# Codes4Fun/moshi.cpp

Measured on AMD Instinct MI355X. Metric: audio frames/sec (12.5 Hz target) moshika-7B q4_k decode, higher is better.
Workload: dtype q4_K weights x q8_K activations (int8 dot, f32 accumulate); bf16 KV; f32 elsewhere; 1 GPU; moshi-sts --bench loop: mimi encode + Temporal step + 8 Depth steps + mimi decode, moshika q4_k, 1 audio stream per GPU, greedy, ctx capacity 3000; context_fill_start=0, parallelism=1 GPU, device= (gfx950:sramecc+:xnack-)

## Files before the change

include/ggml-backend.h:

```cpp
#pragma once

#include "ggml.h"

#ifdef __cplusplus
extern "C" {
#endif

typedef struct ggml_backend_buffer_type * ggml_backend_buffer_type_t;
typedef struct ggml_backend_buffer      * ggml_backend_buffer_t;
typedef struct ggml_backend             * ggml_backend_t;
typedef struct ggml_backend_reg         * ggml_backend_reg_t;
typedef struct ggml_backend_device      * ggml_backend_dev_t;

enum ggml_backend_dev_type {
    GGML_BACKEND_DEVICE_TYPE_CPU,
    GGML_BACKEND_DEVICE_TYPE_GPU,
    GGML_BACKEND_DEVICE_TYPE_ACCEL,
};

struct ggml_backend_dev_caps {
    bool async;
    bool host_buffer;
    bool buffer_from_host_ptr;
    bool events;
// ... 13 lines not shown
GGML_API ggml_backend_reg_t ggml_backend_reg_get(size_t index);
GGML_API const char * ggml_backend_reg_name(ggml_backend_reg_t reg);
GGML_API void * ggml_backend_reg_get_proc_address(ggml_backend_reg_t reg, const char * name);

GGML_API size_t             ggml_backend_dev_count(void);
GGML_API ggml_backend_dev_t ggml_backend_dev_get(size_t index);
GGML_API ggml_backend_dev_t ggml_backend_dev_by_name(const char * name);
GGML_API ggml_backend_dev_t ggml_backend_dev_by_type(enum ggml_backend_dev_type type);
GGML_API const char *       ggml_backend_dev_name(ggml_backend_dev_t device);
GGML_API const char *       ggml_backend_dev_description(ggml_backend_dev_t device);
GGML_API enum ggml_backend_dev_type ggml_backend_dev_type(ggml_backend_dev_t device);
GGML_API void               ggml_backend_dev_memory(ggml_backend_dev_t device, size_t * free, size_t * total);
GGML_API void               ggml_backend_dev_get_props(ggml_backend_dev_t device, struct ggml_backend_dev_props * props);
GGML_API ggml_backend_reg_t ggml_backend_dev_backend_reg(ggml_backend_dev_t device);
GGML_API ggml_backend_t     ggml_backend_dev_init(ggml_backend_dev_t device, const char * params);

GGML_API ggml_backend_t ggml_backend_init_by_name(const char * name, const char * params);
GGML_API ggml_backend_t ggml_backend_init_by_type(enum ggml_backend_dev_type type, const char * params);
GGML_API ggml_backend_t ggml_backend_init_best(void);

GGML_API const char *       ggml_backend_name(ggml_backend_t backend);
GGML_API void               ggml_backend_free(ggml_backend_t backend);
GGML_API ggml_backend_dev_t ggml_backend_get_device(ggml_backend_t backend);
GGML_API void               ggml_backend_synchronize(ggml_backend_t backend);

typedef void (*ggml_backend_set_n_threads_t)(ggml_backend_t backend, int n_threads);

GGML_API ggml_backend_buffer_t ggml_backend_alloc_ctx_tensors(struct ggml_context * ctx, ggml_backend_t backend);
GGML_API void    ggml_backend_buffer_free    (ggml_backend_buffer_t buffer);
GGML_API size_t  ggml_backend_buffer_get_size(ggml_backend_buffer_t buffer);
GGML_API void *  ggml_backend_buffer_get_base(ggml_backend_buffer_t buffer);
GGML_API const char * ggml_backend_buffer_name(ggml_backend_buffer_t buffer);
GGML_API void    ggml_backend_buffer_clear   (ggml_backend_buffer_t buffer, uint8_t value);
GGML_API bool    ggml_backend_buffer_is_host (ggml_backend_buffer_t buffer);

GGML_API void ggml_backend_tensor_set   (      struct ggml_tensor * tensor, const void * data, size_t offset, size_t size);
GGML_API void ggml_backend_tensor_get   (const struct ggml_tensor * tensor,       void * data, size_t offset, size_t size);
GGML_API void ggml_backend_tensor_get_async(ggml_backend_t backend, const struct ggml_tensor * tensor, void * data, size_t offset, size_t size);
typedef struct ggml_backend_event * ggml_backend_event_t;
GGML_API ggml_backend_event_t ggml_backend_event_new(ggml_backend_dev_t device);
GGML_API void ggml_backend_event_free(ggml_backend_event_t event);
GGML_API void ggml_backend_event_record(ggml_backend_event_t event, ggml_backend_t backend);
GGML_API void ggml_backend_event_synchronize(ggml_backend_event_t event);
GGML_API void ggml_backend_event_wait(ggml_backend_t backend, ggml_backend_event_t event);
GGML_API void ggml_backend_tensor_memset(      struct ggml_tensor * tensor, uint8_t value,     size_t offset, size_t size);
GGML_API void ggml_backend_tensor_copy  (struct ggml_tensor * src, struct ggml_tensor * dst);

GGML_API enum ggml_status ggml_backend_graph_compute(ggml_backend_t backend, struct ggml_cgraph * cgraph);
GGML_API bool ggml_backend_supports_op(ggml_backend_t backend, const struct ggml_tensor * op);

struct ggml_mi355x_stats {
    int64_t graphs_computed;
    int64_t graph_replays;
    int64_t kernels_in_last_plan;
    int64_t fused_nodes_in_last_plan;
    int64_t nodes_in_last_plan;
    int64_t uploads_batched;
    int64_t chained_matvecs_in_last_plan;
    int64_t attention_folds_planned;
    int64_t chain_step_programs_in_last_plan;
    int64_t vq_levels_chained_in_last_plan;
    int64_t attn_block_launches_in_last_plan;
    int64_t attn_block_jobs_in_last_plan;
    int64_t generic_attention_nodes_in_last_plan;
    int64_t ring_copy_launches_in_last_plan;
    int64_t ring_copy_jobs_in_last_plan;
};
GGML_API void ggml_backend_mi355x_get_stats(ggml_backend_t backend, struct ggml_mi355x_stats * stats);
struct ggml_mi355x_kernel_profile {
    double  seconds;
    int64_t launches;
    int64_t bytes;
    double  variant_seconds[3];
    int64_t variant_launches[3];
    int64_t variant_bytes[3];
    double  chain_seconds;
    int64_t chain_launches;
    int64_t chain_bytes;
    int64_t chain_phases;
};
GGML_API void ggml_backend_mi355x_get_kernel_profile(ggml_backend_t backend, struct ggml_mi355x_kernel_profile * out);
GGML_API void ggml_backend_mi355x_set_flags(ggml_backend_t backend, int flags);
GGML_API void ggml_backend_mi355x_set_capture(ggml_backend_t backend, int enabled);
GGML_API void * ggml_backend_mi355x_get_stream(ggml_backend_t backend);
GGML_API void ggml_backend_mi355x_make_current(ggml_backend_t backend);
GGML_API ggml_backend_t ggml_backend_mi355x_init_stream(ggml_backend_t base);

#ifdef __cplusplus
}
#endif
```

moshi.cpp_amd/__init__.py:

```python
import ctypes as C
import os

_HERE = os.path.dirname(os.path.abspath(__file__))
LIB_PATH = os.environ.get("MI355X_LIB") or os.path.join(_HERE, "libggml-mi355x.so")
HOT_LIB_PATH = os.environ.get("MI355X_HOT_LIB") or os.path.join(os.path.dirname(LIB_PATH), "libmoshi-hot.so")

GGML_MAX_DIMS, GGML_MAX_SRC, GGML_MAX_NAME = 4, 10, 64

F32, F16, Q4_0, Q8_0, Q4_K, Q8_K, I32, I64, BF16 = 0, 1, 2, 8, 12, 15, 26, 27, 30
TYPE_NAMES = {F32: "f32", F16: "f16", Q4_0: "q4_0", Q8_0: "q8_0", Q4_K: "q4_K", Q8_K: "q8_K", I32: "i32", I64: "i64", BF16: "bf16"}
DEV_CPU, DEV_GPU = 0, 1


class Tensor(C.Structure):
    pass


Tensor._fields_ = [
    ("type", C.c_int),
    ("buffer", C.c_void_p),
    ("ne", C.c_int64 * GGML_MAX_DIMS),
    ("nb", C.c_size_t * GGML_MAX_DIMS),
    ("op", C.c_int),
    ("op_params", C.c_int32 * 16),
# ... 20 lines not shown

class Stats(C.Structure):
    _fields_ = [(n, C.c_int64) for n in ("graphs_computed", "graph_replays", "kernels_in_last_plan",
                                         "fused_nodes_in_last_plan", "nodes_in_last_plan", "uploads_batched", "chained_matvecs_in_last_plan",
                                         "attention_folds_planned", "chain_step_programs_in_last_plan", "vq_levels_chained_in_last_plan",
                                         "attn_block_launches_in_last_plan", "attn_block_jobs_in_last_plan", "generic_attention_nodes_in_last_plan",
                                         "ring_copy_launches_in_last_plan", "ring_copy_jobs_in_last_plan")]


class KernelProfile(C.Structure):
    _fields_ = [("seconds", C.c_double), ("launches", C.c_int64), ("bytes", C.c_int64),
                ("variant_seconds", C.c_double * 3), ("variant_launches", C.c_int64 * 3), ("variant_bytes", C.c_int64 * 3),
                ("chain_seconds", C.c_double), ("chain_launches", C.c_int64), ("chain_bytes", C.c_int64), ("chain_phases", C.c_int64)]


class GGUFInitParams(C.Structure):
    _fields_ = [("no_alloc", C.c_bool), ("ctx", C.POINTER(C.c_void_p))]


P, I, L, Z, F, B, S = C.c_void_p, C.c_int, C.c_int64, C.c_size_t, C.c_float, C.c_bool, C.c_char_p

SIGNATURES = {
    "ggml_time_ms": (L, []), "ggml_time_us": (L, []), "ggml_time_init": (None, []),
    "ggml_type_name": (S, [I]), "ggml_op_name": (S, [I]), "ggml_op_desc": (S, [TP]), "ggml_status_to_string": (S, [I]),
    "ggml_blck_size": (L, [I]), "ggml_type_size": (Z, [I]), "ggml_row_size": (Z, [I, L]), "ggml_is_quantized": (B, [I]),
    "ggml_nelements": (L, [TP]), "ggml_nrows": (L, [TP]), "ggml_nbytes": (Z, [TP]), "ggml_element_size": (Z, [TP]),
    "ggml_n_dims": (I, [TP]), "ggml_is_contiguous": (B, [TP]), "ggml_is_transposed": (B, [TP]), "ggml_is_permuted": (B, [TP]),
    "ggml_are_same_shape": (B, [TP, TP]),
    "ggml_fp16_to_fp32": (F, [C.c_uint16]), "ggml_fp32_to_fp16": (C.c_uint16, [F]),
    "ggml_bf16_to_fp32": (F, [C.c_uint16]), "ggml_fp32_to_bf16": (C.c_uint16, [F]),
    "ggml_init": (P, [InitParams]), "ggml_reset": (None, [P]), "ggml_free": (None, [P]), "ggml_used_mem": (Z, [P]),
    "ggml_get_no_alloc": (B, [P]), "ggml_set_no_alloc": (None, [P, B]),
    "ggml_tensor_overhead": (Z, []), "ggml_graph_overhead": (Z, []), "ggml_graph_overhead_custom": (Z, [Z, B]),
    "ggml_new_tensor": (TP, [P, I, I, C.POINTER(L)]), "ggml_new_tensor_1d": (TP, [P, I, L]), "ggml_new_tensor_2d": (TP, [P, I, L, L]),
    "ggml_new_tensor_3d": (TP, [P, I, L, L, L]), "ggml_new_tensor_4d": (TP, [P, I, L, L, L, L]),
    "ggml_dup_tensor": (TP, [P, TP]), "ggml_view_tensor": (TP, [P, TP]),
    "ggml_get_first_tensor": (TP, [P]), "ggml_get_next_tensor": (TP, [P, TP]), "ggml_get_tensor": (TP, [P, S]),
    "ggml_get_name": (S, [TP]), "ggml_set_name": (TP, [TP, S]), "ggml_format_name": (TP, [TP, S]),
    "ggml_set_input": (None, [TP]), "ggml_set_output": (None, [TP]), "ggml_get_unary_op": (I, [TP]),
    "ggml_dup": (TP, [P, TP]), "ggml_add": (TP, [P, TP, TP]), "ggml_add_inplace": (TP, [P, TP, TP]), "ggml_sub": (TP, [P, TP, TP]),
    "ggml_sub_inplace": (TP, [P, TP, TP]), "ggml_mul_inplace": (TP, [P, TP, TP]), "ggml_div_inplace": (TP, [P, TP, TP]),
    "ggml_mul": (TP, [P, TP, TP]), "ggml_div": (TP, [P, TP, TP]), "ggml_neg": (TP, [P, TP]),
    "ggml_scale": (TP, [P, TP, F]), "ggml_scale_inplace": (TP, [P, TP, F]), "ggml_clamp": (TP, [P, TP, F, F]),
    "ggml_sum": (TP, [P, TP]), "ggml_sum_rows": (TP, [P, TP]), "ggml_argmax": (TP, [P, TP]),
    "ggml_argsort": (TP, [P, TP, I]), "ggml_argsort_top_k": (TP, [P, TP, I]), "ggml_top_k": (TP, [P, TP, I]),
    "ggml_arange": (TP, [P, F, F, F]), "ggml_repeat": (TP, [P, TP, TP]), "ggml_repeat_4d": (TP, [P, TP, L, L, L, L]),
    "ggml_concat": (TP, [P, TP, TP, I]), "ggml_pad": (TP, [P, TP, I, I, I, I]),
    "ggml_silu": (TP, [P, TP]), "ggml_gelu": (TP, [P, TP]), "ggml_elu": (TP, [P, TP]),
    "ggml_norm": (TP, [P, TP, F]), "ggml_rms_norm": (TP, [P, TP, F]), "ggml_mul_mat": (TP, [P, TP, TP]),
    "ggml_soft_max": (TP, [P, TP]), "ggml_soft_max_ext": (TP, [P, TP, TP, F, F]),
    "ggml_cast": (TP, [P, TP, I]), "ggml_cpy": (TP, [P, TP, TP]), "ggml_cont": (TP, [P, TP]),
    "ggml_reshape_1d": (TP, [P, TP, L]), "ggml_reshape_2d": (TP, [P, TP, L, L]), "ggml_reshape_3d": (TP, [P, TP, L, L, L]),
    "ggml_reshape_4d": (TP, [P, TP, L, L, L, L]),
    "ggml_view_1d": (TP, [P, TP, L, Z]), "ggml_view_2d": (TP, [P, TP, L, L, Z, Z]), "ggml_view_3d": (TP, [P, TP, L, L, L, Z, Z, Z]),
    "ggml_view_4d": (TP, [P, TP, L, L, L, L, Z, Z, Z, Z]),
    "ggml_permute": (TP, [P, TP, I, I, I, I]), "ggml_transpose": (TP, [P, TP]),
    "ggml_get_rows": (TP, [P, TP, TP]), "ggml_set_rows": (TP, [P, TP, TP, TP]),
    "ggml_im2col": (TP, [P, TP, TP, I, I, I, I, I, I, B, I]), "ggml_conv_1d": (TP, [P, TP, TP, I, I, I]),
    "ggml_conv_transpose_1d": (TP, [P, TP, TP, I, I, I]), "ggml_timestep_embedding": (TP, [P, TP, I, I]),
    "ggml_new_graph": (P, [P]), "ggml_new_graph_custom": (P, [P, Z, B]), "ggml_build_forward_expand": (None, [P, TP]),
    "ggml_graph_clear": (None, [P]), "ggml_graph_size": (I, [P]), "ggml_graph_n_nodes": (I, [P]), "ggml_graph_node": (TP, [P, I]),
    "ggml_graph_nodes": (C.POINTER(TP), [P]), "ggml_graph_n_leafs": (I, [P]), "ggml_graph_leaf": (TP, [P, I]), "ggml_graph_print": (None, [P]),
    "ggml_quantize_row": (None, [I, P, P, L]), "ggml_dequantize_row": (None, [I, P, P, L]),
    "ggml_backend_load_all": (None, []), "ggml_backend_reg_count": (Z, []), "ggml_backend_reg_get": (P, [Z]),
    "ggml_backend_reg_name": (S, [P]), "ggml_backend_reg_get_proc_address": (P, [P, S]),
    "ggml_backend_dev_count": (Z, []), "ggml_backend_dev_get": (P, [Z]), "ggml_backend_dev_by_name": (P, [S]),
    "ggml_backend_dev_by_type": (P, [I]), "ggml_backend_dev_name": (S, [P]), "ggml_backend_dev_description": (S, [P]),
    "ggml_backend_dev_type": (I, [P]), "ggml_backend_dev_memory": (None, [P, C.POINTER(Z), C.POINTER(Z)]),
    "ggml_backend_dev_get_props": (None, [P, C.POINTER(DevProps)]), "ggml_backend_dev_backend_reg": (P, [P]),
    "ggml_backend_dev_init": (P, [P, S]),
    "ggml_backend_init_by_name": (P, [S, S]), "ggml_backend_init_by_type": (P, [I, S]), "ggml_backend_init_best": (P, []),
    "ggml_backend_name": (S, [P]), "ggml_backend_free": (None, [P]), "ggml_backend_get_device": (P, [P]),
    "ggml_backend_synchronize": (None, [P]),
    "ggml_backend_alloc_ctx_tensors": (P, [P, P]), "ggml_backend_buffer_free": (None, [P]), "ggml_backend_buffer_get_size": (Z, [P]),
    "ggml_backend_buffer_get_base": (P, [P]), "ggml_backend_buffer_name": (S, [P]), "ggml_backend_buffer_clear": (None, [P, C.c_uint8]),
    "ggml_backend_buffer_is_host": (B, [P]),
    "ggml_backend_tensor_set": (None, [TP, P, Z, Z]), "ggml_backend_tensor_get": (None, [TP, P, Z, Z]),
    "ggml_backend_tensor_memset": (None, [TP, C.c_uint8, Z, Z]), "ggml_backend_tensor_copy": (None, [TP, TP]),
    "ggml_backend_graph_compute": (I, [P, P]), "ggml_backend_supports_op": (B, [P, TP]),
    "ggml_backend_mi355x_get_stats": (None, [P, C.POINTER(Stats)]), "ggml_backend_mi355x_set_flags": (None, [P, I]), "ggml_backend_mi355x_set_capture": (None, [P, I]),
    "ggml_backend_mi355x_get_stream": (P, [P]),
    "ggml_backend_mi355x_make_current": (None, [P]),
    "ggml_backend_mi355x_init_stream": (P, [P]),
    "ggml_backend_tensor_get_async": (None, [P, TP, P, Z, Z]),
    "ggml_backend_event_new": (P, [P]), "ggml_backend_event_free": (None, [P]), "ggml_backend_event_record": (None, [P, P]),
    "ggml_backend_event_synchronize": (None, [P]),
    "ggml_backend_event_wait": (None, [P, P]),
    "ggml_backend_mi355x_get_kernel_profile": (None, [P, C.POINTER(KernelProfile)]),
    "ggml_backend_cpu_init": (P, []), "ggml_backend_is_cpu": (B, [P]), "ggml_backend_cpu_set_n_threads": (None, [P, I]),
    "ggml_graph_compute_with_ctx": (I, [P, P, I]),
    "ggml_backend_cpu_reg": (P, []), "ggml_backend_cpu_set_graph_compute": (None, [P]),
    "gguf_init_empty": (P, []), "gguf_init_from_file": (P, [S, GGUFInitParams]), "gguf_free": (None, [P]),
    "gguf_get_version": (C.c_uint32, [P]), "gguf_get_alignment": (Z, [P]), "gguf_get_data_offset": (Z, [P]),
    "gguf_get_n_kv": (L, [P]), "gguf_find_key": (L, [P, S]), "gguf_get_key": (S, [P, L]), "gguf_get_val_str": (S, [P, L]),
    "gguf_get_val_u32": (C.c_uint32, [P, L]), "gguf_set_val_u32": (None, [P, S, C.c_uint32]), "gguf_set_val_str": (None, [P, S, S]),
    "gguf_get_n_tensors": (L, [P]), "gguf_find_tensor": (L, [P, S]), "gguf_get_tensor_name": (S, [P, L]),
    "gguf_get_tensor_type": (I, [P, L]), "gguf_get_tensor_offset": (Z, [P, L]), "gguf_get_tensor_size": (Z, [P, L]),
    "gguf_add_tensor": (None, [P, TP]), "gguf_write_to_file": (B, [P, S, B]),
}

_lib = None


class _Libs:

    def __init__(self, ggml, hot):
        self.ggml, self.hot = ggml, hot

    def __getattr__(self, name):
        for lib in (self.__dict__["ggml"], self.__dict__["hot"]):
            try:
                fn = getattr(lib, name)
            except AttributeError:
                continue
            setattr(self, name, fn)
            return fn
        raise AttributeError(name)


def load():
    global _lib
    if _lib is not None:
        return _lib
    for path in (LIB_PATH, HOT_LIB_PATH):
        if not os.path.exists(path):
            raise RuntimeError(f"{path} not found: build it with moshi.cpp_amd/build.sh (hipcc --offload-arch=gfx950); "
                               "there is no CPU or Python fallback for the decode hot path")
    lib = C.CDLL(LIB_PATH, mode=C.RTLD_GLOBAL)
    missing = []
    for name, (res, args) in SIGNATURES.items():
        try:
            fn = getattr(lib, name)
        except AttributeError:
            missing.append(name)
            continue
        fn.restype, fn.argtypes = res, args
    if missing:
        raise RuntimeError(f"libggml-mi355x.so lacks symbols declared in include/*.h: {missing}")
    stray = [n for n in ("moshi_hot_create", "moshi_hot_sts_frame") if hasattr(lib, n)]
    if stray:
        raise RuntimeError(f"the boundary library must not carry the harness: {stray}")
    hot_lib = C.CDLL(HOT_LIB_PATH, mode=C.RTLD_GLOBAL)
    from . import hot as _hot
    _hot.attach(hot_lib)
    _lib = _Libs(lib, hot_lib)
    return _lib


def declared_symbols():
    return sorted(SIGNATURES)
```

moshi.cpp_amd/csrc/hip_backend.hip:

```cpp
#include "hip_common.h"
#include "ggml-cpu.h"

#include <string.h>

#include <algorithm>
#include <functional>
#include <deque>
#include <map>
#include <memory>
#include <set>
#include <string>
#include <unordered_map>
#include <vector>

#define UPLOAD_SLOTS       8
#define UPLOAD_BLOB_BYTES  (64 * 1024)
#define UPLOAD_MAX_DESCS   1024
#define READBACK_PINNED_BYTES (64 * 1024)
#define AGET_SLOTS 64
#define AGET_SLOT_BYTES 256
#define UPLOAD_SMALL_MAX   16384

struct plan_t;

struct upload_slot {
    char * blob = nullptr;
    upload_desc * descs = nullptr;
    hipEvent_t done = nullptr;
    bool in_flight = false;
};

struct hip_ctx {
    int device = 0;
    std::string name, description;
    hipStream_t stream = nullptr;
    int flags = 0;
    bool no_capture = false;
    ggml_mi355x_stats stats = {};
    std::map<size_t, std::vector<void *>> pool;
    upload_slot slots[UPLOAD_SLOTS];
    int cur_slot = 0;
    int n_pending = 0;
    size_t pending_bytes = 0;
    mv_profile prof = { nullptr, 0, 0 };
    double prof_seconds = 0; int64_t prof_launches = 0, prof_bytes = 0;
    double prof_seconds_v[3] = { 0, 0, 0 }; int64_t prof_launches_v[3] = { 0, 0, 0 }, prof_bytes_v[3] = { 0, 0, 0 };
    double prof_chain_seconds = 0; int64_t prof_chain_launches = 0, prof_chain_bytes = 0, prof_chain_phases = 0;
    hipEvent_t chain_ev[2] = { nullptr, nullptr };
    std::unordered_map<const ggml_cgraph *, plan_t *> plans;
    uint64_t orphan_clock = 0;
    volatile unsigned * err_host = nullptr;
    unsigned * err_dev = nullptr;
    char * readback = nullptr;
    struct async_get { void * dst; size_t size; int slot; uint64_t seq; };
    char * aget_pinned = nullptr;
    std::deque<async_get> aget_pending;
    uint64_t aget_seq = 0;
    bool in_use = false;
    int usable_cus = 0;
    ggml_backend_device dev_obj;
};

static std::vector<hip_ctx *> & contexts() { static std::vector<hip_ctx *> v; return v; }
static std::vector<hip_ctx *> & stream_contexts() { static std::vector<hip_ctx *> v; return v; }

static void set_device(hip_ctx * c) { HIP_CHECK(hipSetDevice(c->device)); }

static void ctx_init_lazy(hip_ctx * c) {
    if (c->stream) return;
    set_device(c);
    {
        hipDeviceProp_t prop;
        HIP_CHECK(hipGetDeviceProperties(&prop, c->device));
        c->usable_cus = prop.multiProcessorCount;
        const char * e = getenv("MI355X_STREAM_CUS");
        const int lim = e ? atoi(e) : 0;
        if (lim > 0 && lim < prop.multiProcessorCount) {
            std::vector<uint32_t> mask((size_t) (prop.multiProcessorCount + 31) / 32, 0u);
            for (int i = 0; i < lim; i++) mask[(size_t) i / 32] |= 1u << (i % 32);
            HIP_CHECK(hipExtStreamCreateWithCUMask(&c->stream, (uint32_t) mask.size(), mask.data()));
            c->usable_cus = lim;
        }
    }
    if (!c->stream) HIP_CHECK(hipStreamCreateWithFlags(&c->stream, hipStreamNonBlocking));
    for (auto & s : c->slots) {
        HIP_CHECK(hipHostMalloc((void **) &s.blob, UPLOAD_BLOB_BYTES, hipHostMallocMapped));
        HIP_CHECK(hipHostMalloc((void **) &s.descs, UPLOAD_MAX_DESCS * sizeof(upload_desc), hipHostMallocMapped));
        HIP_CHECK(hipEventCreateWithFlags(&s.done, hipEventDisableTiming));
    }
    HIP_CHECK(hipHostMalloc((void **) &c->readback, READBACK_PINNED_BYTES, hipHostMallocDefault));
    HIP_CHECK(hipHostMalloc((void **) &c->aget_pinned, AGET_SLOTS * AGET_SLOT_BYTES, hipHostMallocDefault));
    HIP_CHECK(hipHostMalloc((void **) &c->err_host, 64, hipHostMallocMapped));
    c->err_host[0] = 0u;
    HIP_CHECK(hipHostGetDevicePointer((void **) &c->err_dev, (void *) c->err_host, 0));
}

static void check_device_error(hip_ctx * c) {
    if (c->err_host && c->err_host[0] != 0u)
        GGML_ABORT("mi355x backend: a kernel gave up a bounded wait (code %u: 1 = split attention head barrier, 2 = chain engine hand-off, 3 = stream engine hand-off); results are invalid", c->err_host[0]);
}

static size_t size_class(size_t n) {
    if (n > ((size_t) 64 << 20)) return 0;
    size_t c = 256;
    while (c < n) c <<= 1;
    return c;
}
static void * pool_poison(hip_ctx * c, void * p, size_t n) {
    static const bool poison = getenv("MI355X_POISON") != nullptr;
    if (poison && p) { HIP_CHECK(hipMemsetAsync(p, 0xFF, n, c->stream)); HIP_CHECK(hipStreamSynchronize(c->stream)); }
    return p;
}
#define GUARD_BYTES 4096
static bool guard_mode() { static const bool g = getenv("MI355X_GUARD") != nullptr; return g; }
static void guard_fill(hip_ctx * c, char * user, size_t actual) {
    HIP_CHECK(hipMemsetAsync(user - GUARD_BYTES, 0xA5, GUARD_BYTES, c->stream));
    HIP_CHECK(hipMemsetAsync(user + actual, 0xA5, GUARD_BYTES, c->stream));
}
static void guard_check(hip_ctx * c, char * user, size_t actual) {
    static std::vector<unsigned char> h(2 * GUARD_BYTES);
    HIP_CHECK(hipStreamSynchronize(c->stream));
    HIP_CHECK(hipMemcpy(h.data(), user - GUARD_BYTES, GUARD_BYTES, hipMemcpyDeviceToHost));
    HIP_CHECK(hipMemcpy(h.data() + GUARD_BYTES, user + actual, GUARD_BYTES, hipMemcpyDeviceToHost));
    for (size_t i = 0; i < 2 * GUARD_BYTES; i++)
        if (h[i] != 0xA5) GGML_ABORT("mi355x: guard zone %s a %zu-byte allocation was overwritten (offset %zu)", i < GUARD_BYTES ? "before" : "after", actual, i % GUARD_BYTES);
}
static void * pool_alloc(hip_ctx * c, size_t n, size_t * actual) {
    set_device(c);
    const size_t cls = size_class(n ? n : 1);
    if (cls) {
        auto & fl = c->pool[cls];
        *actual = cls;
        if (!fl.empty()) { void * p = fl.back(); fl.pop_back(); if (guard_mode()) guard_fill(c, (char *) p, *actual); return pool_poison(c, p, *actual); }
    } else *actual = n;
    void * p = nullptr;
    hipError_t e = hipMalloc(&p, *actual + (guard_mode() ? 2 * GUARD_BYTES : 0));
    if (e != hipSuccess) { fprintf(stderr, "mi355x: hipMalloc(%zu) failed: %s\n", *actual, hipGetErrorString(e)); return nullptr; }
    if (guard_mode()) { p = (char *) p + GUARD_BYTES; guard_fill(c, (char *) p, *actual); }
    return pool_poison(c, p, *actual);
}
// ... 35 lines not shown
    c->pending_bytes += padded;
}

struct hip_buffer_ctx { hip_ctx * c; size_t actual; };

static void deliver_async_gets(hip_ctx * c, uint64_t upto) {
    while (!c->aget_pending.empty() && c->aget_pending.front().seq <= upto) {
        const hip_ctx::async_get & g = c->aget_pending.front();
        memcpy(g.dst, c->aget_pinned + (size_t) g.slot * AGET_SLOT_BYTES, g.size);
        c->aget_pending.pop_front();
    }
}

static void evict_plans_of_buffer(hip_ctx * c, const ggml_backend_buffer * b);

static void hip_buf_free(ggml_backend_buffer_t b) {
    hip_buffer_ctx * bc = (hip_buffer_ctx *) b->context;
    flush_uploads(bc->c);
    evict_plans_of_buffer(bc->c, b);
    for (hip_ctx * o : contexts()) if (o != bc->c && o->device == bc->c->device) evict_plans_of_buffer(o, b);
    for (hip_ctx * o : stream_contexts()) if (o != bc->c && o->device == bc->c->device) evict_plans_of_buffer(o, b);
    pool_free(bc->c, b->base, bc->actual);
    delete bc;
    delete b;
}
static void hip_buf_set(ggml_backend_buffer_t b, struct ggml_tensor * t, const void * data, size_t offset, size_t size) {
    hip_ctx * c = ((hip_buffer_ctx *) b->context)->c;
    set_device(c);
    if (size <= UPLOAD_SMALL_MAX && !(c->flags & 4)) { queue_upload(c, (char *) t->data + offset, data, size); return; }
    flush_uploads(c);
    HIP_CHECK(hipMemcpyAsync((char *) t->data + offset, data, size, hipMemcpyHostToDevice, c->stream));
    HIP_CHECK(hipStreamSynchronize(c->stream));
}
static void hip_buf_get(ggml_backend_buffer_t b, const struct ggml_tensor * t, void * data, size_t offset, size_t size) {
    hip_ctx * c = ((hip_buffer_ctx *) b->context)->c;
    set_device(c);
    flush_uploads(c);
    if (size <= READBACK_PINNED_BYTES) {
        HIP_CHECK(hipMemcpyAsync(c->readback, (const char *) t->data + offset, size, hipMemcpyDeviceToHost, c->stream));
        HIP_CHECK(hipStreamSynchronize(c->stream));
        memcpy(data, c->readback, size);
    } else {
        HIP_CHECK(hipMemcpyAsync(data, (const char *) t->data + offset, size, hipMemcpyDeviceToHost, c->stream));
        HIP_CHECK(hipStreamSynchronize(c->stream));
    }
    deliver_async_gets(c, c->aget_seq);
    check_device_error(c);
}
static void hip_buf_memset(ggml_backend_buffer_t b, struct ggml_tensor * t, uint8_t v, size_t offset, size_t size) {
    hip_ctx * c = ((hip_buffer_ctx *) b->context)->c;
    set_device(c);
    flush_uploads(c);
    HIP_CHECK(hipMemsetAsync((char *) t->data + offset, v, size, c->stream));
}
static void hip_buf_clear(ggml_backend_buffer_t b, uint8_t v) {
    hip_ctx * c = ((hip_buffer_ctx *) b->context)->c;
    set_device(c);
    flush_uploads(c);
    HIP_CHECK(hipMemsetAsync(b->base, v, b->size, c->stream));
}

static ggml_backend_buffer_t hip_alloc_buffer(ggml_backend_t backend, size_t size) {
    hip_ctx * c = (hip_ctx *) backend->context;
    ctx_init_lazy(c);
    size_t actual = 0;
    void * p = pool_alloc(c, size, &actual);
    if (!p) return NULL;
    auto * b = new ggml_backend_buffer;
    b->iface = { hip_buf_free, hip_buf_memset, hip_buf_set, hip_buf_get, hip_buf_clear };
    b->device = &c->dev_obj;
    b->base = p;
    b->size = size;
    b->context = new hip_buffer_ctx{ c, actual };
    b->is_host = false;
    return b;
}

typedef std::function<void(hipStream_t)> step_fn;
struct pstep {
    step_fn fn; bool is_mv = false; mv_args mv;
    chain_plan * chain = nullptr;
    const vq_level_args * vq = nullptr;
    const char * hoist_dst = nullptr; size_t hoist_bytes = 0;
    template <typename F> pstep(F f) : fn(std::move(f)) { memset(&mv, 0, sizeof(mv)); }
    pstep(const mv_args & a) : fn([a](hipStream_t s) { k_matvec(s, a); }), is_mv(true), mv(a) {}
    template <typename F> static pstep special_step(F f, int special, const attn_args * at, const lowrank_embed_args * lr, const sample_args * smp = nullptr) {
        pstep st(std::move(f));
        st.is_mv = true; st.mv.special = special; st.mv.attn = at; st.mv.lr = lr; st.mv.smp = smp;
        return st;
    }
};

struct plan_t {
    std::vector<pstep> steps;
    std::vector<chain_plan *> chains;
    std::vector<std::pair<void *, size_t>> workspaces;
    std::vector<std::unique_ptr<attn_args>> attn_copies;
    std::vector<std::unique_ptr<lowrank_embed_args>> lowrank_copies;
    std::vector<std::unique_ptr<sample_args>> sampler_copies;
    std::vector<std::unique_ptr<vq_level_args>> vq_copies;
    std::vector<vq_chain_plan *> vq_chains;
    std::vector<std::unique_ptr<conv_scatter>> scatter_slots;
    std::vector<const ggml_backend_buffer *> buffers;
    uint64_t orphan_seq = 0;
    hipGraph_t graph = nullptr;
    hipGraphExec_t exec = nullptr;
    uint64_t hash = 0;
    int n_nodes = 0, n_fused = 0, n_chained = 0, n_attn_folded = 0, n_step_programs = 0, n_vq_chained = 0, n_attn_block_launches = 0, n_attn_block_jobs = 0, n_generic_attn_nodes = 0, n_ring_copy_launches = 0, n_ring_copy_jobs = 0;
};

static void plan_free(hip_ctx * c, plan_t * p) {
    if (p->exec) (void) hipGraphExecDestroy(p->exec);
    if (p->graph) (void) hipGraphDestroy(p->graph);
    for (auto & w : p->workspaces) pool_free(c, w.first, w.second);
    for (chain_plan * ch : p->chains) k_chain_free(ch);
    for (vq_chain_plan * vc : p->vq_chains) k_vq_chain_free(vc);
    delete p;
}

#define MAX_ORPHANS 8
static void collect_plan_buffers(plan_t * p, const ggml_cgraph * g) {
    p->buffers.clear();
    auto note = [&](const ggml_tensor * t) {
        const ggml_backend_buffer * b = t->buffer ? t->buffer : (t->view_src ? t->view_src->buffer : nullptr);
        if (b && std::find(p->buffers.begin(), p->buffers.end(), b) == p->buffers.end()) p->buffers.push_back(b);
    };
    for (int i = 0; i < g->n_nodes; i++) note(g->nodes[i]);
    for (int i = 0; i < g->n_leafs; i++) note(g->leafs[i]);
}
static void evict_plans_of_buffer(hip_ctx * c, const ggml_backend_buffer * b) {
    for (auto & kv : c->plans) {
        plan_t * p = kv.second;
        if (p->orphan_seq || std::find(p->buffers.begin(), p->buffers.end(), b) == p->buffers.end()) continue;
        p->orphan_seq = ++c->orphan_clock;
        p->buffers.clear();
    }
    for (;;) {
        int n = 0; auto oldest = c->plans.end();
        for (auto it = c->plans.begin(); it != c->plans.end(); ++it)
            if (it->second->orphan_seq) { n++; if (oldest == c->plans.end() || it->second->orphan_seq < oldest->second->orphan_seq) oldest = it; }
        if (n <= MAX_ORPHANS) break;
        if (c->stream) { set_device(c); HIP_CHECK(hipStreamSynchronize(c->stream)); }
        plan_free(c, oldest->second);
        c->plans.erase(oldest);
    }
}

static uint64_t graph_hash(const ggml_cgraph * g) {
    constexpr size_t NW = offsetof(ggml_tensor, name) / 8;
    static_assert(offsetof(ggml_tensor, name) % 32 == 0, "tensor descriptor is hashed in 4 lanes of 8-byte words");
    uint64_t h[4] = { 0xcbf29ce484222325ull ^ (uint64_t) g->n_nodes, 0x9e3779b97f4a7c15ull ^ (uint64_t) g->n_leafs, 0xc2b2ae3d27d4eb4full, 0x165667b19e3779f9ull };
    auto mix = [&](const ggml_tensor * t) {
        uint64_t w[NW];
        memcpy(w, t, NW * 8);
        w[offsetof(ggml_tensor, buffer) / 8] = 0;
        h[0] = (h[0] ^ (uint64_t) (uintptr_t) t) * 0x100000001b3ull;
        for (size_t i = 0; i < NW; i += 4) {
            h[0] = (h[0] ^ w[i]) * 0x100000001b3ull; h[1] = (h[1] ^ w[i + 1]) * 0x100000001b3ull;
            h[2] = (h[2] ^ w[i + 2]) * 0x100000001b3ull; h[3] = (h[3] ^ w[i + 3]) * 0x100000001b3ull;
        }
    };
    for (int i = 0; i < g->n_nodes; i++) mix(g->nodes[i]);
    for (int i = 0; i < g->n_leafs; i++) mix(g->leafs[i]);
    uint64_t r = h[0];
    for (int k = 1; k < 4; k++) r = (r ^ (h[k] >> 29) ^ h[k]) * 0x100000001b3ull;
    return r;
}

struct analysis {
    const ggml_cgraph * g;
    std::unordered_map<const ggml_tensor *, int> index;
    std::unordered_map<const ggml_tensor *, int> uses;
    std::unordered_map<const ggml_tensor *, int> last_consumer;
    std::vector<char> skip;
};

static void analyse(analysis & an, const ggml_cgraph * g) {
    an.g = g;
    an.skip.assign((size_t) g->n_nodes, 0);
    for (int i = 0; i < g->n_nodes; i++) {
        const ggml_tensor * n = g->nodes[i];
        an.index[n] = i;
        for (int s = 0; s < GGML_MAX_SRC; s++) {
            const ggml_tensor * src = n->src[s];
            if (!src || src == n) continue;
            bool dup = false;
            for (int s2 = 0; s2 < s; s2++) if (n->src[s2] == src) dup = true;
            if (dup) continue;
            an.uses[src]++;
            an.last_consumer[src] = i;
// ... 1536 lines not shown
            if (!match_scalar_gather(an, i, grp)) continue;
            bool clash = false;
            for (int m : grp.members) if (an.skip[(size_t) m]) clash = true;
            if (clash) continue;
            for (int m : grp.members) an.skip[(size_t) m] = 1;
            for (auto & f : grp.steps) at_pos[grp.emit_pos].push_back(f);
            p->n_fused += (int) grp.members.size();
        }
        static const bool no_sampler = getenv("MI355X_NO_SAMPLER_FUSION") != nullptr;
        for (int i = g->n_nodes - 1; i >= 0 && !no_sampler; i--) {
            if (an.skip[(size_t) i] || g->nodes[i]->op != GGML_OP_GET_ROWS || g->nodes[i]->type != GGML_TYPE_I32) continue;
            step_group grp;
            if (!match_sampler(an, i, grp)) continue;
            bool clash = false;
            for (int m : grp.members) if (an.skip[(size_t) m]) clash = true;
            if (clash) continue;
            for (int m : grp.members) an.skip[(size_t) m] = 1;
            p->sampler_copies.emplace_back(new sample_args(grp.smp));
            for (auto & f : grp.steps) at_pos[grp.emit_pos].push_back(pstep::special_step(f, 3, nullptr, nullptr, p->sampler_copies.back().get()));
            p->n_fused += (int) grp.members.size();
        }
        for (int i = g->n_nodes - 1; i >= 0 && !no_sampler; i--) {
            if (an.skip[(size_t) i] || g->nodes[i]->op != GGML_OP_GET_ROWS || g->nodes[i]->type != GGML_TYPE_I32) continue;
            sample_streams_args sa;
            std::vector<int> members;
            if (!match_sampler_streams(an, i, sa, members)) continue;
            bool clash = false;
            for (int m : members) if (an.skip[(size_t) m]) clash = true;
            if (clash) continue;
            for (int m : members) an.skip[(size_t) m] = 1;
            at_pos[i].push_back([=](hipStream_t s) { k_sample_topk_streams(s, sa); });
            p->n_fused += (int) members.size();
        }
        static const bool no_xattn = getenv("MI355X_NO_CROSS_ATTN_FUSION") != nullptr;
        for (int i = 0; i < g->n_nodes && !no_xattn; i++) {
            if (an.skip[(size_t) i] || g->nodes[i]->op != GGML_OP_CONT) continue;
            xattn_group xg;
            if (!match_cross_attention(an, i, xg)) continue;
            bool clash = false;
            for (int m : xg.members) if (an.skip[(size_t) m]) clash = true;
            if (clash) continue;
            for (int m : xg.members) an.skip[(size_t) m] = 1;
            const xattn_args xa = xg.a;
            at_pos[xg.emit_pos].push_back([=](hipStream_t s) { k_cross_attn(s, xa); });
            p->n_fused += (int) xg.members.size();
        }
        static const bool no_lowrank = getenv("MI355X_NO_LOWRANK_FUSION") != nullptr;
        for (int i = 0; i < g->n_nodes && !no_lowrank; i++) {
            const ggml_tensor * mm = g->nodes[i];
            if (an.skip[(size_t) i] || mm->op != GGML_OP_MUL_MAT || mm->type != GGML_TYPE_F32) continue;
            const ggml_tensor * W = mm->src[0], * gr = mm->src[1];
            if (W->type != GGML_TYPE_Q8_0 || !dense_rows(W) || W->ne[2] * W->ne[3] != 1 || gr->op != GGML_OP_GET_ROWS || gr->type != GGML_TYPE_F32) continue;
            const int pg = pos_of(an, gr);
            if (pg < 0 || an.skip[(size_t) pg] || uses_of(an, gr) != 1 || ggml_nelements(gr) != gr->ne[0] || gr->ne[0] != W->ne[0]) continue;
            const ggml_tensor * tab = gr->src[0], * idx = gr->src[1];
            if (ggml_nelements(idx) != 1 || idx->type != GGML_TYPE_I32 || !dense_rows(tab) || !idx->data) continue;
            switch (tab->type) { case GGML_TYPE_F32: case GGML_TYPE_F16: case GGML_TYPE_BF16: case GGML_TYPE_Q4_0: case GGML_TYPE_Q8_0: break; default: continue; }
            const int64_t K = W->ne[0], M = W->ne[1];
            if (K % 32 != 0 || K > 2048 || ggml_nelements(mm) != M || !ggml_is_contiguous(mm)) continue;
            std::vector<int> members = { pg, i };
            float * out = (float *) mm->data;
            int emit = i;
            const ggml_tensor * cp = sole_consumer(an, mm);
            if (cp && cp->op == GGML_OP_CPY && uses_of(an, mm) == 1 && cp->type == GGML_TYPE_F32 && cp->src[0] == mm && ggml_is_contiguous(cp) && cp->view_src == NULL &&
                ggml_are_same_shape(cp, mm) && pos_of(an, cp) >= 0 && !an.skip[(size_t) pos_of(an, cp)]) {
                members.push_back(pos_of(an, cp)); out = (float *) cp->data; emit = pos_of(an, cp);
            }
            for (int m2 : members) an.skip[(size_t) m2] = 1;
            const lowrank_embed_args la = { (const char *) tab->data, (int64_t) tab->nb[1], tab->ne[1], (int) tab->type, (const int32_t *) idx->data,
                                            (const char *) W->data, (int64_t) W->nb[1], (int) K, (int) M, out };
            p->lowrank_copies.emplace_back(new lowrank_embed_args(la));
            at_pos[emit].push_back(pstep::special_step([=](hipStream_t s) { k_lowrank_embed(s, la); }, 2, nullptr, p->lowrank_copies.back().get()));
            p->n_fused += (int) members.size();
        }
        for (int i = g->n_nodes - 1; i >= 0; i--) {
            if (an.skip[(size_t) i] || g->nodes[i]->op != GGML_OP_ADD) continue;
            embed_group grp;
            if (!match_embed_sum(an, i, grp)) continue;
            bool clash = false;
            for (int m : grp.members) if (m < 0 || an.skip[(size_t) m]) clash = true;
            if (clash) continue;
            for (int m : grp.members) an.skip[(size_t) m] = 1;
            const embed_sum_args a = grp.a;
            at_pos[i].push_back([=](hipStream_t s) { k_embed_sum(s, a); });
            p->n_fused += (int) grp.members.size();
        }
        for (int i = 0; i < g->n_nodes; i++) {
            row_copy_group rg;
            if (an.skip[(size_t) i] || g->nodes[i]->op != GGML_OP_CONT || !match_row_copies(an, i, rg)) continue;
            for (int m : rg.members) an.skip[(size_t) m] = 1;
            const copy_rows_args ra = rg.a;
            at_pos[rg.emit_pos].push_back([=](hipStream_t s) { k_copy_rows(s, ra); });
            p->n_fused += (int) rg.members.size();
        }
        for (int i = 0; i < g->n_nodes; i++) {
            const ggml_tensor * n = g->nodes[i];
            if (an.skip[(size_t) i] || n->op != GGML_OP_CPY) continue;
            const ggml_tensor * ct = n->src[0];
            const int pc = pos_of(an, ct);
            if (ct->op != GGML_OP_CONT || pc < 0 || an.skip[(size_t) pc] || uses_of(an, ct) != 1 || ct->view_src) continue;
            if (ct->type != GGML_TYPE_F32 || n->type != GGML_TYPE_F32 || ct->src[0]->type != GGML_TYPE_F32 || !ggml_are_same_shape(ct, ct->src[0]) ||
                !ggml_are_same_shape(n, ct) || !ggml_is_contiguous(n)) continue;
            bool writer_between = false;
            for (int j = pc + 1; j < i; j++) if (writes_through_alias(g->nodes[j])) writer_between = true;
            if (writer_between) continue;
            an.skip[(size_t) i] = an.skip[(size_t) pc] = 1;
            const tdesc d = make_tdesc(n), x = make_tdesc(ct->src[0]);
            at_pos[i].push_back([=](hipStream_t s) { k_cpy(s, d, x); });
            p->n_fused += 2;
        }
        for (int i = 0; i < g->n_nodes; i++) {
            const ggml_tensor * n = g->nodes[i];
            if (an.skip[(size_t) i] || n->op != GGML_OP_TIMESTEP_EMBEDDING) continue;
            const ggml_tensor * ad = n->src[0];
            const int pa = pos_of(an, ad);
            if (ad->op != GGML_OP_ADD || pa < 0 || an.skip[(size_t) pa] || uses_of(an, ad) != 1 || ad->view_src || ad->type != GGML_TYPE_F32) continue;
            const ggml_tensor * x = ad->src[0], * y = ad->src[1];
            if (x->type != GGML_TYPE_F32 || y->type != GGML_TYPE_F32 || !ggml_is_contiguous(x) || !ggml_is_contiguous(y) || !ggml_are_same_shape(x, ad) ||
                ggml_nelements(ad) != ad->ne[0] || !(ggml_nelements(y) == ggml_nelements(ad) || ggml_nelements(y) == 1)) continue;
            an.skip[(size_t) i] = an.skip[(size_t) pa] = 1;
            const tdesc d = make_tdesc(n), tx = make_tdesc(x);
            const float * yp = (const float *) y->data; const int yn = (int) ggml_nelements(y);
            const int dim = n->op_params[0], mp = n->op_params[1];
            {
                pstep st([=](hipStream_t s) { k_timestep_embedding(s, d, tx, dim, mp, yp, yn); });
                if (x->op == GGML_OP_NONE && y->op == GGML_OP_NONE && !x->view_src && !y->view_src) { st.hoist_dst = (const char *) n->data; st.hoist_bytes = ggml_nbytes(n); }
                at_pos[i].push_back(std::move(st));
            }
            p->n_fused += 2;
        }
        std::unordered_map<const void *, float *> paired_gate;
        size_t paired_consumed = 0;
        static const bool no_pair = getenv("MI355X_PAIRED_GATE") != nullptr && atoi(getenv("MI355X_PAIRED_GATE")) == 0;
        static const bool no_batched_fusion = getenv("MI355X_NO_BATCHED_MM") != nullptr || getenv("MI355X_NO_BATCHED_FUSION") != nullptr;
        for (int i = 0; i < g->n_nodes; i++) {
            if (an.skip[(size_t) i] || g->nodes[i]->op != GGML_OP_MUL_MAT) continue;
            mv_group grp;
            if (!match_matvec(an, i, grp)) {
                bmm_group bg;
                if (!no_batched_fusion && match_batched_mm(an, i, em, bg)) {
                    bool bclash = false;
                    for (int m : bg.members) if (m != i && an.skip[(size_t) m]) bclash = true;
                    if (!bclash) {
                        for (int m : bg.members) an.skip[(size_t) m] = 1;
                        at_pos[bg.emit_pos].push_back(bg.run);
                        p->n_fused += (int) bg.members.size();
                    }
                }
                continue;
            }
            bool clash = false;
            for (int m : grp.members) if (m < 0 || (m != i && an.skip[(size_t) m])) clash = true;
            if (clash) continue;
            for (int m : grp.members) an.skip[(size_t) m] = 1;
            mv_args a = grp.a;
            if (is_qblock((enum ggml_type) a.wtype) && a.ncols == 1 && !no_argmax_epilogue) {
                const ggml_tensor * ynode = g->nodes[grp.emit_pos];
                const ggml_tensor * am = nullptr;
                int n_am = 0;
                for (int j = grp.emit_pos + 1; j < g->n_nodes; j++) if (g->nodes[j]->op == GGML_OP_ARGMAX && g->nodes[j]->src[0] == ynode) { am = g->nodes[j]; n_am++; }
                if (am && n_am == 1 && !an.skip[(size_t) pos_of(an, am)] && (float *) ynode->data == a.y && ggml_nelements(ynode) == a.M && am->data) {
                    a.argmax_out[0] = (int32_t *) am->data;
                    an.skip[(size_t) pos_of(an, am)] = 1;
                    const ggml_tensor * cp = nullptr;
                    for (int j = pos_of(an, am) + 1; j < g->n_nodes; j++)
                        if (g->nodes[j]->op == GGML_OP_CPY && g->nodes[j]->src[0] == am && g->nodes[j]->type == GGML_TYPE_I32 && ggml_nelements(g->nodes[j]) == 1) { cp = g->nodes[j]; break; }
                    if (cp && !an.skip[(size_t) pos_of(an, cp)]) { a.argmax_out[1] = (int32_t *) cp->data; an.skip[(size_t) pos_of(an, cp)] = 1; }
                    unsigned * tk = (unsigned *) em.ws(256 + 2 * 4 * 8192);
                    HIP_CHECK(hipMemsetAsync(tk, 0, 256, em.c->stream));
                    a.ticket = tk;
                    p->n_fused += 1 + (cp ? 1 : 0);
                }
            }
            if (a.prologue == MV_PLAIN && is_qblock((enum ggml_type) a.wtype) && a.ncols == 1 && !no_attn_prologue) {
                for (auto & ag : attn_groups) {
                    const attn_args & at = ag.a;
                    if (ag.emit_pos < 0 || ag.B > 1 || ag.column || (const float *) at.out != a.x || at.T != 1 || at.D != 64 || at.C > 8 || (int64_t) at.H * at.D != a.K) continue;
                    if (a.K != 1024 || at.H != 16 || ag.emit_pos > grp.emit_pos || uses_of(an, g->nodes[ag.emit_pos]) != 1) continue;
                    p->attn_copies.emplace_back(new attn_args(at));
                    a.prologue = MV_ATTN;
                    a.attn = p->attn_copies.back().get();
                    ag.emit_pos = -1;
                    break;
                }
            }
            if (a.prologue == MV_RMSNORM && a.wtype == GGML_TYPE_Q4_K && a.ncols == 1 && keep && !(c->flags & 512) && grp.emit_pos == i) {
                bool merged = false;
                for (auto & ag : attn_groups) {
                    const attn_args & at = ag.a;
                    if (ag.emit_pos < 0 || ag.B > 1 || ag.column || at.q != a.y || ag.emit_pos < grp.emit_pos) continue;
                    if (!k_inproj_attn_supported(a, at, c->usable_cus)) continue;
                    bool private_y = true;
                    std::vector<const ggml_tensor *> aliases { g->nodes[i] };
                    for (int j = i + 1; j < g->n_nodes && private_y; j++) {
                        const ggml_tensor * nj = g->nodes[j];
                        bool reads = false;
                        for (int sidx = 0; sidx < GGML_MAX_SRC; sidx++)
                            if (nj->src[sidx] && std::find(aliases.begin(), aliases.end(), nj->src[sidx]) != aliases.end()) reads = true;
                        if (!reads) continue;
                        const bool layout = nj->op == GGML_OP_VIEW || nj->op == GGML_OP_RESHAPE || nj->op == GGML_OP_PERMUTE || nj->op == GGML_OP_TRANSPOSE;
                        if (layout) { aliases.push_back(nj); continue; }
                        if (std::find(ag.members.begin(), ag.members.end(), j) == ag.members.end()) private_y = false;
                    }
                    if (!private_y || !spin_kernels_allowed(c)) continue;
                    const mv_args am = a; const attn_args aa = at;
                    unsigned * err = c->err_dev;
                    const size_t wn = k_inproj_attn_ws_size(a, at);
                    void * ws = em.ws(wn);
                    HIP_CHECK(hipMemsetAsync(ws, 0, wn, c->stream));
// ... 88 lines not shown
    for (size_t gi = 0; gi < attn_groups.size(); ) {
        if (!attn_groups[gi].column || attn_groups[gi].emit_pos < 0) { gi++; continue; }
        const attn_args & a0 = attn_groups[gi].a;
        std::set<int> inside(attn_groups[gi].members.begin(), attn_groups[gi].members.end());
        size_t ge = gi + 1;
        int lo = attn_groups[gi].emit_pos, hi = lo;
        const attn_args * rows = a0.T > 1 ? &a0 : nullptr;
        while (ge < attn_groups.size() && ge - gi < ATTN_BLOCKS_MAX) {
            const attn_group & n = attn_groups[ge];
            const attn_args & b = n.a;
            if (!n.column || n.emit_pos < 0 || b.H != a0.H || b.D != a0.D || b.C != a0.C || b.scale != a0.scale || b.out_ts != a0.out_ts || (b.rot != nullptr) != (a0.rot != nullptr) ||
                (b.T > 1 && rows && (b.q_ts != rows->q_ts || b.k_ts != rows->k_ts || b.v_ts != rows->v_ts)) || b.q_hs != a0.q_hs || b.k_hs != a0.k_hs || b.v_hs != a0.v_hs ||
                b.k_nb1 != a0.k_nb1 || b.k_nb2 != a0.k_nb2 || b.v_nb1 != a0.v_nb1 || b.v_nb2 != a0.v_nb2 || b.kcache == a0.kcache) break;
            std::set<int> both = inside;
            both.insert(n.members.begin(), n.members.end());
            const int nlo = n.emit_pos < lo ? n.emit_pos : lo, nhi = n.emit_pos > hi ? n.emit_pos : hi;
            bool clean = true;
            for (int i = nlo + 1; i < nhi && clean; i++) if (!is_view_op(g->nodes[i]->op) && !both.count(i)) clean = false;
            if (!clean) break;
            inside.swap(both); lo = nlo; hi = nhi;
            if (b.T > 1 && !rows) rows = &b;
            ge++;
        }
        attn_blocks_args ba;
        memset(&ba, 0, sizeof(ba));
        ba.a = a0;
        if (rows) { ba.a.q_ts = rows->q_ts; ba.a.k_ts = rows->k_ts; ba.a.v_ts = rows->v_ts; }
        ba.n_jobs = (int) (ge - gi);
        for (size_t k = gi; k < ge; k++) {
            const attn_args & b = attn_groups[k].a;
            ba.job[k - gi] = { b.q, b.k, b.v, b.kcache, b.vcache, b.mask, b.rot, b.index, b.out, b.T };
            attn_groups[k].emit_pos = -1;
        }
        unsigned * err = c->err_dev;
        auto & at = at_pos[hi];
        at.insert(at.begin(), [=](hipStream_t s) { attn_blocks_args b = ba; b.write_only = 0; k_attn_blocks(s, b, err); });
        at.insert(at.begin(), [=](hipStream_t s) { attn_blocks_args b = ba; b.write_only = 1; k_attn_blocks(s, b, err); });
        p->n_attn_block_launches += 2; p->n_attn_block_jobs += ba.n_jobs;
        gi = ge;
    }
    for (auto & ag : attn_groups) {
        if (ag.emit_pos < 0) continue;
        const attn_args a = ag.a;
        unsigned * err = c->err_dev;
        if (ag.B > 1) {
            const attn_streams_args sa = ag.sa;
            at_pos[ag.emit_pos].insert(at_pos[ag.emit_pos].begin(), [=](hipStream_t s) { k_attn_streams(s, sa, err); });
            continue;
        }
        if (a.T > 4) {
            at_pos[ag.emit_pos].insert(at_pos[ag.emit_pos].begin(), [=](hipStream_t s) {
                attn_args b = a;
                b.n_groups = (a.T + 3) / 4;
                b.write_only = 1; k_attn_decode(s, b, nullptr, err);
                b.write_only = 0; k_attn_decode(s, b, nullptr, err);
            });
            continue;
        }
        void * ws = nullptr;
        if (const size_t n = k_attn_split_resident(a, c->usable_cus) ? k_attn_decode_ws_size(a) : 0) { ws = em.ws(n); HIP_CHECK(hipMemsetAsync(ws, 0, n, c->stream)); }
        if (a.T <= 4 && a.n_groups <= 1 && !ws) {
            p->attn_copies.emplace_back(new attn_args(a));
            at_pos[ag.emit_pos].insert(at_pos[ag.emit_pos].begin(), pstep::special_step([=](hipStream_t s) { k_attn_decode(s, a, ws, err); }, 1, p->attn_copies.back().get(), nullptr));
        } else
        at_pos[ag.emit_pos].insert(at_pos[ag.emit_pos].begin(), [=](hipStream_t s) { k_attn_decode(s, a, ws, err); });
    }
    const bool dump = getenv("MI355X_DUMP_PLAN") != nullptr;
    for (int i = 0; i < g->n_nodes; i++) {
        if (dump) {
            const ggml_tensor * n = g->nodes[i];
            const bool layout = n->op == GGML_OP_VIEW || n->op == GGML_OP_RESHAPE || n->op == GGML_OP_PERMUTE || n->op == GGML_OP_TRANSPOSE;
            auto itd = at_pos.find(i);
            if (!layout || itd != at_pos.end())
                fprintf(stderr, "plan %4d %-18s [%5lld %5lld %4lld %2lld] %s%s%s\n", i, ggml_op_name(n->op), (long long) n->ne[0], (long long) n->ne[1], (long long) n->ne[2],
                        (long long) n->ne[3], an.skip[(size_t) i] ? "fused" : (layout ? "-" : "GENERIC"), itd != at_pos.end() ? " <emit group>" : "", n->view_src ? " (alias)" : "");
        }
        if (!an.skip[(size_t) i]) {
            if (g->nodes[i]->op == GGML_OP_SOFT_MAX || g->nodes[i]->op == GGML_OP_SET_ROWS) p->n_generic_attn_nodes++;
            emit_generic(em, g->nodes[i]);
        }
        auto it = at_pos.find(i);
        if (it != at_pos.end()) for (auto & f : it->second) p->steps.push_back(f);
    }
    if (fuse && keep && !(c->flags & 16) && ((c->flags & 32) || k_chain_default_on()) && spin_kernels_possible(c)) {
        for (size_t i = 1; i + 1 < p->steps.size(); i++) {
            pstep & h = p->steps[i];
            const pstep & m = p->steps[i - 1];
            if (!h.hoist_dst || !m.is_mv || m.mv.special || m.mv.wtype != GGML_TYPE_F32 || m.mv.ncols != 2 || !p->steps[i + 1].is_mv) continue;
            auto clash = [&](const float * q, int64_t n_floats) { return q && (const char *) q < h.hoist_dst + h.hoist_bytes && h.hoist_dst < (const char *) (q + n_floats); };
            const mv_args & a = m.mv;
            if (clash(a.x, a.x_cs * (a.ncols - 1) + a.K) || clash(a.y, a.y_cs * (a.ncols - 1) + a.M) || clash(a.x_out, a.K * a.ncols) || clash(a.residual, a.r_cs * (a.ncols - 1) + a.M) ||
                clash(a.alpha, a.K) || clash(a.beta, a.K)) continue;
            std::swap(p->steps[i - 1], p->steps[i]);
        }
        std::vector<pstep> merged;
        size_t i = 0;
        while (i < p->steps.size()) {
            if (p->steps[i].vq) {
                size_t e = i;
                std::vector<vq_level_args> lv;
                while (e < p->steps.size() && p->steps[e].vq && lv.size() < 32 && (lv.empty() || ((const void *) p->steps[e].vq->resid == (const void *) lv.back().resid_out && p->steps[e].vq->resid_stride == 4))) {
                    lv.push_back(*p->steps[e].vq); e++;
                }
                if (lv.size() >= 2 && k_vq_chain_accept(lv.data(), (int) lv.size(), c->usable_cus) && spin_kernels_allowed(c)) {
                    void * ws = em.ws(k_vq_chain_ws_size((int) lv.size()));
                    vq_chain_plan * vc = k_vq_chain_create(c->stream, lv.data(), (int) lv.size(), ws, c->err_dev);
                    p->vq_chains.push_back(vc);
                    p->n_vq_chained += (int) lv.size();
                    merged.push_back(pstep([vc](hipStream_t s) { k_vq_chain_launch(s, vc); }));
                    if (dump) fprintf(stderr, "plan: %zu consecutive RVQ levels -> one launch\n", lv.size());
                    i = e;
                    continue;
                }
                merged.push_back(std::move(p->steps[i])); i++; continue;
            }
            if (!p->steps[i].is_mv) { merged.push_back(std::move(p->steps[i])); i++; continue; }
            size_t e = i;
            while (e < p->steps.size() && p->steps[e].is_mv) e++;
            std::vector<mv_args> run;
            for (size_t k = i; k < e; k++) run.push_back(p->steps[k].mv);
            size_t k = 0;
            while (k < run.size()) {
                int len = k_chain_accept(run.data() + k, (int) (run.size() - k), c->usable_cus, !(c->flags & 1024));
                if (len > 0 && !spin_kernels_allowed(c)) len = 0;
                if (len <= 0) {
                    merged.push_back(std::move(p->steps[i + k])); k++; continue;
                }
                void * ws = em.ws(k_chain_ws_size(run.data() + k, len, c->usable_cus, !(c->flags & 1024)));
                chain_plan * ch = k_chain_create(c->stream, run.data() + k, len, ws, c->err_dev, c->usable_cus, !(c->flags & 1024));
                p->chains.push_back(ch);
                if (k_chain_is_step_program(ch)) p->n_step_programs++;
                merged.push_back(pstep([ch](hipStream_t s) { k_chain_launch(s, ch); }));
                merged.back().chain = ch;
                p->n_chained += len;
                if (dump) fprintf(stderr, "plan: %d consecutive mat-vecs -> one chain launch (%.1f MB of weights)\n", len, (double) k_chain_weight_bytes(ch) / 1e6);
                k += (size_t) len;
            }
            i = e;
        }
        p->steps.swap(merged);
    }
    return p;
}

static void run_steps(hip_ctx * c, plan_t * p) { for (auto & st : p->steps) st.fn(c->stream); }

static void run_steps_profiled(hip_ctx * c, plan_t * p) {
    if (!c->prof.recs) {
        c->prof.capacity = 4096;
        c->prof.recs = new mv_profile::rec[(size_t) c->prof.capacity];
        for (int i = 0; i < c->prof.capacity; i++) { HIP_CHECK(hipEventCreate(&c->prof.recs[i].start)); HIP_CHECK(hipEventCreate(&c->prof.recs[i].stop)); }
    }
    c->prof.used = 0;
    k_matvec_set_profile(&c->prof);
    for (auto & st : p->steps) {
        if (!st.chain) { st.fn(c->stream); continue; }
        if (!c->chain_ev[0]) { HIP_CHECK(hipEventCreate(&c->chain_ev[0])); HIP_CHECK(hipEventCreate(&c->chain_ev[1])); }
        HIP_CHECK(hipStreamSynchronize(c->stream));
        HIP_CHECK(hipEventRecord(c->chain_ev[0], c->stream));
        st.fn(c->stream);
        HIP_CHECK(hipEventRecord(c->chain_ev[1], c->stream));
        HIP_CHECK(hipEventSynchronize(c->chain_ev[1]));
        float ms = 0;
        HIP_CHECK(hipEventElapsedTime(&ms, c->chain_ev[0], c->chain_ev[1]));
        c->prof_chain_seconds += (double) ms * 1e-3; c->prof_chain_launches++; c->prof_chain_bytes += k_chain_weight_bytes(st.chain); c->prof_chain_phases += k_chain_length(st.chain);
    }
// ... 142 lines not shown
    set_device(c);
    flush_uploads(c);
    HIP_CHECK(hipStreamWaitEvent(c->stream, h->ev, 0));
}
static bool hip_supports_op(ggml_backend_t, const struct ggml_tensor * op) {
    switch (op->op) {
        case GGML_OP_CPY: case GGML_OP_CONT: case GGML_OP_DUP:
            if (ggml_is_quantized(op->type) || ggml_is_quantized(op->src[0]->type)) {
                if (op->type == op->src[0]->type) return true;
                const enum ggml_type st = op->src[0]->type;
                return (st == GGML_TYPE_F32 || st == GGML_TYPE_F16 || st == GGML_TYPE_BF16) &&
                       (op->type == GGML_TYPE_Q8_0 || op->type == GGML_TYPE_Q4_0 || op->type == GGML_TYPE_Q4_K) && op->src[0]->ne[0] % ggml_blck_size(op->type) == 0;
            }
            return true;
        case GGML_OP_MUL_MAT:
            switch (op->src[0]->type) { case GGML_TYPE_F32: case GGML_TYPE_F16: case GGML_TYPE_BF16: case GGML_TYPE_Q4_0: case GGML_TYPE_Q8_0: case GGML_TYPE_Q4_K: return true; default: return false; }
        default: return op->op < GGML_OP_COUNT;
    }
}

static const char * hip_dev_name(ggml_backend_dev_t d) { return ((hip_ctx *) d->context)->name.c_str(); }
static const char * hip_dev_desc(ggml_backend_dev_t d) { return ((hip_ctx *) d->context)->description.c_str(); }
static void hip_dev_memory(ggml_backend_dev_t d, size_t * free, size_t * total) {
    hip_ctx * c = (hip_ctx *) d->context;
    set_device(c);
    if (hipMemGetInfo(free, total) != hipSuccess) { *free = 0; *total = 0; }
}
static enum ggml_backend_dev_type hip_dev_type(ggml_backend_dev_t) { return GGML_BACKEND_DEVICE_TYPE_GPU; }
static ggml_backend_t hip_dev_init(ggml_backend_dev_t d, const char *) {
    hip_ctx * c = (hip_ctx *) d->context;
    ctx_init_lazy(c);
    if (c->flags != 0) { HIP_CHECK(hipStreamSynchronize(c->stream)); for (auto & kv : c->plans) plan_free(c, kv.second); c->plans.clear(); c->flags = 0; }
    c->stats = {};
    auto * b = new ggml_backend;
    b->iface = { hip_backend_name, hip_backend_free, hip_backend_sync, hip_alloc_buffer, hip_graph_compute, hip_supports_op, hip_get_tensor_async, hip_event_record, hip_event_wait };
    b->device = d;
    b->context = c;
    return b;
}

static const char * hip_reg_name(ggml_backend_reg_t) { return "ROCm"; }
static size_t hip_reg_dev_count(ggml_backend_reg_t) { return contexts().size(); }
static ggml_backend_dev_t hip_reg_get_dev(ggml_backend_reg_t, size_t i) { return &contexts()[i]->dev_obj; }
static void * hip_reg_proc(ggml_backend_reg_t, const char *) { return NULL; }

extern "C" ggml_backend_reg_t ggml_backend_mi355x_reg(void) {
    static ggml_backend_reg reg = { { hip_reg_name, hip_reg_dev_count, hip_reg_get_dev, hip_reg_proc }, NULL };
    static bool init = false;
    if (!init) {
        init = true;
        int n = 0;
        if (hipGetDeviceCount(&n) != hipSuccess) n = 0;
        for (int i = 0; i < n; i++) {
            hipDeviceProp_t prop;
            if (hipGetDeviceProperties(&prop, i) != hipSuccess) continue;
            hip_ctx * c = new hip_ctx;
            c->device = i;
            c->name = "ROCm" + std::to_string(i);
            c->description = std::string(prop.name) + " (" + prop.gcnArchName + ")";
            c->dev_obj.iface = { hip_dev_name, hip_dev_desc, hip_dev_memory, hip_dev_type, hip_dev_init };
            c->dev_obj.reg = &reg;
            c->dev_obj.context = c;
            contexts().push_back(c);
        }
    }
    return contexts().empty() ? NULL : &reg;
}

static hip_ctx * ctx_of(ggml_backend_t b) {
    GGML_ASSERT(b && b->iface.get_name == hip_backend_name && "not an MI355X backend");
    return (hip_ctx *) b->context;
}
extern "C" void ggml_backend_mi355x_get_stats(ggml_backend_t b, struct ggml_mi355x_stats * stats) { *stats = ctx_of(b)->stats; }
extern "C" void ggml_backend_mi355x_set_capture(ggml_backend_t b, int enabled) {
    if (b && b->iface.get_name == hip_backend_name) ((hip_ctx *) b->context)->no_capture = !enabled;
}
extern "C" void ggml_backend_mi355x_set_flags(ggml_backend_t b, int flags) {
    hip_ctx * c = ctx_of(b);
    if (c->stream) { flush_uploads(c); HIP_CHECK(hipStreamSynchronize(c->stream)); }
    for (auto & kv : c->plans) plan_free(c, kv.second);
    c->plans.clear();
    c->flags = flags;
}
extern "C" void ggml_backend_mi355x_get_kernel_profile(ggml_backend_t b, struct ggml_mi355x_kernel_profile * out) {
    hip_ctx * c = ctx_of(b);
    out->seconds = c->prof_seconds; out->launches = c->prof_launches; out->bytes = c->prof_bytes;
    for (int v = 0; v < 3; v++) { out->variant_seconds[v] = c->prof_seconds_v[v]; out->variant_launches[v] = c->prof_launches_v[v]; out->variant_bytes[v] = c->prof_bytes_v[v]; }
    out->chain_seconds = c->prof_chain_seconds; out->chain_launches = c->prof_chain_launches; out->chain_bytes = c->prof_chain_bytes; out->chain_phases = c->prof_chain_phases;
}
extern "C" void * ggml_backend_mi355x_get_stream(ggml_backend_t b) { hip_ctx * c = ctx_of(b); ctx_init_lazy(c); return (void *) c->stream; }
extern "C" void ggml_backend_mi355x_make_current(ggml_backend_t b) { hip_ctx * c = ctx_of(b); ctx_init_lazy(c); set_device(c); }
extern "C" ggml_backend_t ggml_backend_mi355x_init_stream(ggml_backend_t base) {
    if (!base || base->iface.get_name != hip_backend_name) return NULL;
    hip_ctx * b0 = (hip_ctx *) base->context;
    hip_ctx * c = nullptr;
    int n_same = 0;
    for (hip_ctx * o : stream_contexts()) if (o->device == b0->device) { n_same++; if (!o->in_use && !c) c = o; }
    if (!c) {
        c = new hip_ctx;
        c->device = b0->device;
        c->name = b0->name + "/s" + std::to_string(n_same + 1);
        c->description = b0->description + ", additional stream";
        c->dev_obj.iface = b0->dev_obj.iface;
        c->dev_obj.reg = b0->dev_obj.reg;
        c->dev_obj.context = c;
        stream_contexts().push_back(c);
    }
    c->in_use = true;
    ggml_backend_t b = c->dev_obj.iface.init_backend(&c->dev_obj, NULL);
    c->flags = b0->flags;
    c->no_capture = b0->no_capture;
    return b;
}
```

moshi.cpp_amd/csrc/hip_common.h:

```cpp
#pragma once

#include <hip/hip_runtime.h>
#include <stdint.h>

#include "ggml_impl.h"

#define HIP_CHECK(expr) do { hipError_t e_ = (expr); if (e_ != hipSuccess) \
    GGML_ABORT("HIP error %s at %s: %s", hipGetErrorName(e_), #expr, hipGetErrorString(e_)); } while (0)

struct tdesc {
    char *  data;
    int64_t ne[4];
    int64_t nb[4];
    int     type;
};

static inline tdesc make_tdesc(const struct ggml_tensor * t) {
    tdesc d;
    d.data = (char *) t->data;
    for (int i = 0; i < 4; i++) { d.ne[i] = t->ne[i]; d.nb[i] = (int64_t) t->nb[i]; }
    d.type = (int) t->type;
    return d;
}

// ... 60 lines not shown
    float *     x_out;
    embed_src   res_embed;
    int32_t *   argmax_out[2];
    unsigned *  ticket;
    const attn_args * attn;
    int64_t     pair_F;
    int         special;
    const struct lowrank_embed_args * lr;
    const struct sample_args * smp;
};
struct chain_plan;
bool   k_chain_default_on();
int    k_chain_accept(const mv_args * mv, int n, int usable_cus, bool allow_step_program = true);
size_t k_chain_ws_size(const mv_args * mv, int n, int usable_cus, bool allow_step_program = true);
chain_plan * k_chain_create(hipStream_t s, const mv_args * mv, int n, void * ws, unsigned * err, int usable_cus, bool allow_step_program);
bool   k_chain_is_step_program(const chain_plan * c);
void   k_chain_launch(hipStream_t s, const chain_plan * c);
void   k_chain_free(chain_plan * c);
int    k_chain_length(const chain_plan * c);
int64_t k_chain_weight_bytes(const chain_plan * c);
bool k_matvec_supported(int wtype, int64_t K, int64_t M);
bool k_matvec_pair_ok(int wtype, int64_t K, int64_t F);
struct mv_profile {
    struct rec { hipEvent_t start, stop; int64_t bytes; int variant; };
    rec * recs; int capacity; int used;
};
void k_matvec_set_profile(mv_profile * p);
void k_matvec(hipStream_t s, const mv_args & a);
#define MV_XBLK_BYTES 304
void k_gate_quant_q8k(hipStream_t s, const float * h, int64_t K, void * out_blocks, int wtype);
void k_norm_quant_q8k(hipStream_t s, const float * x, const float * alpha, float eps, int64_t K, void * out_blocks, int wtype, float * n_out);
size_t k_mm_q4k_batched_ws_size(int64_t K, int64_t T);
bool k_mm_q4k_batched_supported(int wtype, int64_t K, int64_t M, int64_t T);
void k_mm_q4k_batched(hipStream_t s, int wtype, const char * w, int64_t row_bytes, int64_t K, int64_t M, int64_t T, const float * x, int64_t x_cs,
                      void * ws, float * y, int64_t y_cs, const float * residual, int64_t r_cs, int prologue = 0, const float * alpha = nullptr, float eps = 0.f);

struct attn_args {
    const float * q; const float * k; const float * v;
    int64_t q_ts, q_hs, k_ts, k_hs, v_ts, v_hs;
    const float * rot;
    const float * mask;
    const int32_t * index;
    char * kcache; char * vcache;
    int64_t k_nb1, k_nb2, v_nb1, v_nb2;
    int H, D, C, T;
    float scale;
    float * out;
    int64_t out_ts;
    int n_groups, write_only;
    int row_split;
};
#define ATTN_SPLIT_MIN_C 1024
#define ATTN_SPLIT_SLOTS 128
#define ATTN_SPLIT_BIG_MIN 1024
#define ATTN_SINGLE_MAX 384
size_t k_attn_decode_ws_size(const attn_args & a);
bool k_attn_split_resident(const attn_args & a, int usable_cus);
void k_attn_decode(hipStream_t s, const attn_args & a, void * ws = nullptr, unsigned * err = nullptr);
struct attn_streams_args { attn_args a; int B; int64_t q_bs, k_bs, v_bs, kc_bs, vc_bs, out_bs, mask_bs, rot_bs, index_bs; };
void k_attn_streams(hipStream_t s, const attn_streams_args & a, unsigned * err = nullptr);
#define ATTN_BLOCKS_MAX 16
struct attn_block_job { const float * q, * k, * v; char * kcache, * vcache; const float * mask, * rot; const int32_t * index; float * out; int T; };
struct attn_blocks_args { attn_args a; int n_jobs, write_only; attn_block_job job[ATTN_BLOCKS_MAX]; };
void k_attn_blocks(hipStream_t s, const attn_blocks_args & a, unsigned * err = nullptr);
#define COPY_ROWS_MAX 16
struct copy_rows_args { const float * src[COPY_ROWS_MAX]; float * dst; int64_t n; int rows; };
void k_copy_rows(hipStream_t s, const copy_rows_args & a);
#define RING_COPY_MAX 64
struct ring_copy_job { const char * src; char * dst; int64_t src_hs, dst_hs; };
struct ring_copy_args { int n_jobs, H; int64_t run_bytes; int blocks_per_run; ring_copy_job job[RING_COPY_MAX]; };
void k_ring_copy(hipStream_t s, const ring_copy_args & a, int usable_cus);

bool   k_inproj_attn_supported(const mv_args & a, const attn_args & at, int usable_cus);
size_t k_inproj_attn_ws_size(const mv_args & a, const attn_args & at);
void   k_inproj_attn(hipStream_t s, const mv_args & a, const attn_args & at, void * ws, unsigned * err);

struct xattn_args { const float * q; const char * k; const char * v; int64_t k_nb1, k_nb2, v_nb1, v_nb2; int H, D, Tc; float scale; float * out;
                    int B = 1; int64_t q_cs = 0, out_cs = 0, k_nb3 = 0, v_nb3 = 0; };
void k_cross_attn(hipStream_t s, const xattn_args & a);

#define EMBED_SUM_MAX 40
struct embed_sum_args { embed_src src[EMBED_SUM_MAX]; int n; int64_t K; float * out; int B; };
void k_embed_sum(hipStream_t s, const embed_sum_args & a);
struct vq_level_args {
    const char * emb; int64_t emb_row_bytes; int D, NC;
    const char * resid; int64_t resid_stride;
    const float * add_c; const float * num;
    float * resid_out; float * idx_f; int32_t * idx_i;
    float * cand_val; int32_t * cand_idx; unsigned * counter;
};
#define GATHER_MAX 32
struct gather_args { const float * src[GATHER_MAX]; int n; void * dst; int dst_type; };
void k_gather_scalars(hipStream_t s, const gather_args & a);
#define SAMPLE_MAX_N 32768
#define SAMPLE_MAX_K 256
struct lowrank_embed_args { const char * table; int64_t row_bytes, n_rows; int type; const int32_t * index; const char * w; int64_t w_row_bytes; int K, M; float * out; };
void k_lowrank_embed(hipStream_t s, const lowrank_embed_args & a);
struct sample_args { const float * logits; int n; float scale; int k; const float * noise; int32_t * out; int32_t * out2; };
void k_sample_topk(hipStream_t s, const sample_args & a);
#define SAMPLE_MAX_B 16
struct sample_streams_args { const float * logits; int n; float scale; const float * inv_temp; int k; const float * noise; int32_t * out; int32_t * out2; int B; };
void k_sample_topk_streams(hipStream_t s, const sample_streams_args & a);
#define HEADS_MAX 16
#define HEADS_MAX_M 16
struct heads_streams_args { const char * w[HEADS_MAX]; float * out[HEADS_MAX]; int64_t row_bytes; int wtype; int K, M, n_heads, B; const float * x; int64_t x_cs, out_bs; };
void k_heads_streams(hipStream_t s, const heads_streams_args & a);
#define VQ_LEVEL_WS_BYTES 4096
void k_vq_level(hipStream_t s, const vq_level_args & a);
struct vq_chain_plan;
bool   k_vq_chain_accept(const vq_level_args * lv, int n, int usable_cus);
size_t k_vq_chain_ws_size(int n);
vq_chain_plan * k_vq_chain_create(hipStream_t s, const vq_level_args * lv, int n, void * ws, unsigned * err);
void   k_vq_chain_launch(hipStream_t s, const vq_chain_plan * c);
void   k_vq_chain_free(vq_chain_plan * c);
```

moshi.cpp_amd/csrc/hip_device.h:

```cpp
#pragma once

#include "hip_common.h"

__device__ __forceinline__ char * at(const tdesc & t, int64_t i0, int64_t i1, int64_t i2, int64_t i3) {
    return t.data + i0 * t.nb[0] + i1 * t.nb[1] + i2 * t.nb[2] + i3 * t.nb[3];
}
__device__ __forceinline__ void unravel(const tdesc & t, int64_t i, int64_t & i0, int64_t & i1, int64_t & i2, int64_t & i3) {
    uint32_t r = (uint32_t) i;
    const uint32_t n0 = (uint32_t) t.ne[0], n1 = (uint32_t) t.ne[1], n2 = (uint32_t) t.ne[2];
    uint32_t q = r / n0; i0 = r - q * n0; r = q;
    q = r / n1; i1 = r - q * n1; r = q;
    q = r / n2; i2 = r - q * n2; i3 = q;
}
__device__ __forceinline__ void row_coords(const tdesc & t, int64_t rr, int64_t & i1, int64_t & i2, int64_t & i3) {
    uint32_t r = (uint32_t) rr;
    const uint32_t n1 = (uint32_t) t.ne[1], n2 = (uint32_t) t.ne[2];
    uint32_t q = r / n1; i1 = r - q * n1; r = q;
    q = r / n2; i2 = r - q * n2; i3 = q;
}
__device__ __forceinline__ int64_t wrap(int64_t i, int64_t n) { return n == 1 ? 0 : (i < n ? i : (int64_t) ((uint32_t) i % (uint32_t) n)); }
__host__ __device__ __forceinline__ int elem_size(int type) {
    switch (type) {
        case GGML_TYPE_F32: case GGML_TYPE_I32: return 4;
        case GGML_TYPE_F16: case GGML_TYPE_BF16: case GGML_TYPE_I16: return 2;
// ... 93 lines not shown
}
__device__ __forceinline__ double wave_allsum_f64(double v) {
    v += dpp_f64<DPP_QUAD_XOR1>(v);
    v += dpp_f64<DPP_QUAD_XOR2>(v);
    v += dpp_f64<DPP_HALF_MIRROR>(v);
    v += dpp_f64<DPP_ROW_MIRROR>(v);
    const int lo = __double2loint(v), hi = __double2hiint(v);
    const double r0 = __hiloint2double(__builtin_amdgcn_readlane(hi, 0), __builtin_amdgcn_readlane(lo, 0));
    const double r1 = __hiloint2double(__builtin_amdgcn_readlane(hi, 16), __builtin_amdgcn_readlane(lo, 16));
    const double r2 = __hiloint2double(__builtin_amdgcn_readlane(hi, 32), __builtin_amdgcn_readlane(lo, 32));
    const double r3 = __hiloint2double(__builtin_amdgcn_readlane(hi, 48), __builtin_amdgcn_readlane(lo, 48));
    return (r0 + r1) + (r2 + r3);
}
__device__ __forceinline__ int wave_allmax_i32(int v) {
    v = max(v, dpp_i32<DPP_QUAD_XOR1>(v));
    v = max(v, dpp_i32<DPP_QUAD_XOR2>(v));
    v = max(v, dpp_i32<DPP_HALF_MIRROR>(v));
    v = max(v, dpp_i32<DPP_ROW_MIRROR>(v));
    return max(max(__builtin_amdgcn_readlane(v, 0), __builtin_amdgcn_readlane(v, 16)), max(__builtin_amdgcn_readlane(v, 32), __builtin_amdgcn_readlane(v, 48)));
}
__device__ __forceinline__ void lds_barrier() {
    __builtin_amdgcn_fence(__ATOMIC_RELEASE, "workgroup", "local");
    __builtin_amdgcn_s_barrier();
    __builtin_amdgcn_fence(__ATOMIC_ACQUIRE, "workgroup", "local");
}

template <typename V> __device__ __forceinline__ void st_agent(V * p, V v) { __hip_atomic_store(p, v, __ATOMIC_RELAXED, __HIP_MEMORY_SCOPE_AGENT); }
template <typename V> __device__ __forceinline__ V ld_agent(const V * p) { return __hip_atomic_load(p, __ATOMIC_RELAXED, __HIP_MEMORY_SCOPE_AGENT); }
__device__ __forceinline__ void drain_stores() { __builtin_amdgcn_fence(__ATOMIC_RELEASE, "workgroup"); }
__device__ __forceinline__ void xchg_agent_wait(float * p, float v) { const float o = __hip_atomic_exchange(p, v, __ATOMIC_RELAXED, __HIP_MEMORY_SCOPE_AGENT); asm volatile("" :: "v"(o)); }
__device__ __forceinline__ void xchg_agent_wait(int * p, int v) { const int o = __hip_atomic_exchange(p, v, __ATOMIC_RELAXED, __HIP_MEMORY_SCOPE_AGENT); asm volatile("" :: "v"(o)); }
__device__ __forceinline__ void xchg_agent_wait(double * p, double v) { const double o = __hip_atomic_exchange(p, v, __ATOMIC_RELAXED, __HIP_MEMORY_SCOPE_AGENT); asm volatile("" :: "v"(o)); }

__device__ __forceinline__ double group_allsum_f64(double v, int n) {
    if (n == 16 || n == 8) {
        v += dpp_f64<DPP_QUAD_XOR1>(v);
        v += dpp_f64<DPP_QUAD_XOR2>(v);
        v += dpp_f64<DPP_HALF_MIRROR>(v);
        if (n == 16) v += dpp_f64<DPP_ROW_MIRROR>(v);
        return v;
    }
    for (int o = n >> 1; o > 0; o >>= 1) v += __shfl_xor(v, o, 64);
    return v;
}
__device__ __forceinline__ int quad_allsum_i32(int v) { v += dpp_i32<DPP_QUAD_XOR1>(v); v += dpp_i32<DPP_QUAD_XOR2>(v); return v; }
__device__ __forceinline__ float row16_allsum_f32(float v) {
    v += dpp_f32<DPP_QUAD_XOR1>(v);
    v += dpp_f32<DPP_QUAD_XOR2>(v);
    v += dpp_f32<DPP_HALF_MIRROR>(v);
    v += dpp_f32<DPP_ROW_MIRROR>(v);
    return v;
}

__device__ __forceinline__ float wave_sum_f32(float v) {
    for (int o = 32; o > 0; o >>= 1) v += __shfl_xor(v, o, 64);
    return v;
}
__device__ __forceinline__ double wave_sum_f64(double v) {
    for (int o = 32; o > 0; o >>= 1) v += __shfl_xor(v, o, 64);
    return v;
}
__device__ __forceinline__ float wave_max_f32(float v) {
    for (int o = 32; o > 0; o >>= 1) v = fmaxf(v, __shfl_xor(v, o, 64));
    return v;
}

__device__ __forceinline__ void q4k_unpack_scales(const uint8_t * scales, uint32_t sc[2], uint32_t mn[2]) {
    const uint32_t kmask1 = 0x3f3f3f3fu, kmask2 = 0x0f0f0f0fu, kmask3 = 0x03030303u;
    const uint32_t u0 = ((const uint32_t *) scales)[0], u1 = ((const uint32_t *) scales)[1], u2 = ((const uint32_t *) scales)[2];
    sc[0] = u0 & kmask1;
    sc[1] = (u2 & kmask2) | (((u0 >> 6) & kmask3) << 4);
    mn[0] = u1 & kmask1;
    mn[1] = ((u2 >> 4) & kmask2) | (((u1 >> 6) & kmask3) << 4);
}

__device__ __forceinline__ void q4k_unpack_scales_w(uint32_t u0, uint32_t u1, uint32_t u2, uint32_t sc[2], uint32_t mn[2]) {
    const uint32_t kmask1 = 0x3f3f3f3fu, kmask2 = 0x0f0f0f0fu, kmask3 = 0x03030303u;
    sc[0] = u0 & kmask1;
    sc[1] = (u2 & kmask2) | (((u0 >> 6) & kmask3) << 4);
    mn[0] = u1 & kmask1;
    mn[1] = ((u2 >> 4) & kmask2) | (((u1 >> 6) & kmask3) << 4);
}

__device__ __forceinline__ float dequant_elem(const char * row, int type, int64_t i) {
    switch (type) {
        case GGML_TYPE_F32:  return ((const float *) row)[i];
        case GGML_TYPE_F16:  return h2f(((const uint16_t *) row)[i]);
        case GGML_TYPE_BF16: return bf2f(((const uint16_t *) row)[i]);
        case GGML_TYPE_Q8_0: { const block_q8_0 * b = (const block_q8_0 *) row + i / 32; return b->qs[i % 32] * h2f(b->d); }
        case GGML_TYPE_Q4_0: {
            const block_q4_0 * b = (const block_q4_0 *) row + i / 32;
            const int j = (int) (i % 32);
            const int q = j < 16 ? (b->qs[j] & 0x0F) : (b->qs[j - 16] >> 4);
            return (q - 8) * h2f(b->d);
        }
        case GGML_TYPE_Q4_K: {
            const block_q4_K * b = (const block_q4_K *) row + i / 256;
            const int j = (int) (i % 256);
            const int sub = j / 32, l = j % 32;
            uint32_t sc[2], mn[2];
            q4k_unpack_scales(b->scales, sc, mn);
            const uint32_t s = (sc[sub >> 2] >> (8 * (sub & 3))) & 0xff, m = (mn[sub >> 2] >> (8 * (sub & 3))) & 0xff;
            const uint8_t qb = b->qs[(sub >> 1) * 32 + l];
            const int q = (sub & 1) ? (qb >> 4) : (qb & 0xF);
            const float d = h2f(b->d) * (float) s, mm = h2f(b->dmin) * (float) m;
            return d * (float) q - mm;
        }
        default: return NAN;
    }
}

__device__ __forceinline__ int dot4_i8(int a, int b, int c) { return __builtin_amdgcn_sdot4(a, b, c, false); }

__device__ __forceinline__ float q4k_q8k_block_dot(const block_q4_K * xb, const int8_t * q8, const int16_t * bsums, float d8) {
    uint32_t sc[2], mn[2];
    q4k_unpack_scales(xb->scales, sc, mn);
    const uint32_t * qs = (const uint32_t *) xb->qs;
    const int * y = (const int *) q8;
    int isum = 0, msum = 0;
#pragma unroll
    for (int j = 0; j < 4; j++) {
        int lo = 0, hi = 0;
#pragma unroll
        for (int t = 0; t < 8; t++) {
            const uint32_t q = qs[j * 8 + t];
            lo = dot4_i8((int) (q & 0x0F0F0F0Fu), y[j * 16 + t], lo);
            hi = dot4_i8((int) ((q >> 4) & 0x0F0F0F0Fu), y[j * 16 + 8 + t], hi);
        }
        const int s0 = (int) ((sc[j >> 1] >> (16 * (j & 1))) & 0xff), s1 = (int) ((sc[j >> 1] >> (16 * (j & 1) + 8)) & 0xff);
        const int m0 = (int) ((mn[j >> 1] >> (16 * (j & 1))) & 0xff), m1 = (int) ((mn[j >> 1] >> (16 * (j & 1) + 8)) & 0xff);
        isum += __mul24(s0, lo) + __mul24(s1, hi);
        msum += __mul24(m0, (int) bsums[4 * j] + (int) bsums[4 * j + 1]) + __mul24(m1, (int) bsums[4 * j + 2] + (int) bsums[4 * j + 3]);
    }
    const float d = h2f(xb->d) * d8, dmin = h2f(xb->dmin) * d8;
    return d * (float) isum - dmin * (float) msum;
}
```

moshi.cpp_amd/csrc/hip_kernels_fused.hip:

```cpp
#include "hip_common.h"
#include "hip_device.h"
#include "hip_mv_device.h"
#include <hip/hip_ext.h>
#include <stdlib.h>
#include <map>

struct x_src {
    int prologue;
    const float * x;
    const float * alpha;
    float scale;
    int64_t K;
};

__device__ __forceinline__ float x_value(const x_src & s, int64_t i) {
    switch (s.prologue) {
        case MV_RMSNORM:   return s.alpha[i] * (s.x[i] * s.scale);
        case MV_GATE_SILU: { const float l = s.x[i], r = s.x[s.K + i]; return (l / (1.0f + expf(-l))) * r; }
        default:           return s.x[i];
    }
}

__device__ float block_rms_scale(const float * x, int64_t K, float eps, double * sh) {
    double acc = 0;
// ... 1984 lines not shown
__global__ void __launch_bounds__(256) cross_attn_streams_kernel(xattn_args a) {
    extern __shared__ float xsm[];
    __shared__ float sh_f[4];
    __shared__ double sh_d[4];
    const int h = blockIdx.x, b = blockIdx.y;
    cross_attn_body(a, a.q + (int64_t) b * a.q_cs + (int64_t) h * a.D, a.k + (int64_t) b * a.k_nb3 + (int64_t) h * a.k_nb2,
                    a.v + (int64_t) b * a.v_nb3 + (int64_t) h * a.v_nb2, a.out + (int64_t) b * a.out_cs + (int64_t) h * a.D, xsm, sh_f, sh_d);
}
void k_cross_attn(hipStream_t s, const xattn_args & a) {
    GGML_ASSERT(a.D >= 1 && a.D <= 256 && a.Tc >= 1 && a.H >= 1 && a.B >= 1);
    const size_t smem = (size_t) ((a.D + a.Tc + 1) & ~1) * 4 + (size_t) (256 / a.D > 0 ? 256 / a.D : 1) * a.D * 8;
    GGML_ASSERT(smem <= 64 * 1024);
    if (a.B == 1) cross_attn_kernel<<<a.H, 256, smem, s>>>(a);
    else cross_attn_streams_kernel<<<dim3((unsigned) a.H, (unsigned) a.B), 256, smem, s>>>(a);
}

template <int TYPE, int NMAX>
__global__ void __launch_bounds__(64) embed_sum_kernel(embed_sum_args a) {
    const int64_t i = (int64_t) blockIdx.x * blockDim.x + threadIdx.x;
    if (i >= a.K) return;
    const int b = (int) blockIdx.y;
    int64_t r[NMAX];
    float sc[NMAX], v[NMAX];
#pragma unroll
    for (int t = 0; t < NMAX; t++) {
        const embed_src & e = a.src[t < a.n ? t : 0];
        r[t] = e.index[b];
        sc[t] = e.scale ? e.scale[b] : 1.f;
    }
    if (TYPE == GGML_TYPE_Q4_0 || TYPE == GGML_TYPE_Q8_0) {
        constexpr int BB = TYPE == GGML_TYPE_Q4_0 ? 18 : 34;
        const int64_t boff = (i >> 5) * BB;
        const int j = (int) (i & 31);
        const int64_t qoff = boff + 2 + (TYPE == GGML_TYPE_Q4_0 ? (j & 15) : j);
        uint16_t dh[NMAX]; uint8_t qb[NMAX];
#pragma unroll
        for (int t = 0; t < NMAX; t++) {
            const embed_src & e = a.src[t < a.n ? t : 0];
            const int64_t row = (r[t] < 0 || r[t] >= e.n_rows) ? 0 : r[t];
            const char * base = e.table + row * e.row_bytes;
            dh[t] = *(const uint16_t *) (base + boff);
            qb[t] = *(const uint8_t *) (base + qoff);
        }
        __builtin_amdgcn_sched_barrier(0);
#pragma unroll
        for (int t = 0; t < NMAX; t++) {
            if (TYPE == GGML_TYPE_Q4_0) { const int q = j < 16 ? (qb[t] & 0x0F) : (qb[t] >> 4); v[t] = (q - 8) * h2f(dh[t]); }
            else v[t] = (int8_t) qb[t] * h2f(dh[t]);
        }
    } else {
#pragma unroll
        for (int t = 0; t < NMAX; t++) {
            const embed_src & e = a.src[t < a.n ? t : 0];
            if (r[t] < 0 || r[t] >= e.n_rows) r[t] = 0;
            v[t] = dequant_elem(e.table + r[t] * e.row_bytes, TYPE >= 0 ? TYPE : e.type, i);
        }
    }
    float acc = 0.f;
#pragma unroll
    for (int t = 0; t < NMAX; t++) {
        if (t < a.n) {
            const float x = a.src[t].scale ? v[t] * sc[t] : v[t];
            acc = t == 0 ? x : acc + x;
        }
    }
    a.out[(int64_t) b * a.K + i] = acc;
}
void k_embed_sum(hipStream_t s, const embed_sum_args & a) {
    int type = a.n > 0 ? a.src[0].type : -1;
    for (int t = 1; t < a.n; t++) if (a.src[t].type != type) type = -1;
    const dim3 grid((unsigned) ((a.K + 63) / 64), (unsigned) (a.B > 1 ? a.B : 1));
#define EMBED_LAUNCH(T) do { if (a.n <= 8) embed_sum_kernel<T, 8><<<grid, 64, 0, s>>>(a); else if (a.n <= 24) embed_sum_kernel<T, 24><<<grid, 64, 0, s>>>(a); else embed_sum_kernel<T, EMBED_SUM_MAX><<<grid, 64, 0, s>>>(a); } while (0)
    switch (type) {
        case GGML_TYPE_Q4_0: EMBED_LAUNCH(GGML_TYPE_Q4_0); break;
        case GGML_TYPE_Q8_0: EMBED_LAUNCH(GGML_TYPE_Q8_0); break;
        case GGML_TYPE_F32:  EMBED_LAUNCH(GGML_TYPE_F32); break;
        case GGML_TYPE_BF16: EMBED_LAUNCH(GGML_TYPE_BF16); break;
        case GGML_TYPE_F16:  EMBED_LAUNCH(GGML_TYPE_F16); break;
        default:             EMBED_LAUNCH(-1); break;
    }
#undef EMBED_LAUNCH
}

#define VQ_CPW 4
__global__ void __launch_bounds__(256) vq_level_kernel(vq_level_args a) {
    __shared__ float sv[4];
    __shared__ int si[4];
    __shared__ int s_last;
    const int tid = threadIdx.x, lane = tid & 63, wave = tid >> 6;
    const int D = a.D;
    const int c0 = (blockIdx.x * 4 + wave) * VQ_CPW;
    f32x4 e[VQ_CPW];
#pragma unroll
    for (int u = 0; u < VQ_CPW; u++) {
        const int c = c0 + u < a.NC ? c0 + u : a.NC - 1;
        e[u] = *(const f32x4 *) (a.emb + (int64_t) c * a.emb_row_bytes + lane * 16);
    }
    float x[4];
#pragma unroll
    for (int j = 0; j < 4; j++) x[j] = *(const float *) (a.resid + (int64_t) (lane * 4 + j) * a.resid_stride);
    const float addc = a.add_c[0];
    float best = -INFINITY; int bi = -1;
#pragma unroll
    for (int u = 0; u < VQ_CPW; u++) {
        double acc = 0;
#pragma unroll
        for (int j = 0; j < 4; j++) { const float d = e[u][j] - x[j]; acc += (double) (d * d); }
        acc = wave_allsum_f64(acc);
        const int c = c0 + u;
        if (c < a.NC) {
            const float v = a.num[c] / ((float) acc + addc);
            if (v >= best) { best = v; bi = c; }
        }
    }
    if (lane == 0) { sv[wave] = best; si[wave] = bi; }
    __syncthreads();
    if (tid == 0) {
        for (int w = 1; w < 4; w++) if (sv[w] > best || (sv[w] == best && si[w] > bi)) { best = sv[w]; bi = si[w]; }
        xchg_agent_wait(a.cand_val + blockIdx.x, best); xchg_agent_wait(a.cand_idx + blockIdx.x, bi);
        const unsigned ticket = atomicAdd(a.counter, 1u);
        s_last = ticket == gridDim.x - 1;
    }
    __syncthreads();
    if (!s_last) return;
    best = -INFINITY; bi = -1;
    if (tid < (int) gridDim.x) { best = ld_agent(a.cand_val + tid); bi = ld_agent(a.cand_idx + tid); }
    __shared__ float mv[256];
    __shared__ int mi[256];
    mv[tid] = best; mi[tid] = bi;
    __syncthreads();
    for (int st = 128; st > 0; st >>= 1) {
        if (tid < st) {
            const float v = mv[tid + st]; const int j = mi[tid + st];
            if (v > mv[tid] || (v == mv[tid] && j > mi[tid])) { mv[tid] = v; mi[tid] = j; }
        }
        __syncthreads();
    }
    const int code = mi[0] < 0 ? 0 : mi[0];
    if (tid == 0) { *a.idx_i = code; *a.idx_f = (float) code; *a.counter = 0u; }
    if (a.resid_out) {
        for (int j = tid; j < D; j += 256) {
            const float q = *(const float *) (a.emb + (int64_t) code * a.emb_row_bytes + j * 4);
            a.resid_out[j] = *(const float *) (a.resid + (int64_t) j * a.resid_stride) - q;
        }
    }
}
void k_vq_level(hipStream_t s, const vq_level_args & a) {
    GGML_ASSERT(a.D == 256);
    const int grid = (a.NC + 4 * VQ_CPW - 1) / (4 * VQ_CPW);
    GGML_ASSERT(grid <= 256);
    vq_level_kernel<<<grid, 256, 0, s>>>(a);
}

#if defined(SMP_LOG)
__device__ unsigned long long g_smp_log[16];
#define SMP_STAMP(i) do { if (threadIdx.x == 0) { unsigned long long t_; asm volatile("s_memrealtime %0\n\ts_waitcnt lgkmcnt(0)" : "=s"(t_) :: "memory"); g_smp_log[i] = t_; } } while (0)
#else
#define SMP_STAMP(i) do {} while (0)
#endif
#define SMP_BIN_MAX 64
template <int SMP_THREADS, int SMP_NPT>
__device__ __forceinline__ void sample_topk_body(const sample_args & a) {
    constexpr int NW = SMP_THREADS / 64;
    __shared__ float shf[NW];
    __shared__ double shd[NW];
    __shared__ int shi[NW];
// ... 264 lines not shown
```

moshi.cpp_amd/csrc/hip_kernels_generic.hip:

```cpp
#include "hip_common.h"
#include "hip_device.h"
#include <type_traits>

#define BLOCK 256

static inline int nblocks(int64_t n, int bs = BLOCK) { return (int) ((n + bs - 1) / bs); }

__global__ void binary_kernel(int op, tdesc dst, tdesc a, tdesc b, int64_t n) {
    const int64_t i = (int64_t) blockIdx.x * blockDim.x + threadIdx.x;
    if (i >= n) return;
    int64_t i0, i1, i2, i3;
    unravel(dst, i, i0, i1, i2, i3);
    const float x = *(const float *) at(a, i0, i1, i2, i3);
    const float y = *(const float *) at(b, wrap(i0, b.ne[0]), wrap(i1, b.ne[1]), wrap(i2, b.ne[2]), wrap(i3, b.ne[3]));
    float r;
    switch (op) {
        case GGML_OP_ADD: r = x + y; break;
        case GGML_OP_SUB: r = x - y; break;
        case GGML_OP_MUL: r = x * y; break;
        default:          r = x / y; break;
    }
    *(float *) at(dst, i0, i1, i2, i3) = r;
}
void k_binary(hipStream_t s, int op, tdesc dst, tdesc a, tdesc b) {
// ... 651 lines not shown
        y = conv_at(t);
        if (has2) { y = y + pv[keep + t]; y2 = conv_at(t + keep); }
    }
    pv[t] = y;
    if (has2) pv[t + keep] = y2;
    const float yo = bias ? y + bias[oc] : y;
    *(float *) at(out, t, oc, 0, 0) = yo;
    if (sc.panel) conv_scatter_elem(sc, t, oc, yo);
}
void k_convtr_finish(hipStream_t s, tdesc out, float * prev, const float * bias, const void * ws, int K, int OC, int L, int s0, int nsplit, const conv_scatter * sc) {
    GGML_ASSERT(K - s0 <= L * s0 && "tail longer than the new window is not expected on this path");
    const int64_t n = (int64_t) L * s0 * OC;
    conv_scatter scv;
    memset(&scv, 0, sizeof(scv));
    if (sc) scv = *sc;
    const int nb = nblocks(n) + (scv.panel && scv.TP > 0 ? 1 : 0);
    switch (nsplit) {
        case 1:  convtr_finish_kernel<1><<<nb, BLOCK, 0, s>>>(out, prev, bias, (const double *) ws, K, OC, L, s0, nsplit, scv); break;
        case 2:  convtr_finish_kernel<2><<<nb, BLOCK, 0, s>>>(out, prev, bias, (const double *) ws, K, OC, L, s0, nsplit, scv); break;
        case 4:  convtr_finish_kernel<4><<<nb, BLOCK, 0, s>>>(out, prev, bias, (const double *) ws, K, OC, L, s0, nsplit, scv); break;
        case 8:  convtr_finish_kernel<8><<<nb, BLOCK, 0, s>>>(out, prev, bias, (const double *) ws, K, OC, L, s0, nsplit, scv); break;
        case 16: convtr_finish_kernel<16><<<nb, BLOCK, 0, s>>>(out, prev, bias, (const double *) ws, K, OC, L, s0, nsplit, scv); break;
        default: convtr_finish_kernel<0><<<nb, BLOCK, 0, s>>>(out, prev, bias, (const double *) ws, K, OC, L, s0, nsplit, scv); break;
    }
}

__global__ void dw_convtr_frame_kernel(float * out, float * prev, const float * bias, const char * x, int64_t x_cs, const char * w, int64_t w_cs, int K, int PT, int C, int64_t out_cs, int64_t out_ks) {
    const int c = blockIdx.x * blockDim.x + threadIdx.x;
    if (c >= C) return;
    const float xv = *(const float *) (x + (int64_t) c * x_cs);
    const float * wc = (const float *) (w + (int64_t) c * w_cs);
    float * pv = prev + (int64_t) c * K;
    const int keep = K - PT;
    float y[16];
    for (int k = 0; k < K; k++) { y[k] = xv * wc[k]; if (k < PT) y[k] = y[k] + pv[keep + k]; }
    for (int k = 0; k < K; k++) pv[k] = y[k];
    for (int k = 0; k < keep; k++) out[(int64_t) c * out_cs + k * out_ks] = bias ? y[k] + bias[c] : y[k];
}
void k_dw_convtr_frame(hipStream_t s, float * out, float * prev, const float * bias, const char * x, int64_t x_cs, const char * w, int64_t w_cs, int K, int PT, int C, int64_t out_cs, int64_t out_ks) {
    GGML_ASSERT(K <= 16);
    dw_convtr_frame_kernel<<<(C + 63) / 64, 64, 0, s>>>(out, prev, bias, x, x_cs, w, w_cs, K, PT, C, out_cs < 0 ? K - PT : out_cs, out_ks);
}

__global__ void stream_im2col_kernel(tdesc dst, const float * prev, int TP, tdesc x, int Kw, int s0, int pre_elu, int64_t n) {
    const int64_t i = (int64_t) blockIdx.x * blockDim.x + threadIdx.x;
    if (i >= n) return;
    const uint32_t CK = (uint32_t) dst.ne[0];
    const uint32_t ol = (uint32_t) i / CK, c = (uint32_t) i - ol * CK;
    const uint32_t ci = c / (uint32_t) Kw, k = c - ci * (uint32_t) Kw;
    const int l = (int) (ol * (uint32_t) s0 + k);
    float v;
    if (l < TP) v = prev[l + (int64_t) ci * TP];
    else { v = *(const float *) (x.data + (int64_t) (l - TP) * x.nb[0] + (int64_t) ci * x.nb[1]); if (pre_elu) v = v > 0.f ? v : expm1f(v); }
    ((uint16_t *) dst.data)[i] = f2h(v);
}
void k_stream_im2col(hipStream_t s, tdesc dst, const float * prev, int TP, tdesc x, int Kw, int s0, int pre_elu) {
    const int64_t n = dst.ne[0] * dst.ne[1];
    GGML_ASSERT(dst.type == GGML_TYPE_F16 && x.type == GGML_TYPE_F32 && dst.nb[1] == dst.ne[0] * 2);
    if (n) stream_im2col_kernel<<<nblocks(n), BLOCK, 0, s>>>(dst, prev, TP, x, Kw, s0, pre_elu, n);
}
__global__ void conv_tail_kernel(float * prev, int TP, tdesc x, int pre_elu) {
    const int ci = blockIdx.x * blockDim.x + threadIdx.x;
    if (ci >= (int) x.ne[1]) return;
    const int L = (int) x.ne[0];
    float v[32];
#pragma unroll
    for (int j = 0; j < 32; j++) {
        if (j < TP) {
            const int l = L + j;
            if (l < TP) v[j] = prev[l + (int64_t) ci * TP];
            else { float t = *(const float *) (x.data + (int64_t) (l - TP) * x.nb[0] + (int64_t) ci * x.nb[1]); v[j] = pre_elu ? (t > 0.f ? t : expm1f(t)) : t; }
        }
    }
#pragma unroll
    for (int j = 0; j < 32; j++) if (j < TP) prev[j + (int64_t) ci * TP] = v[j];
}
void k_conv_tail(hipStream_t s, float * prev, int TP, tdesc x, int pre_elu) {
    GGML_ASSERT(TP <= 32);
    if (TP > 0) conv_tail_kernel<<<(int) ((x.ne[1] + 63) / 64), 64, 0, s>>>(prev, TP, x, pre_elu);
}

__global__ void timestep_embedding_kernel(tdesc dst, tdesc ts, int dim, int max_period, const float * addend, int addend_n) {
    const int64_t i = blockIdx.x;
    const int half = dim / 2;
    float * e = (float *) at(dst, 0, i, 0, 0);
    float t = *(const float *) at(ts, i, 0, 0, 0);
    if (addend) t = t + addend[addend_n == 1 ? 0 : i];
    for (int j = threadIdx.x; j < half; j += blockDim.x) {
        const float lf = (float) log((double) max_period);
        const float freq = (float) exp((double) (-lf * j / half));
        const float arg = t * freq;
        e[j] = (float) cos((double) arg);
        e[j + half] = (float) sin((double) arg);
    }
    if (threadIdx.x == 0 && (dim & 1)) e[2 * half] = 0.f;
}
void k_timestep_embedding(hipStream_t s, tdesc dst, tdesc ts, int dim, int max_period, const float * addend, int addend_n) {
    if (ts.ne[0]) timestep_embedding_kernel<<<(int) ts.ne[0], 64, 0, s>>>(dst, ts, dim, max_period, addend, addend_n);
}

static int vec_dot_type(int t) {
    switch (t) {
        case GGML_TYPE_F32: return GGML_TYPE_F32;
        case GGML_TYPE_F16: return GGML_TYPE_F16;
        case GGML_TYPE_BF16: return GGML_TYPE_BF16;
        case GGML_TYPE_Q4_0: case GGML_TYPE_Q8_0: return GGML_TYPE_Q8_0;
        case GGML_TYPE_Q4_K: return GGML_TYPE_Q8_K;
        default: GGML_ABORT("mul_mat: unsupported weight type %s", ggml_type_name((enum ggml_type) t));
    }
}

size_t k_mul_mat_ws_size(const struct ggml_tensor * a, const struct ggml_tensor * b) {
    const int vt = vec_dot_type(a->type);
    return ggml_row_size((enum ggml_type) vt, b->ne[0]) * (size_t) (b->ne[1] * b->ne[2] * b->ne[3]) + 256;
}

__global__ void convert_rows_kernel(tdesc b, int vt, char * ws, int64_t row_bytes) {
    __shared__ float shf[BLOCK / 64];
    int64_t i1, i2, i3;
    row_coords(b, blockIdx.x, i1, i2, i3);
    char * out = ws + (int64_t) blockIdx.x * row_bytes;
    const int64_t K = b.ne[0];
    if (vt == GGML_TYPE_F32 || vt == GGML_TYPE_F16 || vt == GGML_TYPE_BF16) {
        const int es = elem_size(vt);
        for (int64_t i = threadIdx.x; i < K; i += blockDim.x) st_from_f32(out + i * es, vt, ld_as_f32(at(b, i, i1, i2, i3), b.type));
        return;
    }
    if (vt == GGML_TYPE_Q8_0) {
        for (int64_t base = 0; base < K; base += blockDim.x) {
            const int64_t i = base + threadIdx.x;
            const float v = i < K ? *(const float *) at(b, i, i1, i2, i3) : 0.f;
            float amax = fabsf(v);
            for (int o = 16; o > 0; o >>= 1) amax = fmaxf(amax, __shfl_xor(amax, o, 64));
            const float d = amax / 127.f;
            const float id = d ? 1.0f / d : 0.0f;
            if (i < K) {
                block_q8_0 * blk = (block_q8_0 *) out + i / 32;
                blk->qs[i % 32] = (int8_t) roundf(v * id);
                if (i % 32 == 0) blk->d = f2h(d);
            }
        }
        return;
    }
    for (int64_t base = 0; base < K; base += 256) {
        const int tid = threadIdx.x;
        const float v = *(const float *) at(b, base + tid, i1, i2, i3);
        float amax = fabsf(v); int ai = tid;
        for (int o = 32; o > 0; o >>= 1) {
            const float oa = __shfl_xor(amax, o, 64); const int oi = __shfl_xor(ai, o, 64);
            if (oa > amax || (oa == amax && oi < ai)) { amax = oa; ai = oi; }
        }
        __shared__ float s_amax[4]; __shared__ int s_ai[4]; __shared__ float s_vals[256]; __shared__ int s_q[256];
        __syncthreads();
        s_vals[tid] = v;
        if ((tid & 63) == 0) { s_amax[tid >> 6] = amax; s_ai[tid >> 6] = ai; }
        __syncthreads();
        float bm = s_amax[0]; int bi = s_ai[0];
        for (int w = 1; w < 4; w++) if (s_amax[w] > bm || (s_amax[w] == bm && s_ai[w] < bi)) { bm = s_amax[w]; bi = s_ai[w]; }
        block_q8_K * blk = (block_q8_K *) out + base / 256;
        int q = 0;
        float dd = 0.f;
        if (bm != 0.f) {
            const float iscale = -127.f / s_vals[bi];
            q = nearest_int_dev(iscale * v);
            q = q < 127 ? q : 127;
            dd = 1.f / iscale;
        }
        blk->qs[tid] = (int8_t) q;
        s_q[tid] = q;
        __syncthreads();
        if (tid < 16) { int sum = 0; for (int l = 0; l < 16; l++) sum += s_q[tid * 16 + l]; blk->bsums[tid] = (int16_t) sum; }
        if (tid == 0) blk->d = dd;
        (void) shf;
    }
}

#define MM_TAIL_LDS 4096
__device__ __forceinline__ void mm_tail_update(const mm_epilogue & e) {
// ... 335 lines not shown
```

moshi.cpp_amd/csrc/moshi_hot.cpp:

```cpp
#include "moshi_hot.h"
#include "delay_ring.h"
#include "gguf.h"
#include "ggml-cpu.h"

#include <dlfcn.h>
#include <math.h>
#include <stdlib.h>
#include <string.h>

#include <deque>
#include <functional>
#include <map>
#include <set>
#include <string>
#include <vector>

typedef struct ggml_tensor * T;

namespace {

struct Rng {
    uint64_t s;
    explicit Rng(uint64_t seed) : s(seed) {}
    uint64_t next() { uint64_t z = (s += 0x9E3779B97F4A7C15ull); z = (z ^ (z >> 30)) * 0xBF58476D1CE4E5B9ull; z = (z ^ (z >> 27)) * 0x94D049BB133111EBull; return z ^ (z >> 31); }
// ... 435 lines not shown
    s.compute_scratch();
}
void init_cross_expand(Builder & s, const Transformer & tr, Layer & L, T condition_cross, T k_dst, T v_dst) {
    const int H = tr.heads, dim = (int) L.cross_in->ne[1] / 3;
    T kv = linear_view(s, L.cross_in, dim, 2 * dim, condition_cross);
    auto half = [&](size_t off) {
        T t = ggml_view_3d(s, kv, kv->ne[0] / 2, kv->ne[1], kv->ne[2], kv->nb[1], kv->nb[2], off);
        t = ggml_cont(s, t);
        t = ggml_reshape_4d(s, t, t->ne[0] / H, H, t->ne[1], t->ne[2]);
        return ggml_permute(s, t, 0, 2, 1, 3);
    };
    s.expand(ggml_cpy(s, half(0), k_dst));
    s.expand(ggml_cpy(s, half(kv->nb[1] / 2), v_dst));
}

T transformer_layer(Builder & c, const Transformer & tr, Layer & L, int wi, T indices, T x, T attn_bias, const Rot * rot, bool per_step_views) {
    T nx = apply_norm(c, L.norm1, x);
    T update = attention(c, tr, L, wi, indices, nx, attn_bias, rot, per_step_views);
    if (L.layer_scale_1) update = ggml_mul(c, update, L.layer_scale_1);
    x = ggml_add(c, x, update);
    if (L.cross_in) {
        nx = apply_norm(c, L.norm_cross, x);
        x = ggml_add(c, x, cross_attention(c, tr, L, nx));
    }
    nx = apply_norm(c, L.norm2, x);
    if (L.gate_in.empty()) {
        T h = linear(c, L.linear1, nx);
        h = ggml_gelu(c, h);
        update = linear(c, L.linear2, h);
    } else {
        T gx = nx;
        if (per_step_views) gx = ggml_view_3d(c, nx, nx->ne[0], 1, nx->ne[2], nx->nb[1], nx->nb[2], 0);
        update = gating(c, L.gate_in[(size_t) wi], L.gate_out[(size_t) wi], gx);
        if (x->ne[1] > 1 || x->ne[2] > 1) update = ggml_reshape_3d(c, update, update->ne[0], x->ne[1], x->ne[2]);
    }
    if (L.layer_scale_2) update = ggml_mul(c, update, L.layer_scale_2);
    return ggml_add(c, x, update);
}

T transformer_graph_build(Builder & g, Transformer & tr, T x) {
    const int Tn = (int) x->ne[1];
    create_bias_pattern(g.be, tr, Tn);
    tr.g_bias = g.tensor(GGML_TYPE_F32, tr.capacity, Tn);
    Rot rot;
    if (tr.max_period) {
        tr.g_offset = g.tensor(GGML_TYPE_F32, 1);
        rot = timestep_embedding(g, Tn, tr.dim / tr.heads, tr.g_offset, tr.max_period);
    }
    tr.g_indices = g.tensor(GGML_TYPE_I32, Tn);
    for (auto & L : tr.layers) x = transformer_layer(g, tr, L, 0, tr.g_indices, x, tr.g_bias, tr.max_period ? &rot : nullptr, false);
    return x;
}

T transformer_graph_build_slots(Builder & g, Transformer & tr, T x) {
    const int64_t B = x->ne[2], C = tr.capacity, D = tr.dim / tr.heads;
    create_bias_pattern(g.be, tr, 1);
    tr.g_bias = g.tensor(GGML_TYPE_F32, C, 1, 1, B);
    Rot rot;
    if (tr.max_period) {
        tr.g_offset = g.tensor(GGML_TYPE_F32, B);
        T table = ggml_timestep_embedding(g, tr.g_offset, (int) D, tr.max_period);
        rot.rotr = ggml_view_4d(g, table, D / 2, 1, 1, B, table->nb[1], table->nb[1], table->nb[1], 0);
        rot.roti = ggml_view_4d(g, table, D / 2, 1, 1, B, table->nb[1], table->nb[1], table->nb[1], table->nb[0] * (size_t) (D / 2));
    }
    tr.g_indices = g.tensor(GGML_TYPE_I32, 1, 1, B);
    for (auto & L : tr.layers) x = transformer_layer(g, tr, L, 0, tr.g_indices, x, tr.g_bias, tr.max_period ? &rot : nullptr, false);
    return x;
}

void transformer_graph_step_slots(Builder & scratch, Transformer & tr, const std::vector<int64_t> & pos) {
    const int B = (int) pos.size(), C = tr.capacity;
    std::vector<float> off((size_t) B);
    std::vector<int32_t> idx((size_t) B);
    for (int b = 0; b < B; b++) {
        T bias = bias_pattern_index(scratch, tr, 1, (int) pos[(size_t) b]);
        scratch.expand(ggml_cpy(scratch, bias, ggml_view_1d(scratch, tr.g_bias, C, (size_t) b * (size_t) C * 4)));
        off[(size_t) b] = (float) pos[(size_t) b];
        idx[(size_t) b] = (int32_t) (pos[(size_t) b] % C);
    }
    if (tr.g_offset) ggml_backend_tensor_set(tr.g_offset, off.data(), 0, off.size() * 4);
    ggml_backend_tensor_set(tr.g_indices, idx.data(), 0, idx.size() * 4);
}

void transformer_graph_step_at(Builder & scratch, Transformer & tr, int Tn, int offset) {
    T bias = bias_pattern_index(scratch, tr, Tn, offset);
    scratch.expand(ggml_cpy(scratch, bias, tr.g_bias));
    if (tr.g_offset) { const float f = (float) offset; ggml_backend_tensor_set(tr.g_offset, &f, 0, 4); }
    std::vector<int32_t> idx((size_t) Tn);
    for (int i = 0; i < Tn; i++) idx[(size_t) i] = (offset + i) % tr.capacity;
    ggml_backend_tensor_set(tr.g_indices, idx.data(), 0, idx.size() * 4);
}
void transformer_graph_step(Builder & scratch, Transformer & tr, int Tn) {
    transformer_graph_step_at(scratch, tr, Tn, tr.offset);
    tr.offset += Tn;
}

T transformer_inline(Builder & g, Transformer & tr, T x, T mask_override = nullptr) {
    const int Tn = (int) x->ne[1];
    const int offset = tr.offset;
    T attn_bias = mask_override ? mask_override : bias_pattern_index(g, tr, Tn, offset);
    Rot rot;
    if (tr.max_period) rot = timestep_embedding(g, Tn, tr.dim / tr.heads, g.f32((float) offset), tr.max_period);
    std::vector<int32_t> idx((size_t) Tn);
    for (int i = 0; i < Tn; i++) idx[(size_t) i] = (offset + i) % tr.capacity;
    T indices = g.i32s(idx);
    const bool multi = tr.layers[0].in_proj.size() > 1;
    const int wi = !multi ? 0 : tr.schedule.empty() ? offset : tr.schedule[(size_t) offset];
    for (auto & L : tr.layers) x = transformer_layer(g, tr, L, wi, indices, x, attn_bias, tr.max_period ? &rot : nullptr, multi);
    tr.offset += Tn;
    return x;
}

T sample_token(Builder & g, T logits, float temp, int top_k, int site = -1) {
    if (!(temp > 0.f)) return ggml_argmax(g, logits);
    T probs = ggml_soft_max(g, ggml_scale(g, logits, 1.f / temp));
    const int k = (int) probs->ne[0] < top_k ? (int) probs->ne[0] : top_k;
    T indices = ggml_argsort_top_k(g, probs, k);
    T rows = ggml_permute(g, probs, 1, 0, 2, 3);
    rows = ggml_get_rows(g, ggml_cont(g, rows), indices);
    probs = ggml_permute(g, rows, 1, 0, 2, 3);
    T in2 = ggml_reshape_2d(g, probs, probs->ne[0], probs->ne[1] * probs->ne[2] * probs->ne[3]);
    T q = ggml_div(g, in2, g.exponential(in2->ne[0], in2->ne[1], 1.f, site));
    T next = ggml_argmax(g, q);
    next = ggml_reshape_4d(g, next, next->ne[0], probs->ne[1], probs->ne[2], probs->ne[3]);
    T irows = ggml_permute(g, indices, 1, 0, 2, 3);
    return ggml_get_rows(g, ggml_cont(g, irows), next);
}

T sample_tokens_streams(Builder & g, T logits, float temp, int top_k, T inv_temp, int site) {
    const int64_t n = logits->ne[0], B = ggml_nelements(logits) / n;
    T l2 = ggml_reshape_2d(g, logits, n, B);
    if (!(temp > 0.f)) return ggml_argmax(g, l2);
    T probs = ggml_soft_max(g, inv_temp ? ggml_mul(g, l2, inv_temp) : ggml_scale(g, l2, 1.f / temp));
    const int k = (int) n < top_k ? (int) n : top_k;
    T indices = ggml_cont(g, ggml_argsort_top_k(g, probs, k));
    T rows = ggml_cont(g, ggml_permute(g, ggml_reshape_3d(g, probs, n, 1, B), 1, 0, 2, 3));
    T picked = ggml_get_rows(g, rows, indices);
    T in2 = ggml_reshape_2d(g, picked, k, B);
    T q = ggml_div(g, in2, g.exponential(k, B, 1.f, site));
    T next = ggml_argmax(g, q);
    T irows = ggml_cont(g, ggml_permute(g, ggml_reshape_3d(g, indices, k, 1, B), 1, 0, 2, 3));
    T tok = ggml_get_rows(g, irows, ggml_reshape_2d(g, next, 1, B));
    return ggml_reshape_1d(g, tok, B);
}

struct Conv { int cin, cout, k, stride; T w = nullptr, b = nullptr; T prev = nullptr; };
struct ConvTr { int cin, cout, k, stride, groups; T w = nullptr, b = nullptr; T prev = nullptr; };
struct ResBlock { Conv block1, block3; };

T streaming_conv(Builder & g, Conv & cv, T x) {
    const int TP = cv.k - cv.stride;
    x = ggml_concat(g, cv.prev, x, 0);
    T tail = ggml_view_3d(g, x, TP, x->ne[1], x->ne[2], x->nb[1], x->nb[2], x->nb[0] * (size_t) (x->ne[0] - TP));
    g.expand(ggml_cpy(g, tail, cv.prev));
    T y = ggml_conv_1d(g, cv.w, x, cv.stride, 0, 1);
    if (cv.b) y = ggml_add(g, y, cv.b);
    return y;
}
T stateless_conv(Builder & g, Conv & cv, T x) {
    T y = ggml_conv_1d(g, cv.w, x, 1, 0, 1);
    if (cv.b) y = ggml_add(g, y, cv.b);
    return y;
}
T streaming_conv_transpose(Builder & g, ConvTr & ct, T x) {
    const int PT = ct.k - ct.stride;
    T y = nullptr;
    if (ct.groups == 1) y = ggml_conv_transpose_1d(g, ct.w, x, ct.stride, 0, 1);
    else {
        for (int i = 0; i < ct.w->ne[0]; i++) {
// ... 55 lines not shown
    d = ggml_add(g, d, g.f32(1.f));
    d = ggml_div(g, g.fill(d->ne, 1.f), d);
    return ggml_argmax(g, d);
}
T rvq_encode(Builder & g, Rvq & rvq, T x, T * latent = nullptr) {
    x = ggml_conv_1d(g, rvq.input_proj, x, 1, 0, 1);
    if (latent) *latent = x;
    T residual = x, out = nullptr;
    for (int i = 0; i < rvq.n_q; i++) {
        T xp = ggml_permute(g, residual, 1, 0, 2, 3);
        T idx = codebook_encode(g, rvq.layers[(size_t) i], xp);
        T quant = vq_decode(g, rvq.layers[(size_t) i], idx);
        idx = ggml_cast(g, idx, GGML_TYPE_F32);
        residual = ggml_sub(g, residual, quant);
        out = out ? ggml_concat(g, out, idx, 2) : idx;
    }
    return ggml_permute(g, out, 0, 2, 1, 3);
}

}

enum class ModelKind { single, lockstep, slots };
struct moshi_hot_model {
    moshi_hot_config cfg;
    ggml_backend_t be;
    ggml_backend_t be_codec = nullptr; bool own_codec_be = false;
    Weights * W = nullptr;
    struct ggml_context * st_ctx = nullptr; ggml_backend_buffer_t st_buf = nullptr;
    std::vector<std::pair<T, std::vector<uint8_t>>> st_init;
    Builder * scratch = nullptr, * scratch_codec = nullptr;

    Transformer temporal, depth;
    Norm out_norm;
    T text_emb = nullptr, text_linear = nullptr;
    std::vector<T> emb, depformer_in, depformer_emb, linears;
    T depformer_text_emb = nullptr;
    std::vector<T> extra_heads;
    T heads_out = nullptr; std::vector<float> last_heads;
    T text_out1 = nullptr, text_out2 = nullptr, dep_text_out1 = nullptr, dep_text_out2 = nullptr;
    T dep_text_low_rank = nullptr; std::vector<T> depformer_emb_low_rank;
    T cond_sum = nullptr, cond_cross = nullptr;
    T emb_right_idx = nullptr, emb_right_scale = nullptr, dep_right_idx = nullptr, dep_right_scale = nullptr;
    moshi_hot_text_hook_t text_hook = nullptr; void * text_hook_user = nullptr;
    T transformer_out = nullptr;
    T tok_state = nullptr;
    struct InFlight { bool done = false; bool steady = false; int ok = 0; std::vector<int32_t> raw; int32_t out_text = 0; std::vector<int32_t> out_audio; ggml_backend_event_t ev = nullptr; };
    std::deque<InFlight> inflight;
    std::vector<ggml_backend_event_t> ev_pool;
    int tok_state_for = -1;
    Builder * g_temporal = nullptr; std::vector<T> emb_idx, emb_scale; T sampler_out = nullptr, text_logits = nullptr, g_transformer_out = nullptr, g_transformer_in = nullptr, g_stack_out = nullptr;
    Builder * g_depth = nullptr; T dep_text_idx = nullptr, dep_text_scale = nullptr, dep_tokens = nullptr; std::vector<T> dep_logits;
    std::vector<Builder *> g_shard_step, g_shard_import; Builder * g_shard_begin = nullptr;
    T shard_msg = nullptr, shard_tout = nullptr, shard_tokens = nullptr;
    std::vector<T> shard_text_idx, shard_text_scale;
    moshi_hot_depth_hook_t depth_hook = nullptr; void * depth_hook_user = nullptr;
    moshi_hot_bcast_t shard_bcast = nullptr; void * shard_bcast_user = nullptr;
    void * rccl_lib = nullptr, * rccl_comm = nullptr;
    int64_t shard_hops = 0;
    int (*rccl_broadcast)(const void *, void *, size_t, int, int, void *, void *) = nullptr;
    int (*rccl_comm_destroy)(void *) = nullptr;
    int (*rccl_all_reduce)(const void *, void *, size_t, int, int, void *, void *) = nullptr;
    moshi_hot_allreduce_t tp_allreduce = nullptr; void * tp_allreduce_user = nullptr;
    int64_t tp_reductions = 0;
    Transformer temporal_tp; T tp_x = nullptr, tp_msg = nullptr; std::vector<Builder *> g_tp;
    bool tp_frame = false; T tp_in = nullptr; Builder * g_tp_pre = nullptr, * g_tp_import = nullptr, * g_tp_post = nullptr; int64_t tp_frames = 0;
    DelayProtocol proto; DelayRing ring;
    struct Column { DelayRing ring; int64_t pos = 0; bool open = false, held = false; };
    int n_streams = 1; ModelKind kind = ModelKind::single; std::vector<Column> cols;
    struct Sampling { moshi_hot_sampling s; bool seeded = false; };
    std::vector<Sampling> sampling; bool any_seeded = false, sampling_dirty = true;
    T inv_temp_text = nullptr, inv_temp = nullptr;

    Rvq rvq_first, rvq_rest;
    ConvTr upsample; Conv downsample;
    Transformer dec_tr, enc_tr;
    std::vector<Conv> dec_convs; std::vector<ConvTr> dec_convtrs; std::vector<ResBlock> dec_res;
    std::vector<Conv> enc_convs; std::vector<ResBlock> enc_res;
    Builder * g_dec = nullptr; T dec_codes = nullptr, dec_frame = nullptr; int dec_T = 0;
    Builder * g_enc = nullptr; T enc_frame = nullptr, enc_codes = nullptr; int enc_T = 0;
    T enc_latent[2] = { nullptr, nullptr };

    std::vector<int32_t> tokens_tmp;
    std::vector<int32_t> pipe_codes, pipe_tokens; bool pipe_have_codes = false, pipe_have_tokens = false; float pipe_vad = 0.f;
    bool temporal_staged = false;
    std::function<void()> after_temporal_launch;
    int32_t last_text = 0; std::vector<int32_t> last_audio;
    bool timing = false; double phase_us[4] = { 0, 0, 0, 0 }; int64_t phase_n[4] = { 0, 0, 0, 0 };
};

#define STREAMS_REFUSE(ret) do { if (m->n_streams > 1) return ret; } while (0)

namespace {

T state(moshi_hot_model * m, enum ggml_type type, int64_t n0, int64_t n1 = 1, int64_t n2 = 1) {
    T t = ggml_new_tensor_3d(m->st_ctx, type, n0, n1, n2);
    m->st_init.push_back({ t, std::vector<uint8_t>(ggml_nbytes(t), 0) });
    return t;
}
T state4(moshi_hot_model * m, enum ggml_type type, int64_t n0, int64_t n1, int64_t n2, int64_t n3) {
    T t = ggml_new_tensor_4d(m->st_ctx, type, n0, n1, n2, n3);
    m->st_init.push_back({ t, std::vector<uint8_t>(ggml_nbytes(t), 0) });
    return t;
}

bool owns_step(const moshi_hot_config & c, int k) { return c.dep_shard_world <= 1 || k % c.dep_shard_world == c.dep_shard_rank; }

void make_transformer(moshi_hot_model * m, Transformer & tr, const std::string & name, int dim, int heads, int n_layers, int ffn_hidden,
                      int capacity, int max_period, int n_weight_sets, bool mimi_style, enum ggml_type wtype, int cross_len = 0, bool norms_only = false) {
    Weights & W = *m->W;
    tr.dim = dim; tr.heads = heads; tr.capacity = capacity; tr.max_period = max_period;
    tr.layers.resize((size_t) n_layers);
    const float s_in = 1.f / sqrtf((float) dim);
    const float upd = m->cfg.update_scale > 0.f ? m->cfg.update_scale : 1.f;
    auto qgen = [](float sd) { return [sd](T t, Rng & r, std::vector<uint8_t> & o) { gen_quant(t, r, o, sd); }; };
    auto ones = [](T t, Rng &, std::vector<uint8_t> & o) { gen_const(t, 1.f, o); };
    auto zeros = [](T t, Rng &, std::vector<uint8_t> & o) { gen_const(t, 0.f, o); };
    for (int l = 0; l < n_layers; l++) {
        Layer & L = tr.layers[(size_t) l];
        const std::string p = name + ".layers." + std::to_string(l) + ".";
        if (mimi_style) {
            L.norm1 = { false, 1e-5f, W.add(p + "norm1.weight", GGML_TYPE_F32, dim, 1, 1, ones), W.add(p + "norm1.bias", GGML_TYPE_F32, dim, 1, 1, zeros) };
            L.norm2 = { false, 1e-5f, W.add(p + "norm2.weight", GGML_TYPE_F32, dim, 1, 1, ones), W.add(p + "norm2.bias", GGML_TYPE_F32, dim, 1, 1, zeros) };
            L.layer_scale_1 = W.add(p + "layer_scale_1.scale", GGML_TYPE_F32, dim, 1, 1, [](T t, Rng &, std::vector<uint8_t> & o) { gen_const(t, 0.5f, o); });
            L.layer_scale_2 = W.add(p + "layer_scale_2.scale", GGML_TYPE_F32, dim, 1, 1, [](T t, Rng &, std::vector<uint8_t> & o) { gen_const(t, 0.5f, o); });
            L.linear1 = W.add(p + "linear1.weight", wtype, dim, ffn_hidden, 1, qgen(s_in));
            L.linear2 = W.add(p + "linear2.weight", wtype, ffn_hidden, dim, 1, qgen(1.f / sqrtf((float) ffn_hidden)));
        } else {
            L.norm1 = { true, 1e-8f, W.add(p + "norm1.alpha", GGML_TYPE_F32, dim, 1, 1, ones), nullptr };
            L.norm2 = { true, 1e-8f, W.add(p + "norm2.alpha", GGML_TYPE_F32, dim, 1, 1, ones), nullptr };
        }
        if (norms_only) continue;
        for (int w = 0; w < n_weight_sets; w++) {
            const std::string ws = n_weight_sets > 1 ? "." + std::to_string(w) : "";
            if (n_weight_sets > 1 && !owns_step(m->cfg, w)) {
                L.in_proj.push_back(nullptr); L.out_proj.push_back(nullptr);
                if (!mimi_style) { L.gate_in.push_back(nullptr); L.gate_out.push_back(nullptr); }
                continue;
            }
            L.in_proj.push_back(W.add(p + "self_attn.in_projs" + ws + ".weight", wtype, dim, 3 * dim, 1, qgen(s_in)));
            L.out_proj.push_back(W.add(p + "self_attn.out_projs" + ws + ".weight", wtype, dim, dim, 1, qgen(s_in * upd)));
            if (!mimi_style) {
                L.gate_in.push_back(W.add(p + "gating" + ws + ".linear_in.weight", wtype, dim, 2 * ffn_hidden, 1, qgen(s_in)));
                L.gate_out.push_back(W.add(p + "gating" + ws + ".linear_out.weight", wtype, ffn_hidden, dim, 1, qgen(upd / sqrtf((float) ffn_hidden))));
            }
        }
        if (m->n_streams > 1 && !mimi_style) {
            L.kcache = state4(m, GGML_TYPE_BF16, dim / heads, capacity, heads, m->n_streams);
            L.vcache = state4(m, GGML_TYPE_BF16, dim / heads, capacity, heads, m->n_streams);
        } else {
            L.kcache = state(m, GGML_TYPE_BF16, dim / heads, capacity, heads);
            L.vcache = state(m, GGML_TYPE_BF16, dim / heads, capacity, heads);
        }
        if (cross_len > 0) {
            L.norm_cross = { false, 0.0f, W.add(p + "norm_cross.weight", GGML_TYPE_F32, dim, 1, 1, ones),
                             W.add(p + "norm_cross.bias", GGML_TYPE_F32, dim, 1, 1, [](T t, Rng & r, std::vector<uint8_t> & o) { gen_normal(t, r, o, 0.02f); }) };
            L.cross_in = W.add(p + "cross_attention.in_projs.0.weight", wtype, dim, 3 * dim, 1, qgen(s_in));
            L.cross_out = W.add(p + "cross_attention.out_projs.0.weight", wtype, dim, dim, 1, qgen(s_in * upd));
            if (m->n_streams > 1) {
                L.k_cross = state4(m, GGML_TYPE_F32, dim / heads, cross_len, heads, m->n_streams);
                L.v_cross = state4(m, GGML_TYPE_F32, dim / heads, cross_len, heads, m->n_streams);
            } else {
                L.k_cross = state(m, GGML_TYPE_F32, dim / heads, cross_len, heads);
                L.v_cross = state(m, GGML_TYPE_F32, dim / heads, cross_len, heads);
            }
        }
    }
// ... 1 lines not shown

Conv make_conv(moshi_hot_model * m, const std::string & name, int cin, int cout, int k, int stride, bool bias, bool stateful) {
    Weights & W = *m->W;
    Conv c = { cin, cout, k, stride };
    const float sd = 1.f / sqrtf((float) (cin * k));
    c.w = W.add(name + ".weight", GGML_TYPE_F16, k, cin, cout, [sd](T t, Rng & r, std::vector<uint8_t> & o) { gen_normal(t, r, o, sd); });
    if (bias) c.b = W.add(name + ".bias", GGML_TYPE_F32, 1, cout, 1, [](T t, Rng & r, std::vector<uint8_t> & o) { gen_normal(t, r, o, 0.02f); });
    if (stateful && k - stride > 0) c.prev = state(m, GGML_TYPE_F32, k - stride, cin);
    return c;
}
ConvTr make_convtr(moshi_hot_model * m, const std::string & name, int cin, int cout, int k, int stride, int groups, bool bias, int64_t in_len) {
    Weights & W = *m->W;
    ConvTr c = { cin, cout, k, stride, groups };
    const float sd = 1.f / sqrtf((float) (cin / groups));
    c.w = W.add(name + ".weight", GGML_TYPE_F32, k, cout / groups, cin, [sd](T t, Rng & r, std::vector<uint8_t> & o) { gen_normal(t, r, o, sd); });
    if (bias) c.b = W.add(name + ".bias", GGML_TYPE_F32, 1, cout, 1, [](T t, Rng & r, std::vector<uint8_t> & o) { gen_normal(t, r, o, 0.02f); });
    c.prev = state(m, GGML_TYPE_F32, (in_len - 1) * stride + k, cout);
    return c;
}
ResBlock make_res(moshi_hot_model * m, const std::string & name, int dim) {
    ResBlock rb;
    rb.block1 = make_conv(m, name + ".block.1.conv", dim, dim / 2, 3, 1, true, true);
    rb.block3 = make_conv(m, name + ".block.3.conv", dim / 2, dim, 1, 1, true, false);
    return rb;
}
void make_rvq(moshi_hot_model * m, Rvq & rvq, const std::string & name, int n_layers, int card) {
    Weights & W = *m->W;
    rvq.n_q = n_layers;
    for (int i = 0; i < n_layers; i++) {
        Codebook cb;
        cb.embedding = W.add(name + ".vq.layers." + std::to_string(i) + "._codebook.embedding", GGML_TYPE_F32, 256, card, 1,
                             [](T t, Rng & r, std::vector<uint8_t> & o) { gen_normal(t, r, o, 1.f); });
        rvq.layers.push_back(cb);
    }
    rvq.input_proj = W.add(name + ".input_proj.weight", GGML_TYPE_F16, 1, 512, 256, [](T t, Rng & r, std::vector<uint8_t> & o) { gen_normal(t, r, o, 1.f / sqrtf(512.f)); });
    rvq.output_proj = W.add(name + ".output_proj.weight", GGML_TYPE_F16, 1, 256, 512, [](T t, Rng & r, std::vector<uint8_t> & o) { gen_normal(t, r, o, 1.f / 16.f); });
}

T build_input_embedding(moshi_hot_model * m, Builder & g) {
    const moshi_hot_config & c = m->cfg;
    const int B = m->n_streams;
    auto embed = [&](T table) {
        const int i = (int) m->emb_idx.size();
        T idx = m->tok_state && i <= c.dep_q ? ggml_view_1d(g, m->tok_state, 1, (size_t) i * 4) : g.tensor(GGML_TYPE_I32, B), scale = B > 1 ? g.tensor(GGML_TYPE_F32, 1, B) : g.tensor(GGML_TYPE_F32, 1);
        m->emb_idx.push_back(idx); m->emb_scale.push_back(scale);
        return ggml_mul(g, ggml_get_rows(g, table, idx), scale);
    };
    T input;
    if (c.demux_second_stream) {
        T left = g.tensor(GGML_TYPE_I32, B);
        m->emb_idx.push_back(left); m->emb_scale.push_back(nullptr);
        m->emb_right_idx = g.tensor(GGML_TYPE_I32, B); m->emb_right_scale = B > 1 ? g.tensor(GGML_TYPE_F32, 1, B) : g.tensor(GGML_TYPE_F32, 1);
        T l = ggml_get_rows(g, m->text_emb, left), r = ggml_get_rows(g, m->text_emb, m->emb_right_idx);
        T ry = linear(g, m->text_out2, r), ly = linear(g, m->text_out1, l);
        input = ggml_add(g, ly, ggml_mul(g, ry, m->emb_right_scale));
    } else input = embed(m->text_emb);
    for (int k = 0; k < c.n_q; k++) input = ggml_add(g, input, embed(m->emb[(size_t) k]));
    if (c.condition_sum) input = ggml_add(g, m->cond_sum, input);
    if (B > 1) input = ggml_reshape_3d(g, input, input->ne[0], 1, B);
    m->g_transformer_in = input;
    return input;
}
void build_temporal_graph(moshi_hot_model * m) {
    const moshi_hot_config & c = m->cfg;
    m->g_temporal = new Builder(m->be, 256);
    Builder & g = *m->g_temporal;
    T input = build_input_embedding(m, g);
    T x = m->kind == ModelKind::slots ? transformer_graph_build_slots(g, m->temporal, input) : transformer_graph_build(g, m->temporal, input);
    m->g_stack_out = x;
    x = apply_norm(g, m->out_norm, x);
    m->g_transformer_out = x;
    m->text_logits = linear(g, m->text_linear, x);
    g.expand(ggml_cpy(g, x, m->transformer_out));
    if (m->n_streams > 1 && c.temp_text > 0.f) { m->inv_temp_text = g.tensor(GGML_TYPE_F32, 1, m->n_streams); m->sampling_dirty = true; }
    m->sampler_out = m->n_streams > 1 ? sample_tokens_streams(g, m->text_logits, c.temp_text, c.top_k_text, m->inv_temp_text, 0) : sample_token(g, m->text_logits, c.temp_text, c.top_k_text, 0);
    g.expand(m->sampler_out);
    if (m->tok_state) g.expand(ggml_cpy(g, ggml_reshape_1d(g, m->sampler_out, 1), ggml_view_1d(g, m->tok_state, 1, 0)));
    if (m->heads_out) for (size_t k = 0; k < m->extra_heads.size(); k++) {
        T sm = ggml_soft_max(g, linear(g, m->extra_heads[k], x));
        T row = ggml_view_3d(g, m->heads_out, m->heads_out->ne[0], 1, m->n_streams, m->heads_out->nb[1], m->heads_out->nb[2], k * m->heads_out->nb[1]);
        g.expand(ggml_cpy(g, sm, row));
    }
    g.alloc();
}

void build_depth_graph(moshi_hot_model * m) {
    const moshi_hot_config & c = m->cfg;
    m->g_depth = new Builder(m->be, 256);
    Builder & g = *m->g_depth;
    m->dep_text_idx = g.tensor(GGML_TYPE_I32, 1);
    if (c.chain_depth) {
        GGML_ASSERT(!c.demux_second_stream && !c.delay_steps && m->tok_state && m->sampler_out->type == GGML_TYPE_I32 && ggml_nelements(m->sampler_out) == 1);
        m->dep_text_idx = ggml_view_1d(g, m->tok_state, 1, 0);
    }
    T last;
    if (c.demux_second_stream) {
        m->dep_right_idx = g.tensor(GGML_TYPE_I32, 1); m->dep_right_scale = g.tensor(GGML_TYPE_F32, 1);
        T l = ggml_get_rows(g, m->depformer_text_emb, m->dep_text_idx), r = ggml_get_rows(g, m->depformer_text_emb, m->dep_right_idx);
        T ry = linear(g, m->dep_text_out2, r), ly = linear(g, m->dep_text_out1, l);
        last = ggml_add(g, ly, ggml_mul(g, ry, m->dep_right_scale));
    } else {
        m->dep_text_scale = g.tensor(GGML_TYPE_F32, 1);
        last = ggml_mul(g, ggml_get_rows(g, m->depformer_text_emb, m->dep_text_idx), m->dep_text_scale);
        if (m->dep_text_low_rank) last = linear(g, m->dep_text_low_rank, last);
    }
    T tokens = m->tok_state ? ggml_view_1d(g, m->tok_state, c.dep_q, 4) : g.tensor(GGML_TYPE_I32, c.dep_q);
    T view = nullptr, next = nullptr;
    for (int k = 0; k < c.dep_q; k++) {
        if (k > 0) {
            last = ggml_get_rows(g, m->depformer_emb[(size_t) (k - 1)], next);
            if (!m->depformer_emb_low_rank.empty()) last = linear(g, m->depformer_emb_low_rank[(size_t) (k - 1)], last);
        }
        const int in_index = c.dep_schedule_len ? c.dep_schedule[k] : k;
        T din = linear(g, m->depformer_in[(size_t) in_index], m->transformer_out);
        last = ggml_cast(g, last, GGML_TYPE_F32);
        din = ggml_add(g, din, last);
        T dout = transformer_inline(g, m->depth, din);
        T logits = linear(g, m->linears[(size_t) k], dout);
        m->dep_logits.push_back(logits);
        next = sample_token(g, logits, c.temp, c.top_k, 1 + k);
        view = k == 0 ? ggml_view_1d(g, tokens, 1, 0) : ggml_view_1d(g, view, 1, 4);
        g.expand(ggml_cpy(g, next, view));
    }
    m->dep_tokens = ggml_view_1d(g, view, tokens->ne[0], (size_t) (-(int64_t) (c.dep_q - 1) * 4));
    g.expand(m->dep_tokens);
    g.alloc();
}

void build_depth_graph_streams(moshi_hot_model * m) {
    const moshi_hot_config & c = m->cfg;
    const int B = m->n_streams;
    m->g_depth = new Builder(m->be, 256);
    Builder & g = *m->g_depth;
    m->dep_text_idx = g.tensor(GGML_TYPE_I32, B);
    T last;
    if (c.demux_second_stream) {
        m->dep_right_idx = g.tensor(GGML_TYPE_I32, B); m->dep_right_scale = g.tensor(GGML_TYPE_F32, 1, B);
        T l = ggml_get_rows(g, m->depformer_text_emb, m->dep_text_idx), r = ggml_get_rows(g, m->depformer_text_emb, m->dep_right_idx);
        T ry = linear(g, m->dep_text_out2, r), ly = linear(g, m->dep_text_out1, l);
        last = ggml_add(g, ly, ggml_mul(g, ry, m->dep_right_scale));
    } else {
        m->dep_text_scale = g.tensor(GGML_TYPE_F32, 1, B);
        last = ggml_mul(g, ggml_get_rows(g, m->depformer_text_emb, m->dep_text_idx), m->dep_text_scale);
        if (m->dep_text_low_rank) last = linear(g, m->dep_text_low_rank, last);
    }
    T tokens = g.tensor(GGML_TYPE_I32, (int64_t) B * c.dep_q);
    if (c.temp > 0.f) { m->inv_temp = g.tensor(GGML_TYPE_F32, 1, B); m->sampling_dirty = true; }
    T view = nullptr, next = nullptr;
    for (int k = 0; k < c.dep_q; k++) {
        if (k > 0) {
            last = ggml_get_rows(g, m->depformer_emb[(size_t) (k - 1)], next);
            if (!m->depformer_emb_low_rank.empty()) last = linear(g, m->depformer_emb_low_rank[(size_t) (k - 1)], last);
        }
        const int in_index = c.dep_schedule_len ? c.dep_schedule[k] : k;
        T din = linear(g, m->depformer_in[(size_t) in_index], m->transformer_out);
        last = ggml_cast(g, last, GGML_TYPE_F32);
        din = ggml_add(g, din, ggml_reshape_3d(g, last, last->ne[0], 1, B));
        T dout = transformer_inline(g, m->depth, din);
        T logits = linear(g, m->linears[(size_t) k], dout);
        m->dep_logits.push_back(logits);
        next = sample_tokens_streams(g, logits, c.temp, c.top_k, m->inv_temp, 1 + k);
        view = k == 0 ? ggml_view_1d(g, tokens, B, 0) : ggml_view_1d(g, view, B, (size_t) B * 4);
        g.expand(ggml_cpy(g, next, view));
    }
    m->dep_tokens = ggml_view_1d(g, view, tokens->ne[0], (size_t) (-(int64_t) (c.dep_q - 1) * B * 4));
    g.expand(m->dep_tokens);
    g.alloc();
}

void build_decode_graph(moshi_hot_model * m) {
    const moshi_hot_config & c = m->cfg;
    m->g_dec = new Builder(m->be_codec, 256);
    Builder & g = *m->g_dec;
    T codes = ggml_new_tensor_2d(g, GGML_TYPE_I32, 1, c.mimi_n_q);
    m->dec_codes = codes;
    const int64_t B = codes->ne[2], K = codes->ne[1], Tn = codes->ne[0];
    T first = ggml_view_3d(g, codes, Tn, 1, B, codes->nb[1], codes->nb[2], 0);
    T emb = rvq_decode(g, m->rvq_first, first);
    if (K > 1) {
        T rest = ggml_view_3d(g, codes, Tn, K - 1, B, codes->nb[1], codes->nb[2], codes->nb[1] * 1);
        emb = ggml_add(g, emb, rvq_decode(g, m->rvq_rest, rest));
    }
    emb = streaming_conv_transpose(g, m->upsample, emb);
    m->dec_T = (int) emb->ne[0];
    T x = ggml_cont(g, ggml_transpose(g, emb));
// ... 277 lines not shown
            for (int k = 0; k < n_sets; k++)
                m->depformer_in.push_back(!owns_step(c, k) ? nullptr : W.add("lm.depformer_in." + std::to_string(k) + ".weight", lt, c.dim, c.dep_dim, 1, qgen(1.f / sqrtf((float) c.dim))));
            for (int k = 0; k < c.dep_q; k++) {
                m->linears.push_back(!owns_step(c, k) ? nullptr : W.add("lm.linears." + std::to_string(k) + ".weight", lt, c.dep_dim, c.card, 1, qgen(1.f / sqrtf((float) c.dep_dim))));
                if (k > 0) {
                    W.part = 4;
                    m->depformer_emb.push_back(!owns_step(c, k) ? nullptr : W.add("lm.depformer_emb." + std::to_string(k - 1) + ".weight", fit(et, E), E, c.card + 1, 1, qgen(1.f)));
                    W.part = 1;
                    if (c.depformer_low_rank)
                        m->depformer_emb_low_rank.push_back(W.add("lm.depformer_emb." + std::to_string(k - 1) + ".low_rank.weight", fit(lt, E), E, c.dep_dim, 1, qgen(1.f / sqrtf((float) E))));
                }
            }
            W.part = 4;
            if (owns_step(c, 0)) m->depformer_text_emb = W.add("lm.depformer_text_emb.weight", fit(et, E), E, c.text_card + 1, 1, qgen(1.f));
            W.part = 1;
            if (c.demux_second_stream) {
                m->dep_text_out1 = W.add("lm.depformer_text_emb.out1.weight", fit(lt, E), E, c.dep_dim, 1, qgen(1.f / sqrtf((float) E)));
                m->dep_text_out2 = W.add("lm.depformer_text_emb.out2.weight", fit(lt, E), E, c.dep_dim, 1, qgen(1.f / sqrtf((float) E)));
            } else if (c.depformer_low_rank)
                m->dep_text_low_rank = W.add("lm.depformer_text_emb.low_rank.weight", fit(lt, E), E, c.dep_dim, 1, qgen(1.f / sqrtf((float) E)));
            make_transformer(m, m->depth, "lm.depformer", c.dep_dim, c.dep_heads, c.dep_layers, c.dep_ffn_hidden, c.dep_context ? c.dep_context : c.dep_schedule_len, 0, n_sets, false, lt);
            for (int i = 0; i < c.dep_schedule_len; i++) m->depth.schedule.push_back(c.dep_schedule[i]);
            if (c.dep_shard_world >= 1) {
                m->shard_msg = state(m, GGML_TYPE_F32, (int64_t) c.dep_layers * c.dep_dim + 8);
                m->shard_tout = state(m, GGML_TYPE_F32, (int64_t) c.dim + 8);
                m->shard_tokens = state(m, GGML_TYPE_I32, c.dep_q);
            }
        }
        DelayProtocol & p = m->proto;
        p.n_q = c.n_q; p.dep_q = c.dep_q; p.io_dep_q = c.personaplex ? 8 : c.dep_q;
        p.delays.assign(c.delays, c.delays + p.cols());
        for (int d : p.delays) if (d > p.max_delay) p.max_delay = d;
        p.rows = p.max_delay + 2 + (c.personaplex ? 1 : 0);
        p.initial.assign((size_t) p.cols(), c.card); p.initial[0] = c.text_card;
        DelayRing fresh; fresh.p = &p; fresh.reset();
        if (m->n_streams > 1) m->cols.assign((size_t) m->n_streams, { fresh, 0, kind == ModelKind::lockstep }); else m->ring = fresh;
    }
    if (c.enable_mimi_decoder || c.enable_mimi_encoder) {
        W.part = c.enable_mimi_decoder ? 3 : 2;
        make_rvq(m, m->rvq_first, "mimi.quantizer.rvq_first", 1, c.mimi_codebook_size);
        make_rvq(m, m->rvq_rest, "mimi.quantizer.rvq_rest", c.mimi_n_q > 1 ? c.mimi_n_q - 1 : 0, c.mimi_codebook_size);
    }
    if (c.enable_mimi_decoder) {
        W.part = 3;
        m->upsample = make_convtr(m, "mimi.upsample.convtr", 512, 512, 4, 2, 512, false, 1);
        make_transformer(m, m->dec_tr, "mimi.decoder_transformer.transformer", 512, 8, 8, 2048, 250, 10000, 1, true, GGML_TYPE_F32);
        m->dec_convs.push_back(make_conv(m, "mimi.decoder.model.0.conv", 512, 1024, 7, 1, true, true));
        const int ch[5] = { 1024, 512, 256, 128, 64 }, ks[4] = { 16, 12, 10, 8 }, st[4] = { 8, 6, 5, 4 };
        int64_t len = 2;
        for (int i = 0; i < 4; i++) {
            m->dec_convtrs.push_back(make_convtr(m, "mimi.decoder.model." + std::to_string(2 + 3 * i) + ".convtr", ch[i], ch[i + 1], ks[i], st[i], 1, true, len));
            len = len * st[i];
            m->dec_res.push_back(make_res(m, "mimi.decoder.model." + std::to_string(3 + 3 * i), ch[i + 1]));
        }
        m->dec_convs.push_back(make_conv(m, "mimi.decoder.model.14.conv", 64, 1, 3, 1, true, true));
    }
    if (c.enable_mimi_encoder) {
        W.part = 2;
        m->enc_convs.push_back(make_conv(m, "mimi.encoder.model.0.conv", 1, 64, 7, 1, true, true));
        const int ch[5] = { 64, 128, 256, 512, 1024 }, ks[4] = { 8, 10, 12, 16 }, st[4] = { 4, 5, 6, 8 };
        for (int i = 0; i < 4; i++) {
            m->enc_res.push_back(make_res(m, "mimi.encoder.model." + std::to_string(1 + 3 * i), ch[i]));
            m->enc_convs.push_back(make_conv(m, "mimi.encoder.model." + std::to_string(3 + 3 * i) + ".conv", ch[i], ch[i + 1], ks[i], st[i], true, true));
        }
        m->enc_convs.push_back(make_conv(m, "mimi.encoder.model.14.conv", 1024, 512, 3, 1, true, true));
        make_transformer(m, m->enc_tr, "mimi.encoder_transformer.transformer", 512, 8, 8, 2048, 250, 10000, 1, true, GGML_TYPE_F32);
        m->downsample = make_conv(m, "mimi.downsample.conv", 512, 512, 4, 2, false, true);
    }
    W.load();
    m->st_buf = ggml_backend_alloc_ctx_tensors(m->st_ctx, backend);
    GGML_ASSERT(m->st_buf);
    for (auto & s : m->st_init) ggml_backend_tensor_set(s.first, s.second.data(), 0, s.second.size());
    m->st_init.clear();
    m->tokens_tmp.resize((size_t) (c.n_q + 1 + 32));
    m->pipe_codes.resize((size_t) (c.n_q + 1 + 32)); m->pipe_tokens.resize((size_t) (c.n_q + 1 + 32));
    ggml_backend_synchronize(backend);
    return m;
}

extern "C" void moshi_hot_free(moshi_hot_model_t * m) {
    if (!m) return;
    ggml_backend_synchronize(m->be);
    moshi_hot_depth_shard_rccl_free(m);
    for (auto & f : m->inflight) if (f.ev) ggml_backend_event_free(f.ev);
    for (auto e : m->ev_pool) ggml_backend_event_free(e);
    if (m->own_codec_be) ggml_backend_synchronize(m->be_codec);
    delete m->g_temporal; delete m->g_depth; delete m->g_dec; delete m->g_enc; if (m->scratch_codec != m->scratch) delete m->scratch_codec; delete m->scratch; delete m->g_shard_begin;
    for (auto * b : m->g_shard_step) delete b;
    for (auto * b : m->g_shard_import) delete b;
    for (auto * b : m->g_tp) delete b;
    delete m->g_tp_pre; delete m->g_tp_import; delete m->g_tp_post;
    if (m->st_buf) ggml_backend_buffer_free(m->st_buf);
    ggml_free(m->st_ctx);
    delete m->W;
    if (m->own_codec_be) ggml_backend_free(m->be_codec);
    delete m;
}

namespace {
struct PhaseTimer {
    moshi_hot_model * m; int phase; int64_t t0;
    ggml_backend_t be() const { return phase == 0 || phase == 3 ? m->be_codec : m->be; }
    PhaseTimer(moshi_hot_model * m_, int p) : m(m_), phase(p), t0(0) { if (m->timing) { ggml_backend_synchronize(be()); t0 = ggml_time_us(); } }
    ~PhaseTimer() { if (m->timing) { ggml_backend_synchronize(be()); m->phase_us[phase] += (double) (ggml_time_us() - t0); m->phase_n[phase]++; } }
};
}

namespace {
void mimi_decode_launch(moshi_hot_model * m, const int32_t * codes) {
    if (!m->g_dec) build_decode_graph(m);
    ggml_backend_tensor_set(m->dec_codes, codes, 0, ggml_nbytes(m->dec_codes));
    transformer_graph_step(*m->scratch_codec, m->dec_tr, m->dec_T);
    m->scratch_codec->compute_scratch();
    m->g_dec->compute();
}
void mimi_decode_finish(moshi_hot_model * m, float * pcm) {
    if (pcm) ggml_backend_tensor_get(m->dec_frame, pcm, 0, ggml_nbytes(m->dec_frame));
    else { float tmp; ggml_backend_tensor_get(m->dec_frame, &tmp, 0, 4); }
}
void mimi_encode_launch(moshi_hot_model * m, const float * pcm) {
    if (!m->g_enc) build_encode_graph(m);
    ggml_backend_tensor_set(m->enc_frame, pcm, 0, ggml_nbytes(m->enc_frame));
    transformer_graph_step(*m->scratch_codec, m->enc_tr, m->enc_T);
    m->scratch_codec->compute_scratch();
    m->g_enc->compute();
}
void mimi_encode_finish(moshi_hot_model * m, int32_t * codes) { ggml_backend_tensor_get(m->enc_codes, codes, 0, ggml_nbytes(m->enc_codes)); }
}

extern "C" void moshi_hot_mimi_decode(moshi_hot_model_t * m, const int32_t * codes, float * pcm) { STREAMS_REFUSE();
    PhaseTimer pt(m, 3);
    mimi_decode_launch(m, codes);
    mimi_decode_finish(m, pcm);
}
extern "C" void moshi_hot_mimi_encode(moshi_hot_model_t * m, const float * pcm, int32_t * codes) { STREAMS_REFUSE();
    PhaseTimer pt(m, 0);
    mimi_encode_launch(m, pcm);
    mimi_encode_finish(m, codes);
}

namespace {
void demux_set(const moshi_hot_config & c, int32_t input, T left, T right, T right_scale) {
    if (input < 0) input = 0;
    const int32_t n = c.text_card + 1;
    int32_t l = input % n, r = input / n - 1;
    const float sc = r < 0 ? 0.f : 1.f;
    if (r < 0) r = 0;
    ggml_backend_tensor_set(left, &l, 0, 4);
    ggml_backend_tensor_set(right, &r, 0, 4);
    ggml_backend_tensor_set(right_scale, &sc, 0, 4);
}
void demux_set_columns(const moshi_hot_config & c, const std::vector<int32_t> & inputs, T left, T right, T right_scale) {
    const int32_t n = c.text_card + 1;
    std::vector<int32_t> l(inputs.size()), r(inputs.size()); std::vector<float> sc(inputs.size());
    for (size_t b = 0; b < inputs.size(); b++) {
        const int32_t input = inputs[b] < 0 ? 0 : inputs[b];
        l[b] = input % n; r[b] = input / n - 1;
        sc[b] = r[b] < 0 ? 0.f : 1.f;
        if (r[b] < 0) r[b] = 0;
    }
    ggml_backend_tensor_set(left, l.data(), 0, l.size() * 4);
    ggml_backend_tensor_set(right, r.data(), 0, r.size() * 4);
    ggml_backend_tensor_set(right_scale, sc.data(), 0, sc.size() * 4);
}
void depth_step(moshi_hot_model * m, int32_t text_token, std::vector<int32_t> & audio) {
    PhaseTimer pt(m, 2);
    if (!m->g_depth) build_depth_graph(m);
    if (m->cfg.demux_second_stream) demux_set(m->cfg, text_token, m->dep_text_idx, m->dep_right_idx, m->dep_right_scale);
    else {
        int32_t id = text_token; const float sc = id == -1 ? 0.f : 1.f;
        if (id < 0) id = 0;
        if (!m->cfg.chain_depth) ggml_backend_tensor_set(m->dep_text_idx, &id, 0, 4);
        ggml_backend_tensor_set(m->dep_text_scale, &sc, 0, 4);
    }
    if (m->any_seeded) stage_sampling(m);
    m->g_depth->compute();
    if (m->cfg.chain_depth && !m->temporal_staged) {
        transformer_graph_step(*m->scratch, m->temporal, 1);
        m->scratch->compute_scratch();
        m->temporal_staged = true;
    }
    ggml_backend_tensor_get(m->dep_tokens, audio.data(), 0, audio.size() * 4);
}
void unstage_temporal(moshi_hot_model * m) { if (m->temporal_staged) { m->temporal.offset -= 1; m->temporal_staged = false; } }
}

namespace {
void build_tp_segment(moshi_hot_model * m, int i) {
    const moshi_hot_config & c = m->cfg;
    Transformer & tp = m->temporal_tp;
    const int Lc = c.num_layers;
    Builder * b = new Builder(m->be, 32);
    Builder & g = *b;
    T x = m->tp_x;
    if (i > 0) { x = ggml_add(g, m->tp_x, m->tp_msg); g.expand(ggml_cpy(g, x, m->tp_x)); }
    if (i < 2 * Lc) {
        Layer & L = tp.layers[(size_t) (i / 2)];
        T part;
        if ((i & 1) == 0) {
            T nx = apply_norm(g, L.norm1, x);
            Rot rot;
            if (tp.max_period) rot = timestep_embedding(g, 1, tp.dim / tp.heads, tp.g_offset, tp.max_period);
            part = attention(g, tp, L, 0, tp.g_indices, nx, tp.g_bias, tp.max_period ? &rot : nullptr, false);
        } else {
            T nx = apply_norm(g, L.norm2, x);
            part = gating(g, L.gate_in[0], L.gate_out[0], nx);
        }
        g.expand(ggml_cpy(g, part, m->tp_msg));
    }
    g.alloc();
    if ((int) m->g_tp.size() <= i) m->g_tp.resize((size_t) i + 1, nullptr);
    m->g_tp[(size_t) i] = b;
}
}

extern "C" void * moshi_hot_tp_msg(moshi_hot_model_t * m, int64_t * n) { STREAMS_REFUSE(nullptr); GGML_ASSERT(m->tp_msg); if (n) *n = ggml_nelements(m->tp_msg); return m->tp_msg->data; }
extern "C" void moshi_hot_tp_begin(moshi_hot_model_t * m, const float * x) { STREAMS_REFUSE();
    GGML_ASSERT(m->tp_x);
    ggml_backend_tensor_set(m->tp_x, x, 0, (size_t) m->cfg.dim * 4);
    transformer_graph_step(*m->scratch, m->temporal_tp, 1);
    m->scratch->compute_scratch();
}
extern "C" void moshi_hot_tp_segment(moshi_hot_model_t * m, int i) { STREAMS_REFUSE();
    GGML_ASSERT(i >= 0 && i <= 2 * m->cfg.num_layers);
    if ((int) m->g_tp.size() <= i || !m->g_tp[(size_t) i]) build_tp_segment(m, i);
    m->g_tp[(size_t) i]->compute();
}
extern "C" void moshi_hot_tp_msg_read(moshi_hot_model_t * m, float * out) { STREAMS_REFUSE(); GGML_ASSERT(m->tp_msg); ggml_backend_tensor_get(m->tp_msg, out, 0, ggml_nbytes(m->tp_msg)); }
extern "C" void moshi_hot_tp_msg_write(moshi_hot_model_t * m, const float * in) { STREAMS_REFUSE(); GGML_ASSERT(m->tp_msg); ggml_backend_tensor_set(m->tp_msg, in, 0, ggml_nbytes(m->tp_msg)); }
extern "C" void moshi_hot_tp_end(moshi_hot_model_t * m, float * out) { STREAMS_REFUSE(); ggml_backend_tensor_get(m->tp_x, out, 0, (size_t) m->cfg.dim * 4); }
extern "C" void moshi_hot_tp_set_transport(moshi_hot_model_t * m, moshi_hot_allreduce_t fn, void * user) { STREAMS_REFUSE(); m->tp_allreduce = fn; m->tp_allreduce_user = user; }
extern "C" int64_t moshi_hot_tp_reductions(moshi_hot_model_t * m) { return m->tp_reductions; }
namespace {
void tp_run_segments(moshi_hot_model * m) {
    const moshi_hot_config & c = m->cfg;
    const int last = 2 * c.num_layers;
    for (int i = 0; i <= last; i++) {
        moshi_hot_tp_segment(m, i);
        if (i == last || (c.tp_world <= 1 && !m->rccl_comm && !m->tp_allreduce)) continue;
        m->tp_reductions++;
        const int64_t n = ggml_nelements(m->tp_msg);
        if (m->tp_allreduce) { m->tp_allreduce(m->tp_allreduce_user, (float *) m->tp_msg->data, n); continue; }
        GGML_ASSERT(m->rccl_comm && "moshi_hot tensor-parallel stack: no transport (moshi_hot_depth_shard_rccl_init or moshi_hot_tp_set_transport first)");
        const int rc = m->rccl_all_reduce(m->tp_msg->data, m->tp_msg->data, (size_t) n,  7,  0, m->rccl_comm, ggml_backend_mi355x_get_stream(m->be));
        GGML_ASSERT(rc == 0 && "ncclAllReduce failed");
    }
}
void tp_broadcast_in(moshi_hot_model * m) {
    const moshi_hot_config & c = m->cfg;
    if (c.tp_world <= 1 && !m->rccl_comm && !m->shard_bcast) return;
    const size_t bytes = ggml_nbytes(m->tp_in);
    if (m->shard_bcast) { m->shard_bcast(m->shard_bcast_user, m->tp_in->data, (int64_t) bytes, 0); return; }
    GGML_ASSERT(m->rccl_comm && "moshi_hot tensor-parallel frame: no transport");
    const int rc = m->rccl_broadcast(m->tp_in->data, m->tp_in->data, bytes,  1, 0, m->rccl_comm, ggml_backend_mi355x_get_stream(m->be));
    GGML_ASSERT(rc == 0 && "ncclBroadcast failed");
}
void tp_stack_from_in(moshi_hot_model * m) {
    const moshi_hot_config & c = m->cfg;
    if (!m->g_tp_import) {
        m->g_tp_import = new Builder(m->be, 8);
        Builder & g = *m->g_tp_import;
        g.expand(ggml_cpy(g, ggml_view_1d(g, m->tp_in, c.dim, 0), m->tp_x));
        g.alloc();
    }
// ... 221 lines not shown
    if (!init || !m->rccl_broadcast || !m->rccl_comm_destroy || !m->rccl_all_reduce) return -2;
    if (ggml_backend_dev_type(ggml_backend_get_device(m->be)) != GGML_BACKEND_DEVICE_TYPE_GPU) return -3;
    nccl_id id;
    memcpy(id.internal, id128, 128);
    m->rccl_lib = lib;
    ggml_backend_mi355x_make_current(m->be);
    if (m->rccl_comm) { ggml_backend_synchronize(m->be); m->rccl_comm_destroy(m->rccl_comm); m->rccl_comm = nullptr; }
    return init(&m->rccl_comm, world, id, rank);
}
extern "C" void moshi_hot_depth_shard_rccl_free(moshi_hot_model_t * m) {
    if (m->rccl_comm && m->rccl_comm_destroy) { ggml_backend_mi355x_make_current(m->be); ggml_backend_synchronize(m->be); m->rccl_comm_destroy(m->rccl_comm); }
    m->rccl_comm = nullptr;
}
extern "C" void moshi_hot_depth_shard_broadcast(moshi_hot_model_t * m, int which, int root) { STREAMS_REFUSE(); shard_broadcast(m, which ? m->shard_tout : m->shard_msg, root); }
extern "C" int64_t moshi_hot_depth_shard_hops(moshi_hot_model_t * m) { return m->shard_hops; }
extern "C" void moshi_hot_depth_shard_install(moshi_hot_model_t * m) { STREAMS_REFUSE(); moshi_hot_set_depth_hook(m, shard_frame_hook, m); }
extern "C" void moshi_hot_depth_shard_stop(moshi_hot_model_t * m) { STREAMS_REFUSE();
    moshi_hot_depth_shard_begin_export(m, 0, 0);
    shard_broadcast(m, m->shard_tout, 0);
}
extern "C" int64_t moshi_hot_depth_shard_serve(moshi_hot_model_t * m) { STREAMS_REFUSE(-1);
    int64_t frames = 0;
    for (;;) {
        shard_broadcast(m, m->shard_tout, 0);
        if (!moshi_hot_depth_shard_begin_import(m)) return frames;
        shard_chain(m);
        frames++;
    }
}
extern "C" int moshi_hot_host_ring(moshi_hot_model_t * m, int32_t * dst, int max_values) { STREAMS_REFUSE(-1);
    const int n = (int) m->ring.rows.size();
    if (dst && n <= max_values) m->ring.export_rows(dst);
    return !dst || n <= max_values ? n : 0;
}
extern "C" void moshi_hot_set_depth_hook(moshi_hot_model_t * m, moshi_hot_depth_hook_t fn, void * user) { STREAMS_REFUSE(); m->depth_hook = fn; m->depth_hook_user = user; }

namespace {
int lm_finish(moshi_hot_model * m, int32_t text_token, std::vector<int32_t> audio, bool provided, bool replace, int32_t * text_token_out, int32_t * out_audio, float * vad, bool newer_step_queued = false) {
    m->last_text = text_token; m->last_audio = audio;
    m->ring.commit(text_token, audio.data(), provided, newer_step_queued);
    const DelayRing::ReadOut r = replace ? DelayRing::ReadOut::filling : m->ring.read_out(text_token_out, audio.data());
    if (r == DelayRing::ReadOut::filling) return 0;
    for (int i = 0; i < m->proto.io_dep_q; i++) out_audio[i] = audio[(size_t) i];
    if (r != DelayRing::ReadOut::valid) return 0;
    if (vad) {
        if (m->extra_heads.size() > 2) {
            Builder & s = *m->scratch;
            T sm = ggml_soft_max(s, linear(s, m->extra_heads[2], m->transformer_out));
            s.expand_read(ggml_view_1d(s, sm, 1, 0), vad);
            s.compute_scratch();
        } else *vad = 0.f;
    }
    return 1;
}
}

namespace { void lm_finish_entry(moshi_hot_model * m, moshi_hot_model::InFlight & f); }
extern "C" int moshi_hot_lm_step_n(moshi_hot_model_t * m, const int32_t * tokens, int n_tokens, int32_t * text_token_out, int32_t * out_audio, float * vad) { STREAMS_REFUSE(-1);
    for (auto & o : m->inflight) lm_finish_entry(m, o);
    const moshi_hot_config & c = m->cfg;
    DelayRing & ring = m->ring;
    const int ncb = c.n_q + 1, needed = m->proto.needed();
    const int offset = (int) ring.frames;
    const bool provided = needed > 0 && n_tokens == ncb;
    if (provided) ring.feed_provided(tokens);
    else if (needed > 0) { GGML_ASSERT(n_tokens >= needed); ring.feed_user(tokens, ring.frames); }

    if (m->tp_frame) tp_build_frame_graphs(m);
    else if (!m->g_temporal) build_temporal_graph(m);
    int32_t text_token = 0;
    const bool chain = c.chain_depth && c.dep_q > 0 && !m->depth_hook;
    GGML_ASSERT(!(c.chain_depth && (m->text_hook || m->depth_hook)) && "chain_depth: the text token never visits the host between the two graphs");
    {
    PhaseTimer pt(m, 1);
    for (int i = 0; i < ncb; i++) {
        const int32_t id = ring.input(i, ring.frames);
        if (i == 0 && c.demux_second_stream) { demux_set(c, id, m->emb_idx[0], m->emb_right_idx, m->emb_right_scale); continue; }
        const TokenInput in = token_input(id);
        ggml_backend_tensor_set(m->emb_idx[(size_t) i], &in.row, 0, 4);
        ggml_backend_tensor_set(m->emb_scale[(size_t) i], &in.scale, 0, 4);
    }
    if (m->tp_frame) tp_temporal_frame(m);
    else {
    if (m->temporal_staged) m->temporal_staged = false;
    else {
        transformer_graph_step(*m->scratch, m->temporal, 1);
        m->scratch->compute_scratch();
    }
    if (m->any_seeded) stage_sampling(m);
    m->g_temporal->compute();
    }
    if (m->after_temporal_launch) { m->after_temporal_launch(); m->after_temporal_launch = nullptr; }
    if (!chain) ggml_backend_tensor_get(m->sampler_out, &text_token, 0, 4);
    }
    if (m->text_hook) text_token = m->text_hook(m->text_hook_user, offset, text_token);

    std::vector<int32_t> audio((size_t) c.dep_q, 0);
    const bool replace = offset < c.delay_steps;
    if (c.dep_q > 0) {
        if (!replace) {
            if (m->depth_hook) m->depth_hook(m->depth_hook_user, text_token, audio.data()); else depth_step(m, text_token, audio);
            if (chain) ggml_backend_tensor_get(m->sampler_out, &text_token, 0, 4);
        }
        else for (auto & a : audio) a = -1;
        if (c.delay_steps)
            for (int q = 0; q < c.dep_q; q++) if (offset < c.delays[q + 1] + c.delay_steps) audio[(size_t) q] = -1;
    }
    m->tok_state_for = provided ? -1 : offset + 1;
    return lm_finish(m, text_token, audio, provided, replace, text_token_out, out_audio, vad);
}

namespace {
bool run_ahead_config(const moshi_hot_model * m) {
    const moshi_hot_config & c = m->cfg;
    return c.chain_depth == 2 && m->tok_state && c.dep_q > 0 && !c.demux_second_stream && !c.delay_steps && !c.extra_heads &&
           !m->text_hook && !m->depth_hook && c.dep_shard_world <= 1;
}
ggml_backend_event_t take_event(moshi_hot_model * m) {
    if (!m->ev_pool.empty()) { ggml_backend_event_t e = m->ev_pool.back(); m->ev_pool.pop_back(); return e; }
    return ggml_backend_event_new(ggml_backend_get_device(m->be));
}
void lm_finish_entry(moshi_hot_model * m, moshi_hot_model::InFlight & f) {
    if (f.done || !f.ev) return;
    ggml_backend_event_synchronize(f.ev);
    m->ev_pool.push_back(f.ev); f.ev = nullptr;
    std::vector<int32_t> audio(f.raw.begin() + 1, f.raw.end());
    bool newer = false, seen = false;
    for (auto & o : m->inflight) { if (&o == &f) seen = true; else if (seen && o.steady) newer = true; }
    f.ok = lm_finish(m, f.raw[0], audio, false, false, &f.out_text, f.out_audio.data(), nullptr, newer);
    f.done = true;
}
void lm_queue(moshi_hot_model * m, const int32_t * user_codes) {
    const moshi_hot_config & c = m->cfg;
    const int ncb = c.n_q + 1, dep_q_1 = m->proto.io_dep_q + 1, needed = m->proto.needed();
    auto from_device = [&](int i) { return i < dep_q_1 || (i <= c.dep_q && c.delays[i] > 0); };
    int q = (int) m->ring.frames;
    for (auto & o : m->inflight) if (!o.done) q++;
    bool steady = run_ahead_config(m) && !m->timing && m->g_temporal && m->g_depth && m->tok_state_for == q;
    for (int i = 0; steady && i < ncb; i++) if (from_device(i) && q <= c.delays[i]) steady = false;
    m->inflight.emplace_back();
    moshi_hot_model::InFlight & f = m->inflight.back();
    f.out_audio.assign((size_t) c.dep_q + 8, 0);
    if (!steady) {
        for (auto & o : m->inflight) if (&o != &f) lm_finish_entry(m, o);
        f.ok = moshi_hot_lm_step_n(m, user_codes, needed, &f.out_text, f.out_audio.data(), nullptr);
        f.done = true;
        return;
    }
    f.steady = true;
    m->ring.feed_user(user_codes, q);
    for (int i = 0; i < ncb; i++) {
        TokenInput in = token_input(m->ring.input(i, q));
        if (from_device(i)) in.scale = 1.f;
        else ggml_backend_tensor_set(m->emb_idx[(size_t) i], &in.row, 0, 4);
        ggml_backend_tensor_set(m->emb_scale[(size_t) i], &in.scale, 0, 4);
    }
    if (m->temporal_staged) m->temporal_staged = false;
    else { transformer_graph_step(*m->scratch, m->temporal, 1); m->scratch->compute_scratch(); }
    m->g_temporal->compute();
    if (m->after_temporal_launch) { m->after_temporal_launch(); m->after_temporal_launch = nullptr; }
    { const float one = 1.f; ggml_backend_tensor_set(m->dep_text_scale, &one, 0, 4); }
    m->g_depth->compute();
    transformer_graph_step(*m->scratch, m->temporal, 1);
    m->scratch->compute_scratch();
    m->temporal_staged = true;
    f.raw.assign((size_t) c.dep_q + 1, 0);
    f.ev = take_event(m);
    ggml_backend_tensor_get_async(m->be, m->tok_state, f.raw.data(), 0, f.raw.size() * 4);
    ggml_backend_event_record(f.ev, m->be);
    m->tok_state_for = q + 1;
}
int lm_complete(moshi_hot_model * m, int32_t * text_token, int32_t * out_audio) {
    GGML_ASSERT(!m->inflight.empty());
    moshi_hot_model::InFlight & f = m->inflight.front();
    lm_finish_entry(m, f);
    const int ok = f.ok;
    if (ok) { *text_token = f.out_text; memcpy(out_audio, f.out_audio.data(), (size_t) m->proto.io_dep_q * sizeof(int32_t)); }
    m->inflight.pop_front();
    return ok;
}
}

extern "C" int moshi_hot_lm_step_run_ahead(moshi_hot_model_t * m, const int32_t * in_audio, int32_t * text_token_out, int32_t * out_audio) { STREAMS_REFUSE(-1);
    if (in_audio) lm_queue(m, in_audio);
    const size_t keep = in_audio ? 1 : 0;
    if (m->inflight.size() <= keep) return -1;
    return lm_complete(m, text_token_out, out_audio);
}

extern "C" int moshi_hot_lm_step(moshi_hot_model_t * m, const int32_t * in_audio, int32_t * text_token_out, int32_t * out_audio) {
    return moshi_hot_lm_step_n(m, in_audio, m->proto.needed(), text_token_out, out_audio, nullptr);
}

namespace {
void set_token_inputs(T idx, T scale, const std::vector<int32_t> & ids) {
    std::vector<int32_t> rows(ids.size()); std::vector<float> sc(ids.size());
    for (size_t b = 0; b < ids.size(); b++) { const TokenInput in = token_input(ids[b]); rows[b] = in.row; sc[b] = in.scale; }
    ggml_backend_tensor_set(idx, rows.data(), 0, rows.size() * 4);
    ggml_backend_tensor_set(scale, sc.data(), 0, sc.size() * 4);
}
struct PassInputs {
    std::vector<std::vector<int32_t>> ids; std::vector<std::vector<float>> scales;
    PassInputs(int ncb, int Tn) : ids((size_t) ncb, std::vector<int32_t>((size_t) Tn)), scales((size_t) ncb, std::vector<float>((size_t) Tn)) {}
    void set(int i, int row, TokenInput in) { ids[(size_t) i][(size_t) row] = in.row; scales[(size_t) i][(size_t) row] = in.scale; }
};
void provided_frames(DelayRing & ring, const int32_t * tokens, int n, int row0, PassInputs & in) {
    const int ncb = ring.p->cols();
    for (int t = 0; t < n; t++) {
        ring.feed_provided(tokens + (size_t) t * ncb);
        for (int i = 0; i < ncb; i++) in.set(i, row0 + t, token_input(ring.input(i, ring.frames)));
        ring.commit(0, nullptr, true);
    }
}
T embedding_sum_rows(moshi_hot_model * m, Builder & s, const PassInputs & in, int Tn) {
    T input = nullptr;
    for (size_t i = 0; i < in.ids.size(); i++) {
        T idx = s.i32s(in.ids[i]);
        T sc = s.constant(s.tensor(GGML_TYPE_F32, 1, Tn), in.scales[i].data());
        T e = ggml_mul(s, ggml_get_rows(s, i == 0 ? m->text_emb : m->emb[i - 1], idx), sc);
        input = input ? ggml_add(s, input, e) : e;
    }
    return m->cfg.condition_sum ? ggml_add(s, m->cond_sum, input) : input;
}
T causal_mask_block(Builder & s, int C, int64_t pos, int n) {
    std::vector<float> mv((size_t) C * (size_t) n);
    for (int t = 0; t < n; t++) for (int cc = 0; cc < C; cc++) mv[(size_t) t * (size_t) C + (size_t) cc] = cc <= pos + t ? 0.0f : -INFINITY;
    return s.constant(s.tensor(GGML_TYPE_F32, C, n), mv.data());
}
void lm_step_columns(moshi_hot_model * m, const int32_t * in_audio, const int32_t * text_in, int32_t * text_token_out, int32_t * out_audio, int32_t * status) {
    const moshi_hot_config & c = m->cfg;
    const int B = m->n_streams, ncb = c.n_q + 1, dep_q = c.dep_q, needed = m->proto.needed();
    int n_open = 0;
    for (int b = 0; b < B; b++) {
        const auto & col = m->cols[(size_t) b];
        status[b] = !col.open ? -1 : col.held ? -2 : 0;
        n_open += col.open && !col.held;
    }
    m->last_heads.assign(m->last_heads.size(), -1.f);
    if (!n_open) return;
    if (!m->g_temporal) build_temporal_graph(m);
    if (dep_q > 0 && !m->g_depth) build_depth_graph_streams(m);
    for (int b = 0; b < B; b++) {
        auto & col = m->cols[(size_t) b];
        if (needed > 0 && col.open && !col.held) col.ring.feed_user(in_audio + (size_t) b * needed, col.ring.frames);
    }
    std::vector<int32_t> ids((size_t) B), text((size_t) B), toks((size_t) B * dep_q), audio((size_t) dep_q);
    std::vector<float> heads(m->last_heads.size());
    const size_t heads_row = heads.size() / (size_t) B;
// ... 600 lines not shown
```

Before: 448.2 frames/s.

## Fuse RoPE table, embedding sum and mask row into one temporal head kernel

Adds a temporal_head kernel that computes the input embedding sum, the timestep/RoPE row and the attention mask bias row in a single launch. Because the mask row is now computed on device from the offset, the per-step scratch graph (bias pattern copy) and its compute are skipped. Only the offset/index uploads remain. Redundant dep_text_scale uploads are also cached. This removes a separate scratch graph launch and host sync per frame. It adds plan-time aliasing checks and a new kernel whose correctness depends on matching the old mask pattern.

After: 449.9 frames/s (median of 6 runs). About the same (+0.4%).

```diff
diff --git a/include/ggml-backend.h b/include/ggml-backend.h
--- a/include/ggml-backend.h
+++ b/include/ggml-backend.h
@@ -119,6 +119,8 @@
 GGML_API void ggml_backend_mi355x_get_kernel_profile(ggml_backend_t backend, struct ggml_mi355x_kernel_profile * out);
 GGML_API void ggml_backend_mi355x_set_flags(ggml_backend_t backend, int flags);
 GGML_API void ggml_backend_mi355x_set_capture(ggml_backend_t backend, int enabled);
+GGML_API int ggml_backend_mi355x_bind_step_feed(ggml_backend_t backend, const struct ggml_tensor * offset, const struct ggml_tensor * bias);
+GGML_API int ggml_backend_mi355x_graph_step_head(ggml_backend_t backend, const struct ggml_cgraph * cgraph);
 GGML_API void * ggml_backend_mi355x_get_stream(ggml_backend_t backend);
 GGML_API void ggml_backend_mi355x_make_current(ggml_backend_t backend);
 GGML_API ggml_backend_t ggml_backend_mi355x_init_stream(ggml_backend_t base);
diff --git a/moshi.cpp_amd/__init__.py b/moshi.cpp_amd/__init__.py
--- a/moshi.cpp_amd/__init__.py
+++ b/moshi.cpp_amd/__init__.py
@@ -126,6 +126,7 @@
     "ggml_backend_mi355x_get_stream": (P, [P]),
     "ggml_backend_mi355x_make_current": (None, [P]),
     "ggml_backend_mi355x_init_stream": (P, [P]),
+    "ggml_backend_mi355x_bind_step_feed": (I, [P, TP, TP]), "ggml_backend_mi355x_graph_step_head": (I, [P, P]),
     "ggml_backend_tensor_get_async": (None, [P, TP, P, Z, Z]),
     "ggml_backend_event_new": (P, [P]), "ggml_backend_event_free": (None, [P]), "ggml_backend_event_record": (None, [P, P]),
     "ggml_backend_event_synchronize": (None, [P]),
diff --git a/moshi.cpp_amd/csrc/hip_backend.hip b/moshi.cpp_amd/csrc/hip_backend.hip
--- a/moshi.cpp_amd/csrc/hip_backend.hip
+++ b/moshi.cpp_amd/csrc/hip_backend.hip
@@ -56,6 +56,8 @@
     char * aget_pinned = nullptr;
     std::deque<async_get> aget_pending;
     uint64_t aget_seq = 0;
+    struct step_feed { const void * offset; float * bias; int C; };
+    std::vector<step_feed> feeds;
     bool in_use = false;
     int usable_cus = 0;
     ggml_backend_device dev_obj;
@@ -257,6 +259,7 @@
     chain_plan * chain = nullptr;
     const vq_level_args * vq = nullptr;
     const char * hoist_dst = nullptr; size_t hoist_bytes = 0;
+    std::shared_ptr<temporal_head_args> head; int head_part = 0, head_node = -1, head_earliest = -1, head_bias_reader = -1;
     template <typename F> pstep(F f) : fn(std::move(f)) { memset(&mv, 0, sizeof(mv)); }
     pstep(const mv_args & a) : fn([a](hipStream_t s) { k_matvec(s, a); }), is_mv(true), mv(a) {}
     template <typename F> static pstep special_step(F f, int special, const attn_args * at, const lowrank_embed_args * lr, const sample_args * smp = nullptr) {
@@ -281,6 +284,7 @@
     hipGraph_t graph = nullptr;
     hipGraphExec_t exec = nullptr;
     uint64_t hash = 0;
+    bool step_head = false;
     int n_nodes = 0, n_fused = 0, n_chained = 0, n_attn_folded = 0, n_step_programs = 0, n_vq_chained = 0, n_attn_block_launches = 0, n_attn_block_jobs = 0, n_generic_attn_nodes = 0, n_ring_copy_launches = 0, n_ring_copy_jobs = 0;
 };
 
@@ -1983,7 +1987,9 @@
             if (clash) continue;
             for (int m : grp.members) an.skip[(size_t) m] = 1;
             const embed_sum_args a = grp.a;
-            at_pos[i].push_back([=](hipStream_t s) { k_embed_sum(s, a); });
+            pstep st([=](hipStream_t s) { k_embed_sum(s, a); });
+            if (a.B <= 1 && !c->feeds.empty() && !(c->flags & 2048)) { st.head = std::make_shared<temporal_head_args>(); memset(st.head.get(), 0, sizeof(temporal_head_args)); st.head->es = a; st.head_part = 2; st.head_node = i; }
+            at_pos[i].push_back(std::move(st));
             p->n_fused += (int) grp.members.size();
         }
         for (int i = 0; i < g->n_nodes; i++) {
@@ -2026,6 +2032,25 @@
             {
                 pstep st([=](hipStream_t s) { k_timestep_embedding(s, d, tx, dim, mp, yp, yn); });
                 if (x->op == GGML_OP_NONE && y->op == GGML_OP_NONE && !x->view_src && !y->view_src) { st.hoist_dst = (const char *) n->data; st.hoist_bytes = ggml_nbytes(n); }
+                if (st.hoist_dst && yn == 1 && ggml_nelements(ad) == 1 && ggml_is_contiguous(n) && n->type == GGML_TYPE_F32 && ggml_nelements(n) == dim && !(c->flags & 2048))
+                    for (const hip_ctx::step_feed & f : c->feeds) if (f.offset == (const void *) yp) {
+                        st.head = std::make_shared<temporal_head_args>(); memset(st.head.get(), 0, sizeof(temporal_head_args));
+                        st.head->rope = (float *) n->data; st.head->ts = (const float *) x->data; st.head->offset = yp; st.head->dim = dim; st.head->max_period = mp;
+                        st.head->bias = f.bias; st.head->C = f.C; st.head_part = 1; st.head_node = i;
+                        auto overlaps = [](const ggml_tensor * t, const char * q, size_t nq) { return t && t->data && (const char *) t->data < q + nq && q < (const char *) t->data + ggml_nbytes(t); };
+                        int earliest = 0, reader = g->n_nodes;
+                        for (int k = 0; k < g->n_nodes; k++) {
+                            const ggml_tensor * o = g->nodes[k];
+                            bool touches = overlaps(o, (const char *) n->data, ggml_nbytes(n));
+                            for (int sidx = 0; sidx < GGML_MAX_SRC; sidx++) {
+                                if (overlaps(o->src[sidx], (const char *) n->data, ggml_nbytes(n))) touches = true;
+                                if (overlaps(o->src[sidx], (const char *) f.bias, (size_t) f.C * 4) && k < reader) reader = k;
+                            }
+                            if (touches && k < i) earliest = k + 1;
+                        }
+                        st.head_bias_reader = reader;
+                        st.head_earliest = earliest;
+                    }
                 at_pos[i].push_back(std::move(st));
             }
             p->n_fused += 2;
@@ -2280,6 +2305,22 @@
         auto it = at_pos.find(i);
         if (it != at_pos.end()) for (auto & f : it->second) p->steps.push_back(f);
     }
+    for (size_t i = 0; fuse && keep && i < p->steps.size(); i++) {
+        if (p->steps[i].head_part != 2) continue;
+        size_t j = p->steps.size();
+        if (i > 0 && p->steps[i - 1].head_part == 1) j = i - 1;
+        else for (size_t k = i + 1; k < p->steps.size() && j == p->steps.size(); k++) if (p->steps[k].head_part == 1 && (k == i + 1 || p->steps[k].head_earliest <= p->steps[i].head_node)) j = k;
+        if (j == p->steps.size()) continue;
+        temporal_head_args ha = *p->steps[j].head;
+        ha.es = p->steps[i].head->es;
+        const size_t at = i < j ? i : j;
+        if (!k_temporal_head_supported(ha) || p->steps[j].head_bias_reader < p->steps[at].head_node) continue;
+        p->steps[at] = pstep([=](hipStream_t s) { k_temporal_head(s, ha); });
+        p->steps.erase(p->steps.begin() + (long) (i < j ? j : i));
+        p->step_head = true;
+        if (dump) fprintf(stderr, "plan: RoPE table + %d-term embedding sum + mask row -> one head launch\n", ha.es.n);
+        break;
+    }
     if (fuse && keep && !(c->flags & 16) && ((c->flags & 32) || k_chain_default_on()) && spin_kernels_possible(c)) {
         for (size_t i = 1; i + 1 < p->steps.size(); i++) {
             pstep & h = p->steps[i];
@@ -2588,6 +2629,21 @@
     c->plans.clear();
     c->flags = flags;
 }
+extern "C" int ggml_backend_mi355x_bind_step_feed(ggml_backend_t b, const struct ggml_tensor * offset, const struct ggml_tensor * bias) {
+    if (!b || b->iface.get_name != hip_backend_name || !offset || !offset->data) return 0;
+    hip_ctx * c = (hip_ctx *) b->context;
+    for (size_t i = c->feeds.size(); i-- > 0;) if (c->feeds[i].offset == offset->data) c->feeds.erase(c->feeds.begin() + (long) i);
+    if (!bias || (c->flags & 2048)) return 0;
+    if (offset->type != GGML_TYPE_F32 || ggml_nelements(offset) != 1 || bias->type != GGML_TYPE_F32 || !bias->data || !ggml_is_contiguous(bias) || ggml_nelements(bias) != bias->ne[0]) return 0;
+    c->feeds.push_back({ offset->data, (float *) bias->data, (int) bias->ne[0] });
+    return 1;
+}
+extern "C" int ggml_backend_mi355x_graph_step_head(ggml_backend_t b, const struct ggml_cgraph * g) {
+    if (!b || b->iface.get_name != hip_backend_name) return 0;
+    hip_ctx * c = (hip_ctx *) b->context;
+    auto it = c->plans.find(g);
+    return it != c->plans.end() && !it->second->orphan_seq && it->second->step_head && !(c->flags & 2048) ? 1 : 0;
+}
 extern "C" void ggml_backend_mi355x_get_kernel_profile(ggml_backend_t b, struct ggml_mi355x_kernel_profile * out) {
     hip_ctx * c = ctx_of(b);
     out->seconds = c->prof_seconds; out->launches = c->prof_launches; out->bytes = c->prof_bytes;
diff --git a/moshi.cpp_amd/csrc/hip_common.h b/moshi.cpp_amd/csrc/hip_common.h
--- a/moshi.cpp_amd/csrc/hip_common.h
+++ b/moshi.cpp_amd/csrc/hip_common.h
@@ -166,6 +166,13 @@
 #define EMBED_SUM_MAX 40
 struct embed_sum_args { embed_src src[EMBED_SUM_MAX]; int n; int64_t K; float * out; int B; };
 void k_embed_sum(hipStream_t s, const embed_sum_args & a);
+struct temporal_head_args {
+    embed_sum_args es;
+    float * rope; const float * ts; const float * offset; int dim, max_period;
+    float * bias; int C;
+};
+bool k_temporal_head_supported(const temporal_head_args & a);
+void k_temporal_head(hipStream_t s, const temporal_head_args & a);
 struct vq_level_args {
     const char * emb; int64_t emb_row_bytes; int D, NC;
     const char * resid; int64_t resid_stride;
diff --git a/moshi.cpp_amd/csrc/hip_device.h b/moshi.cpp_amd/csrc/hip_device.h
--- a/moshi.cpp_amd/csrc/hip_device.h
+++ b/moshi.cpp_amd/csrc/hip_device.h
@@ -199,6 +199,17 @@
     mn[1] = ((u2 >> 4) & kmask2) | (((u1 >> 6) & kmask3) << 4);
 }
 
+__device__ __forceinline__ void timestep_row(float * e, float t, int dim, int max_period, int tid, int n) {
+    const int half = dim / 2;
+    for (int j = tid; j < half; j += n) {
+        const float lf = (float) log((double) max_period);
+        const float freq = (float) exp((double) (-lf * j / half));
+        const float arg = t * freq;
+        e[j] = (float) cos((double) arg);
+        e[j + half] = (float) sin((double) arg);
+    }
+    if (tid == 0 && (dim & 1)) e[2 * half] = 0.f;
+}
 __device__ __forceinline__ float dequant_elem(const char * row, int type, int64_t i) {
     switch (type) {
         case GGML_TYPE_F32:  return ((const float *) row)[i];
diff --git a/moshi.cpp_amd/csrc/hip_kernels_fused.hip b/moshi.cpp_amd/csrc/hip_kernels_fused.hip
--- a/moshi.cpp_amd/csrc/hip_kernels_fused.hip
+++ b/moshi.cpp_amd/csrc/hip_kernels_fused.hip
@@ -2090,6 +2090,90 @@
 #undef EMBED_LAUNCH
 }
 
+#define HEAD_EPL 4
+#define HEAD_NMAX 24
+template <int TYPE>
+__device__ __forceinline__ void head_embed_sum(const embed_sum_args & a, int wg, int tid) {
+    const int64_t i0 = ((int64_t) wg * 256 + tid) * HEAD_EPL;
+    if (i0 >= a.K) return;
+    constexpr int BB = TYPE == GGML_TYPE_Q4_0 ? 18 : 34;
+    const int64_t boff = (i0 >> 5) * BB;
+    const int j = (int) (i0 & 31);
+    const int64_t qoff = boff + 2 + (TYPE == GGML_TYPE_Q4_0 ? (j & 15) : j);
+    int64_t r[HEAD_NMAX];
+    float sc[HEAD_NMAX];
+    uint16_t dh[HEAD_NMAX], qa[HEAD_NMAX], qb[HEAD_NMAX];
+#pragma unroll
+    for (int t = 0; t < HEAD_NMAX; t++) {
+        if (t < a.n) {
+            const embed_src & e = a.src[t];
+            r[t] = e.index[0];
+            sc[t] = e.scale ? e.scale[0] : 1.f;
+        }
+    }
+#pragma unroll
+    for (int t = 0; t < HEAD_NMAX; t++) {
+        if (t < a.n) {
+            const embed_src & e = a.src[t];
+            const int64_t row = (r[t] < 0 || r[t] >= e.n_rows) ? 0 : r[t];
+            const char * base = e.table + row * e.row_bytes;
+            dh[t] = *(const uint16_t *) (base + boff);
+            qa[t] = *(const uint16_t *) (base + qoff);
+            qb[t] = *(const uint16_t *) (base + qoff + 2);
+        }
+    }
+    __builtin_amdgcn_sched_barrier(0);
+    float acc[HEAD_EPL] = { 0.f, 0.f, 0.f, 0.f };
+#pragma unroll
+    for (int t = 0; t < HEAD_NMAX; t++) {
+        if (t < a.n) {
+            const float d = h2f(dh[t]);
+            const uint32_t q4 = (uint32_t) qa[t] | ((uint32_t) qb[t] << 16);
+#pragma unroll
+            for (int k = 0; k < HEAD_EPL; k++) {
+                const uint32_t byte = (q4 >> (8 * k)) & 0xFFu;
+                float v;
+                if (TYPE == GGML_TYPE_Q4_0) { const int q = j < 16 ? (int) (byte & 0x0F) : (int) (byte >> 4); v = (q - 8) * d; }
+                else v = (int8_t) byte * d;
+                const float x = a.src[t].scale ? v * sc[t] : v;
+                acc[k] = t == 0 ? x : acc[k] + x;
+            }
+        }
+    }
+#pragma unroll
+    for (int k = 0; k < HEAD_EPL; k++) a.out[i0 + k] = acc[k];
+}
+template <int TYPE>
+__global__ void __launch_bounds__(256) temporal_head_kernel(temporal_head_args a, int n_sum_wgs) {
+    const int wg = (int) blockIdx.x, tid = (int) threadIdx.x;
+    if (wg < n_sum_wgs) { head_embed_sum<TYPE>(a.es, wg, tid); return; }
+    if (wg == n_sum_wgs) { timestep_row(a.rope, a.ts[0] + a.offset[0], a.dim, a.max_period, tid, 256); return; }
+    const int C = a.C, off = (int) a.offset[0];
+    const int col = off <= C ? 2 * C - 1 - off : C - off % C;
+    for (int i = tid; i < C; i += 256) a.bias[i] = col + i < 2 * C ? 0.0f : -INFINITY;
+}
+static int temporal_head_type(const temporal_head_args & a) {
+    int type = a.es.n > 0 ? a.es.src[0].type : -1;
+    for (int t = 1; t < a.es.n; t++) if (a.es.src[t].type != type) type = -1;
+    return type;
+}
+bool k_temporal_head_supported(const temporal_head_args & a) {
+    const int type = temporal_head_type(a);
+    if (type != GGML_TYPE_Q4_0 && type != GGML_TYPE_Q8_0) return false;
+    if (a.es.n < 1 || a.es.n > HEAD_NMAX || a.es.B > 1 || a.es.K < 32 || a.es.K % 32 != 0 || !a.es.out) return false;
+    for (int t = 0; t < a.es.n; t++) {
+        const embed_src & e = a.es.src[t];
+        if (!e.table || !e.index || ((uintptr_t) e.table & 1) || (e.row_bytes & 1) || e.row_bytes < a.es.K / 32 * (type == GGML_TYPE_Q4_0 ? 18 : 34) || e.n_rows < 1) return false;
+    }
+    return a.rope && a.ts && a.offset && a.bias && a.dim >= 2 && a.max_period > 0 && a.C >= 1;
+}
+void k_temporal_head(hipStream_t s, const temporal_head_args & a) {
+    GGML_ASSERT(k_temporal_head_supported(a));
+    const int n_sum_wgs = (int) ((a.es.K + 256 * HEAD_EPL - 1) / (256 * HEAD_EPL));
+    if (temporal_head_type(a) == GGML_TYPE_Q4_0) temporal_head_kernel<GGML_TYPE_Q4_0><<<n_sum_wgs + 2, 256, 0, s>>>(a, n_sum_wgs);
+    else temporal_head_kernel<GGML_TYPE_Q8_0><<<n_sum_wgs + 2, 256, 0, s>>>(a, n_sum_wgs);
+}
+
 #define VQ_CPW 4
 __global__ void __launch_bounds__(256) vq_level_kernel(vq_level_args a) {
     __shared__ float sv[4];
diff --git a/moshi.cpp_amd/csrc/hip_kernels_generic.hip b/moshi.cpp_amd/csrc/hip_kernels_generic.hip
--- a/moshi.cpp_amd/csrc/hip_kernels_generic.hip
+++ b/moshi.cpp_amd/csrc/hip_kernels_generic.hip
@@ -757,18 +757,10 @@
 
 __global__ void timestep_embedding_kernel(tdesc dst, tdesc ts, int dim, int max_period, const float * addend, int addend_n) {
     const int64_t i = blockIdx.x;
-    const int half = dim / 2;
     float * e = (float *) at(dst, 0, i, 0, 0);
     float t = *(const float *) at(ts, i, 0, 0, 0);
     if (addend) t = t + addend[addend_n == 1 ? 0 : i];
-    for (int j = threadIdx.x; j < half; j += blockDim.x) {
-        const float lf = (float) log((double) max_period);
-        const float freq = (float) exp((double) (-lf * j / half));
-        const float arg = t * freq;
-        e[j] = (float) cos((double) arg);
-        e[j + half] = (float) sin((double) arg);
-    }
-    if (threadIdx.x == 0 && (dim & 1)) e[2 * half] = 0.f;
+    timestep_row(e, t, dim, max_period, (int) threadIdx.x, (int) blockDim.x);
 }
 void k_timestep_embedding(hipStream_t s, tdesc dst, tdesc ts, int dim, int max_period, const float * addend, int addend_n) {
     if (ts.ne[0]) timestep_embedding_kernel<<<(int) ts.ne[0], 64, 0, s>>>(dst, ts, dim, max_period, addend, addend_n);
diff --git a/moshi.cpp_amd/csrc/moshi_hot.cpp b/moshi.cpp_amd/csrc/moshi_hot.cpp
--- a/moshi.cpp_amd/csrc/moshi_hot.cpp
+++ b/moshi.cpp_amd/csrc/moshi_hot.cpp
@@ -541,9 +541,13 @@
     ggml_backend_tensor_set(tr.g_indices, idx.data(), 0, idx.size() * 4);
 }
 
+void transformer_step_uploads(Transformer & tr, int Tn, int offset);
 void transformer_graph_step_at(Builder & scratch, Transformer & tr, int Tn, int offset) {
     T bias = bias_pattern_index(scratch, tr, Tn, offset);
     scratch.expand(ggml_cpy(scratch, bias, tr.g_bias));
+    transformer_step_uploads(tr, Tn, offset);
+}
+void transformer_step_uploads(Transformer & tr, int Tn, int offset) {
     if (tr.g_offset) { const float f = (float) offset; ggml_backend_tensor_set(tr.g_offset, &f, 0, 4); }
     std::vector<int32_t> idx((size_t) Tn);
     for (int i = 0; i < Tn; i++) idx[(size_t) i] = (offset + i) % tr.capacity;
@@ -765,6 +769,8 @@
 
     std::vector<int32_t> tokens_tmp;
     std::vector<int32_t> pipe_codes, pipe_tokens; bool pipe_have_codes = false, pipe_have_tokens = false; float pipe_vad = 0.f;
+    bool temporal_feed = false;
+    bool dep_text_scale_known = false; float dep_text_scale_value = 0.f;
     bool temporal_staged = false;
     std::function<void()> after_temporal_launch;
     int32_t last_text = 0; std::vector<int32_t> last_audio;
@@ -932,6 +938,8 @@
         g.expand(ggml_cpy(g, sm, row));
     }
     g.alloc();
+    if (m->kind == ModelKind::single && m->n_streams == 1 && m->temporal.g_offset)
+        m->temporal_feed = ggml_backend_mi355x_bind_step_feed(m->be, m->temporal.g_offset, m->temporal.g_bias) != 0;
 }
 
 void build_depth_graph(moshi_hot_model * m) {
@@ -951,6 +959,7 @@
         last = ggml_add(g, ly, ggml_mul(g, ry, m->dep_right_scale));
     } else {
         m->dep_text_scale = g.tensor(GGML_TYPE_F32, 1);
+        m->dep_text_scale_known = false;
         last = ggml_mul(g, ggml_get_rows(g, m->depformer_text_emb, m->dep_text_idx), m->dep_text_scale);
         if (m->dep_text_low_rank) last = linear(g, m->dep_text_low_rank, last);
     }
@@ -1394,6 +1403,7 @@
     if (!m) return;
     ggml_backend_synchronize(m->be);
     moshi_hot_depth_shard_rccl_free(m);
+    if (m->temporal_feed) ggml_backend_mi355x_bind_step_feed(m->be, m->temporal.g_offset, nullptr);
     for (auto & f : m->inflight) if (f.ev) ggml_backend_event_free(f.ev);
     for (auto e : m->ev_pool) ggml_backend_event_free(e);
     if (m->own_codec_be) ggml_backend_synchronize(m->be_codec);
@@ -1475,6 +1485,26 @@
     ggml_backend_tensor_set(right, r.data(), 0, r.size() * 4);
     ggml_backend_tensor_set(right_scale, sc.data(), 0, sc.size() * 4);
 }
+void set_dep_text_scale(moshi_hot_model * m, float sc) {
+    if (m->dep_text_scale_known && m->dep_text_scale_value == sc) return;
+    ggml_backend_tensor_set(m->dep_text_scale, &sc, 0, 4);
+    m->dep_text_scale_known = true; m->dep_text_scale_value = sc;
+}
+bool temporal_plan_has_head(moshi_hot_model * m) {
+    return m->temporal_feed && m->g_temporal && m->g_temporal->gf && ggml_backend_mi355x_graph_step_head(m->be, m->g_temporal->gf) != 0;
+}
+void temporal_step_inputs(moshi_hot_model * m) {
+    if (m->temporal_staged) { m->temporal_staged = false; return; }
+    if (temporal_plan_has_head(m)) { transformer_step_uploads(m->temporal, 1, m->temporal.offset); m->temporal.offset += 1; return; }
+    transformer_graph_step(*m->scratch, m->temporal, 1);
+    m->scratch->compute_scratch();
+}
+void stage_temporal(moshi_hot_model * m) {
+    if (m->temporal_staged || temporal_plan_has_head(m)) return;
+    transformer_graph_step(*m->scratch, m->temporal, 1);
+    m->scratch->compute_scratch();
+    m->temporal_staged = true;
+}
 void depth_step(moshi_hot_model * m, int32_t text_token, std::vector<int32_t> & audio) {
     PhaseTimer pt(m, 2);
     if (!m->g_depth) build_depth_graph(m);
@@ -1483,15 +1513,11 @@
         int32_t id = text_token; const float sc = id == -1 ? 0.f : 1.f;
         if (id < 0) id = 0;
         if (!m->cfg.chain_depth) ggml_backend_tensor_set(m->dep_text_idx, &id, 0, 4);
-        ggml_backend_tensor_set(m->dep_text_scale, &sc, 0, 4);
+        set_dep_text_scale(m, sc);
     }
     if (m->any_seeded) stage_sampling(m);
     m->g_depth->compute();
-    if (m->cfg.chain_depth && !m->temporal_staged) {
-        transformer_graph_step(*m->scratch, m->temporal, 1);
-        m->scratch->compute_scratch();
-        m->temporal_staged = true;
-    }
+    if (m->cfg.chain_depth) stage_temporal(m);
     ggml_backend_tensor_get(m->dep_tokens, audio.data(), 0, audio.size() * 4);
 }
 void unstage_temporal(moshi_hot_model * m) { if (m->temporal_staged) { m->temporal.offset -= 1; m->temporal_staged = false; } }
@@ -1879,11 +1905,7 @@
     }
     if (m->tp_frame) tp_temporal_frame(m);
     else {
-    if (m->temporal_staged) m->temporal_staged = false;
-    else {
-        transformer_graph_step(*m->scratch, m->temporal, 1);
-        m->scratch->compute_scratch();
-    }
+    temporal_step_inputs(m);
     if (m->any_seeded) stage_sampling(m);
     m->g_temporal->compute();
     }
@@ -1952,15 +1974,12 @@
         else ggml_backend_tensor_set(m->emb_idx[(size_t) i], &in.row, 0, 4);
         ggml_backend_tensor_set(m->emb_scale[(size_t) i], &in.scale, 0, 4);
     }
-    if (m->temporal_staged) m->temporal_staged = false;
-    else { transformer_graph_step(*m->scratch, m->temporal, 1); m->scratch->compute_scratch(); }
+    temporal_step_inputs(m);
     m->g_temporal->compute();
     if (m->after_temporal_launch) { m->after_temporal_launch(); m->after_temporal_launch = nullptr; }
-    { const float one = 1.f; ggml_backend_tensor_set(m->dep_text_scale, &one, 0, 4); }
+    set_dep_text_scale(m, 1.f);
     m->g_depth->compute();
-    transformer_graph_step(*m->scratch, m->temporal, 1);
-    m->scratch->compute_scratch();
-    m->temporal_staged = true;
+    stage_temporal(m);
     f.raw.assign((size_t) c.dep_q + 1, 0);
     f.ev = take_event(m);
     ggml_backend_tensor_get_async(m->be, m->tok_state, f.raw.data(), 0, f.raw.size() * 4);
```
